# cts198859/deeprl_network

Hardware: AMD Instinct MI355X
Metric: env-steps/sec (agents x envs x steps/s), full rollout + A2C update loop (higher is better)
Workload: dtype f32; 1 GPU; CACC catchup, 8 agents x 4096 replicas/GPU, ia2c_fp (config_ia2c_fp_catchup.ini), n_step 60; replicas_per_gpu=4096, global_replicas=4096, parallelism=dp1, hipgraph_rollout=True, hipgraph_update=True, gemm_autotune=True

## Files before the change

deeprl_network_amd/_lib.py:

```python
import ctypes as C
import os

import torch

_PKG = os.path.dirname(os.path.abspath(__file__))
LIB_PATH = os.path.join(_PKG, 'libnmarl_hip.so')

if not os.path.exists(LIB_PATH):
    raise ImportError(
        'deeprl_network_amd: %s not found. Build it with `python -m deeprl_network_amd.build` '
        '(hipcc --offload-arch=gfx950). There is no CPU fallback.' % LIB_PATH)

from . import build as _build

if _build.built_hash() != _build.source_hash():
    raise ImportError(
        'deeprl_network_amd: %s is stale (built from sources %s, current sources %s). Rebuild it with '
        '`python -m deeprl_network_amd.build`.' % (LIB_PATH, _build.built_hash(), _build.source_hash()))

LIB_PATH = os.environ.get('NMARL_LIB_AB') or LIB_PATH
lib = C.CDLL(LIB_PATH)

ABI_VERSION = 4

# ... 49 lines not shown


class NetTopo(C.Structure):
    _fields_ = [('N', C.c_int32), ('L', C.c_int32), ('A', C.c_int32), ('m_max', C.c_int32), ('n_s', C.c_void_p),
                ('image', C.c_void_p)]


NET_OFF = dict(green=0, src=6144, group=7680, share=8448, fan=11520, dnptr=11648, dnpair=11728, nbr=13264)
NET_IMAGE_BYTES = 13568


class FcPart(C.Structure):
    _fields_ = [('x', C.c_void_p), ('x_sn', C.c_int64), ('x_row', C.c_int64), ('F', C.c_int32), ('gather_A', C.c_int32),
                ('m_max', C.c_int32), ('pad_', C.c_int32), ('nbr_idx', C.c_void_p), ('w', C.c_void_p), ('w_sn', C.c_int64),
                ('b', C.c_void_p), ('b_sn', C.c_int64)]


FC_MAX_PARTS = 4


class CaccEncode(C.Structure):
    _fields_ = ([(k, C.c_void_p) for k in ('w_ob', 'b_ob', 'w_fp', 'b_fp', 'fp', 'nbr_idx', 'out')] +
                [(k, C.c_int64) for k in ('w_ob_sn', 'b_ob_sn', 'w_fp_sn', 'b_fp_sn', 'fp_sn', 'out_sn', 'out_row')] +
                [('act', C.c_int32), ('n_parts', C.c_int32)])


class BatchEpilogue(C.Structure):
    _fields_ = ([('E', C.c_int64)] + [(k, C.c_int32) for k in ('N', 'H', 'A', 'F', 'T', 'T_env')] +
                [(k, C.c_void_p) for k in ('g', 'done', 'ep_sum', 'ep_sq', 'ep_len', 'fin', 'h_fw', 'c_fw', 'h_bw', 'c_bw', 'fp_T',
                                           'fp_uniform', 'x_T', 'fp_0', 'x_0', 'done_pre', 'scratch', 'skip_if')])


class TrainRecord(C.Structure):
    _fields_ = ([('rows', C.c_int64)] + [(k, C.c_int32) for k in ('N', 'A', 'G', 'K')] + [('lr', C.c_float), ('e_coef', C.c_float)] +
                [(k, C.c_void_p) for k in ('n_a', 'terms', 'grad_norm', 'lr_dev', 'R', 'Adv', 'action', 'ring', 'count', 'skip_if',
                                           'ws')])


class BpttCoupled(C.Structure):
    _fields_ = ([(k, C.c_int32) for k in ('kind', 'N', 'T', 'H', 'm_max', 'r_max', 'r_row', 'symmetric', 'mode', 'ring_slots')] +
                [('E', C.c_int64)] +
                [(k, C.c_void_p) for k in ('gates', 'c_all', 'done', 'dh_ext', 'img', 'img_m', 'mask', 'dz', 'd1', 'ring', 'db_part',
                                           'dbm_part', 'dhr_io', 'dc_io', 'ws', 'status', 'rev_agent', 'rev_col', 'rev_w')] +
                [(k, C.c_int64) for k in ('gates_sn', 'gates_st', 'c_sn', 'c_st', 'dh_sn', 'dh_st', 'img_sn', 'imgm_sn', 'mask_sn',
                                          'mask_st', 'mask_row', 'dz_sn', 'dz_st', 'd1_sn', 'd1_st', 'ring_sn', 'ring_slot', 'db_sn',
                                          'dbm_sn', 'io_sn')] +
                [('dy8', C.c_void_p), ('hw', C.c_void_p), ('dy_sn', C.c_int64), ('dy_st', C.c_int64), ('hw_sn', C.c_int64),
                 ('O', C.c_int32), ('pad2_', C.c_int32)])


class BpttDial(C.Structure):
    _fields_ = ([(k, C.c_int32) for k in ('N', 'T', 'H', 'm_max', 'r_max', 'r_row', 'symmetric', 'mode', 'ring_slots', 'O')] +
                [('E', C.c_int64)] +
                [(k, C.c_void_p) for k in ('gates', 'c_all', 'done', 'dh_ext', 'dy8', 'hw', 'img', 'img_m', 'img_f', 'hm', 'msg', 'dz',
                                           'ds', 'd1', 'd2', 'ring', 'db_part', 'dbm_part', 'dbf_part', 'dhr_io', 'dc_io', 'ws',
                                           'status', 'rev_agent', 'rev_col', 'rev_w')] +
                [(k, C.c_int64) for k in ('gates_sn', 'gates_st', 'c_sn', 'c_st', 'dh_sn', 'dh_st', 'dy_sn', 'dy_st', 'hw_sn', 'img_sn',
                                          'imgm_sn', 'imgf_sn', 'hm_sn', 'hm_st', 'hm_row', 'msg_sn', 'msg_st', 'dz_sn', 'dz_st',
                                          'ds_sn', 'ds_st', 'd1_sn', 'd1_st', 'd2_sn', 'd2_st', 'ring_sn', 'ring_slot', 'db_sn',
                                          'dbm_sn', 'dbf_sn', 'io_sn')])


class GridParams(C.Structure):
    _fields_ = [('norm_wave', C.c_float), ('clip_wave', C.c_float), ('peak1', C.c_float), ('peak2', C.c_float),
                ('T', C.c_int32), ('per_agent_reward', C.c_int32), ('compact_obs', C.c_int32),
                ('objective', C.c_int32), ('coef_wait', C.c_float), ('head_wait', C.c_void_p)]


class GridEnv(C.Structure):
    _fields_ = ([('params', C.POINTER(GridParams))] +
                [(k, C.c_void_p) for k in ('q', 'transit', 'prev_action', 't', 'xi', 'obs_out', 'reward', 'done', 'global_reward')] +
                [('auto_reset', C.c_int32), ('pad_', C.c_int32), ('seed', C.c_uint64), ('env_id_base', C.c_int64),
                 ('episode', C.c_void_p), ('words', C.c_void_p)])


class StepX(C.Structure):
    _fields_ = ([('E', C.c_int64)] + [(k, C.c_int32) for k in ('N', 'H', 'KX', 'KX2', 'precision', 'pad_')] +
                [('x', C.c_void_p), ('x_sn', C.c_int64), ('x_row', C.c_int64), ('x2', C.c_void_p), ('x2_sn', C.c_int64),
                 ('x2_row', C.c_int64)] +
                [('h_in', C.c_void_p), ('h_sn', C.c_int64)] +
                [f for k in ('img', 'bias', 'zadd1', 'zadd2', 'c_prev') for f in ((k, C.c_void_p), (k + '_sn', C.c_int64))] +
                [('done', C.c_void_p)] +
                [f for k in ('gates', 'c_new', 'h_new') for f in ((k, C.c_void_p), (k + '_sn', C.c_int64))] +
                [('head', C.POINTER(Head)), ('msg', C.POINTER(Msg)), ('enc', C.POINTER(StepEnc)), ('genv', C.POINTER(GridEnv))])


_p = C.c_void_p
_i64 = C.c_int64
_i32 = C.c_int32
_u64 = C.c_uint64
_f32 = C.c_float

SIGNATURES = {
    'nmarl_abi_version': [],
    'nmarl_cacc_reset': [C.POINTER(CaccParams), _i64, _p, _p, _u64, _i64, _p,
                         _p, _p, _p, _p, _p, _p, _p, _p, _i32, _p],
    'nmarl_cacc_step': [C.POINTER(CaccParams), _i64, _p, _p, _p, _p, _p, _p, _p, _p, _p, _p, _p,
                        _i32, _u64, _i64, _p, _p],
    'nmarl_cacc_step_encode': [C.POINTER(CaccParams), _i64, _p, _p, _p, _p, _p, _p, _p, _p, _p, _p, _p,
                               _i32, _u64, _i64, _p, C.POINTER(CaccEncode), _p],
    'nmarl_cacc_step_nv': [C.POINTER(CaccParams), _i64, _p, _p, _p, _p, _p, _p, _p, _p, _p, _p, _p,
                           _i32, _u64, _i64, _p, _i32, _p],
    'nmarl_cacc_reset_nv': [C.POINTER(CaccParams), _i64, _p, _p, _u64, _i64, _p,
                            _p, _p, _p, _p, _p, _p, _p, _p, _i32, _i32, _p],
    'nmarl_grid_reset': [C.POINTER(GridParams), _i64, _p, _p, _u64, _i64, _p, _p, _p, _p, _p, _p, _p, _p],
    'nmarl_grid_step': [C.POINTER(GridParams), _i64, _p, _p, _p, _p, _p, _p, _p, _p, _p, _p, _i32, _u64, _i64, _p, _p],
    'nmarl_grid_reset_rc': [C.POINTER(GridParams), _i64, _p, _p, _u64, _i64, _p, _p, _p, _p, _p, _p, _p, _p, _i32, _i32],
    'nmarl_grid_step_rc': [C.POINTER(GridParams), _i64, _p, _p, _p, _p, _p, _p, _p, _p, _p, _p, _i32, _u64, _i64, _p, _p,
                           _i32, _i32],
    'nmarl_net_reset': [C.POINTER(NetTopo), _i64, _p, _p, _u64, _i64, _p, _p, _p, _p, _p, _p, _p, _p],
    'nmarl_net_reset_obj': [C.POINTER(NetParams), C.POINTER(NetTopo), _i64, _p, _p, _u64, _i64, _p, _p, _p, _p, _p, _p, _p, _p],
    'nmarl_net_step': [C.POINTER(NetParams), C.POINTER(NetTopo), _i64, _p, _p, _p, _p, _p, _p, _p, _p, _p, _p, _i32, _u64, _i64,
                       _p, _p],
    'nmarl_atsc_traffic_begin': [_i64, _i32, _i32, _p, _p, _p, _p, _p],
    'nmarl_atsc_traffic_step': [_i64, _i32, _i32, _p, _p, _p, _p, _p, _p, _p, _p, _p, _p, _p],
    'nmarl_atsc_greedy': [_i64, _i32, _i32, _p, _p, _p, _i64, _p, _p],
    'nmarl_atsc_maxpressure': [_i64, _i32, _i32, _i32, _p, _p, _i32, _i32, _p, _p, _p, _p, _p, _i64, _p, _p],
    'nmarl_nbr_gather_fwd': [_i64, _i32, _i32, _i32, _p, _p, _p, _p],
    'nmarl_nbr_gather_bwd': [_i64, _i32, _i32, _i32, _p, _p, _p, _p],
    'nmarl_nbr_mean_fwd': [_i64, _i32, _i32, _i32, _p, _p, _p, _p],
    'nmarl_nbr_mean_bwd': [_i64, _i32, _i32, _i32, _p, _p, _p, _p],
    'nmarl_nbr_gather_bwd_add': [_i64, _i32, _i32, _i32, _p, _p, _p, _p, _p],
    'nmarl_nbr_mean_bwd_add': [_i64, _i32, _i32, _i32, _p, _p, _p, _p, _p],
    'nmarl_nbr_onehot': [_i64, _i32, _i32, _i32, _p, _p, _p, _i64, _p],
    'nmarl_lstm_cell_fwd': [_i64, _i32, _i32, _p, _i64, _p, _i64, _p, _i64, _p, _i64, _p, _p, _i64, _p, _i64, _p, _i64, _p],
    'nmarl_lstm_wimage_floats': [_i32],
    'nmarl_lstm_wimage': [_i32, _i32, _p, _i64, _p, _i64, _p, _i64, _i32, _p],
    'nmarl_lstm_step_x': [C.POINTER(StepX), _p],
    'nmarl_lstm_msg_wimage': [_i32, _i32, _p, _i64, _p, _i64, _p],
    'nmarl_lstm_step_sync_words': [_i64, _i32],
    'nmarl_lstm_step_env_words': [_i64],
    'nmarl_lstm_step_grid_words': [_i64],
    'nmarl_lstm_step_grid_env_blocks': [_i64, _i32],
    'nmarl_lstm_bptt_wimage_floats': [_i32],
    'nmarl_lstm_bptt_wimage': [_i32, _i32, _p, _i64, _p, _i64, _p, _i64, _p],
    'nmarl_lstm_bptt_step': [_i64, _i32, _i32, _i32, _p, _i64, _p, _i64, _p, _i64, _p, _p, _i64, _p, _i64, _p, _i64, _p, _i64, _p,
                             _i64, _p, _i64, _p, _i64, _p, _i64, _i64, _p, _i64, _i32, _p, _i64, _p],
    'nmarl_lstm_bptt_step_parts': [_i64],
    'nmarl_lstm_bptt_seq_blocks': [_i64],
    'nmarl_lstm_bptt_seq': [_i32, _i64, _i32, _i32, _p, _i64, _i64, _p, _i64, _i64, _p, _p, _i64, _i64, _p, _i64, _i64, _p, _i64, _i32,
                            _p, _i64, _p, _i64, _i64, _p, _i64, _p, _i64, _p, _i64, _p],
    'nmarl_lstm_bptt_msg_wimage': [_i32, _i32, _p, _i64, _p, _i64, _p],
    'nmarl_lstm_bptt_coupled_ws_words': [_i64, _i32],
    'nmarl_lstm_bptt_coupled': [C.POINTER(BpttCoupled), _p],
    'nmarl_lstm_bptt_dial': [C.POINTER(BpttDial), _p],
    'nmarl_fc_fwd': [_i64, _i32, _i32, _i32, _p, _i64, _i64, _p, _i64, _p, _i64, _i32, _p, _i64, _i64, _p],
    'nmarl_fc_fwd_multi': [_i64, _i32, _i32, C.POINTER(FcPart), _i32, _p, _i64, _i64, _p],
    'nmarl_dial_msg_adjoint': [_i64, _i32, _i32, _p, _i64, _p, _i64, _p, _i64, _p, _i64, _p, _i64, _p, _i64, _p, _p, _p, _i32,
                               _p, _i64, _p, _i64, _p, _i64, _p, _i64, _p, _i64, _p],
    'nmarl_dial_msg_adjoint_parts': [_i64],
    'nmarl_onehot_argmax_add': [_i64, _i32, _i32, _i32, _p, _i64, _p, _p, _i64, _i64, _p],
    'nmarl_fc_bwd_chunks': [_i64, _i32],
    'nmarl_fc_bwd': [_i64, _i32, _i32, _i32, _p, _i64, _i64, _p, _i64, _i64, _p, _i64, _i64, _i32, _p, _p, _i64, _p, _i64, _p],
    'nmarl_fc_bwd_pair': [_i64, _i32, _p, _p, _i64, _i64, _p, _i64, _p, _i64, _i64, _i32, _p, _p, _p],
    'nmarl_fc_bwd_gather': [_i64, _i32, _i32, _i32, _p, _i32, _p, _i64, _i64, _p, _i64, _i64, _p, _i64, _i64, _i32, _p, _p, _i64, _p, _i64, _p],
    'nmarl_heads_loss': [_i64, _i32, _i32, _i32, _p, _i64, _p, _i64, _p, _i64, _p, _p, _p, _p, _f32, _f32, _p, _p, _p, _p, _p, _i64, _p, _i64, _p,
                         _i64, _p],
    'nmarl_thin_linear_bwd': [_i64, _i32, _i32, _i32, _p, _i64, _p, _i64, _p, _i64, _p, _i64, _p, _p, _i64, _p, _i64, _p, _i64, _p],
    'nmarl_nbr_action_value_fwd': [_i64, _i32, _i32, _i32, _p, _p, _p, _i64, _p, _i32, _p],
    'nmarl_nbr_action_value_bwd': [_i64, _i32, _i32, _i32, _p, _p, _p, _p, _p, _i64, _p],
    'nmarl_bias_act': [_i64, _i32, _i32, _p, _i64, _p, _i64, _i32, _p, _i64, _i64, _p],
    'nmarl_lstm_cell_bwd': [_i64, _i32, _i32, _p, _i64, _p, _i64, _p, _i64, _p, _p, _i64, _p, _i64, _p, _i64, _p, _i64, _p, _i64, _p],
    'nmarl_a2c_loss_chunks': [_i64, _i32],
    'nmarl_a2c_loss_fwd': [_i64, _i32, _i32, _p, _i64, _i64, _p, _p, _p, _p, _f32, _f32, _p, _p, _p],
    'nmarl_a2c_loss_bwd': [_i64, _i32, _i32, _p, _i64, _i64, _p, _p, _p, _p, _f32, _f32, _p, _p, _p, _p],
    'nmarl_sample_actions': [_i64, _i32, _i32, _p, _p, _i32, _u64, _i64, _i64, _p, _p, _p],
    'nmarl_nstep_return': [_i64, _i32, _i32, _p, _p, _p, _p, C.c_double, C.c_double, _p, _p, _p, _p],
# ... 49 lines not shown
```

deeprl_network_amd/agents/models.py:

```python
import logging
import os

import numpy as np
import torch

from .. import ops, train_record
from .policies import (ConsensusPolicy, DIALMultiAgentPolicy, FPPolicy, IC3MultiAgentPolicy, LstmPolicy,
                       NCMultiAgentPolicy)
from .utils import Scheduler

F32 = torch.float32


class IA2C:

    policy_cls = LstmPolicy
    per_agent_optimizer = True
    uses_fingerprint = False

    def __init__(self, n_s_ls, n_a_ls, neighbor_mask, distance_mask, coop_gamma, total_step, model_config,
                 seed=0, num_envs=1, device='cuda', dist_group=None, n_feat=None, n_feat_ls=None, obs_order=None):
        self.name = getattr(self, 'name', 'ia2c')
        self._init_algo(n_s_ls, n_a_ls, neighbor_mask, distance_mask, coop_gamma, total_step, seed,
                        model_config, num_envs, device, dist_group, n_feat, n_feat_ls, obs_order)
# ... 144 lines not shown
        p = self.policy
        if p.hetero or p.n_obs == p.n_feat:
            return False
        if p.params[p.k_ob].shape[2] != ops.FC_J or p.n_obs > ops.FC_MAX_F:
            return False
        T, E, N = self.n_step, self.E, self.n_agent
        self.buf_x = torch.zeros(T + 1, E, N, p.n_feat, dtype=F32, device=self.device)
        self.compact_obs = True
        return True

    compact_obs = False

    def _save_slots(self, t):
        d = {k: v[:, t] for k, v in self.policy._extra.items()}
        d['S'] = self.S_buf[:, t]
        for k, v in getattr(self, '_extra_next', {}).items():
            d[k + '_next'] = v[:, t + 1]
        return d

    def reset_states(self, mask=None):
        self.policy.invalidate_cached_msg()
        if mask is None:
            for s in (self.h_fw, self.c_fw, self.h_bw, self.c_bw):
                s.zero_()
            self.fp.copy_(self.fp_uniform.expand_as(self.fp))
        else:
            keep = (mask == 0).to(F32).view(1, -1, 1)
            for s in (self.h_fw, self.c_fw, self.h_bw, self.c_bw):
                s.mul_(keep)
            self.fp.mul_(keep).add_((1.0 - keep) * self.fp_uniform)

    def _policy_step(self, obs, done, done_is_zero=False):
        self.policy.refresh_wimage()
        self._enc = self.policy.encode(obs, self.fp)
        self.policy.step(self._enc, self.h_fw, self.c_fw, done, self.h_fw, self.c_fw, done_is_zero)
        with torch.no_grad():
            return self.policy.pi(self.h_fw)

    def _value_step(self, obs, done, na_onehot, done_is_zero=False, out=None, reuse_enc=False):
        if not reuse_enc:
            self.policy.refresh_wimage()
        enc = self._enc if reuse_enc else self.policy.encode(obs, self.fp)
        self.policy.step(enc, self.h_fw, self.c_fw, done, self._h2, self._c2, done_is_zero, second=True)
        with torch.no_grad():
            return self.policy.value(self._h2, na_onehot, out=out)

    def encode_target(self, t):
        if t < self.n_step:
            return self.S_buf[:, t]
        if getattr(self, '_enc_boot', None) is None:
            self._enc_boot = torch.zeros_like(self.S_buf[:, 0])
        return self._enc_boot

    def act(self, done, mode=ops.SAMPLE_PHILOX, u=None, seed=0, env_id_base=0, step=0, step_dev=None,
            done_is_zero=False, pre_encoded=False, env_step=None):
        t = self.t
        p = self.policy
        ob = None
        if t == 0:
            p.refresh_wimage()
            if self.save_acts:
                self.H_all[:, 0].copy_(self.h_fw)
                self.C_all[:, 0].copy_(self.c_fw)
        if pre_encoded:
            enc = self.S_buf[:, t]
        elif self.save_acts and p.enc_in_kernel(self.E, self.compact_obs):
            enc, ob = self.S_buf[:, t], dict(x=self.buf_x[t], fp=self.fp, env=env_step, bits=self._relu_bits(t))
        elif self.save_acts and 'ENC' in p._extra:
            if p.encodes_in_step(self.E, self.compact_obs):
                enc, ob = p._extra['ENC'][:, t], (self.buf_x[t] if env_step is None else dict(x=self.buf_x[t], genv=env_step))
            else:
                enc = p.encode(self.buf_x[t], self.fp, out=p._extra['ENC'][:, t])
            p._enc_was_saved = True
        else:
            enc = p.encode(self.buf_x[t], self.fp, out=self.S_buf[:, t]) if self.save_acts else p.encode(self.buf_x[t], self.fp)
        if env_step is not None and (ob is None or not isinstance(ob, dict)):
            raise ValueError('env_step needs the lock-step kernel that runs the input encoders itself (policy.enc_in_kernel / encodes_in_step)')
        draw = dict(mode=mode, u=u, seed=seed, env_id_base=env_id_base, step=step, step_dev=step_dev)
        if self.save_acts and p.pv_one_launch(self.E):
            p.step_policy_value(enc, self.H_all[:, t], self.C_all[:, t], done, self.buf_fp[t + 1], self.buf_act[t],
                                self.buf_vn[:, t], h_out=self.H_all[:, t + 1], c_out=self.C_all[:, t + 1],
                                gates=self.G_buf[:, t], defer_action_term=True,
                                **(dict(save=self._save_slots(t), ob=ob, carry=self._msg_carry(t)) if p.coupled else
                                   (dict(ob=ob) if ob is not None else {})),
                                **draw)
            return self.buf_act[t]
        if self.save_acts:
            p.step_policy(enc, self.H_all[:, t], self.C_all[:, t], done, self.H_all[:, t + 1], self.C_all[:, t + 1],
                          self.buf_fp[t + 1], self.buf_act[t], done_is_zero, gates=self.G_buf[:, t], save=self._save_slots(t),
                          **draw)
            p.step_value(enc, self.H_all[:, t + 1], self.C_all[:, t + 1], done, self._h2, self._c2, self.buf_act[t],
                         self.buf_v[t], done_is_zero)
            return self.buf_act[t]
        if p.fused_pv:
            p.step_policy_value(enc, self.h_fw, self.c_fw, done, self.buf_fp[t + 1], self.buf_act[t], self.buf_v[t], **draw)
            return self.buf_act[t]
        p.step_policy(enc, self.h_fw, self.c_fw, done, self.h_fw, self.c_fw, self.buf_fp[t + 1], self.buf_act[t],
                      done_is_zero, **draw)
        p.step_value(enc, self.h_fw, self.c_fw, done, self._h2, self._c2, self.buf_act[t], self.buf_v[t], done_is_zero)
        return self.buf_act[t]

    _carry_buf = None
    _carry_holds = -1

    def _msg_carry(self, t):
        p = self.policy
        if not p.coupled or getattr(p, 'msg_kind', 0) not in (ops.MSG_GATHER_RELU, ops.MSG_MEAN_ADD) or \
                os.environ.get('NMARL_MSG_CARRY', '1') == '0':
            return None
        if self._carry_buf is None:
            self._carry_buf = torch.zeros(self.n_agent, self.E, self.n_lstm, dtype=F32, device=self.device)
        d = dict(carry_in=self._carry_buf if (t > 0 and self._carry_holds == t) else None,
                 carry_out=self._carry_buf if t < self.n_step else None)
        mm = getattr(p, '_extra_full', {}).get('MM')
        if mm is not None and t + 1 < self.n_step and p.msg_kind == ops.MSG_MEAN_ADD:
            d['mean_next'] = mm[:, t + 1]
        self._carry_holds = t + 1 if t < self.n_step else -1
        return d

    S_bits = None

    def _relu_bits(self, t):
        if os.environ.get('NMARL_FC_BWD_PAIR', '1') == '0' or not getattr(self.policy, 'enc_writes_bits', False):
            return None
        if self.S_bits is None:
            self.S_bits = torch.zeros(self.n_agent, self.n_step, self.E, 4, dtype=torch.int32, device=self.device)
        p = self.policy
        p._bits_steps = 1 if t == 0 else p._bits_steps + 1
        return self.S_bits[:, t]

    def record(self, reward, done_post):
        t = self.t
        self.buf_r[t].copy_(self._norm_reward(reward))
        self.buf_done_post[t].copy_(done_post)
        self.t = t + 1

    def _norm_reward(self, r):
        if self.reward_norm > 0:
            r = r / self.reward_norm
        if self.reward_clip > 0:
            r = torch.clamp(r, -self.reward_clip, self.reward_clip)
        return r

    def load_rewards(self, raw_rewards):
        if self.reward_norm > 0:
            torch.div(raw_rewards, self.reward_norm, out=self.buf_r)
        else:
            torch.mul(raw_rewards, 1.0, out=self.buf_r)
        if self.reward_clip > 0:
            self.buf_r.clamp_(-self.reward_clip, self.reward_clip)
        self.t = self.n_step

    def bootstrap(self, done, action_scratch, mode=ops.SAMPLE_PHILOX, u=None, seed=0, env_id_base=0,
                  step=0, step_dev=None, done_is_zero=False, pre_encoded=False):
        assert self.t == self.n_step
        p = self.policy
        ob = None
        if pre_encoded:
            enc = self.encode_target(self.n_step)
        elif self.save_acts and p.enc_in_kernel(self.E, self.compact_obs):
            enc, ob = (self.encode_target(self.n_step) if p.coupled else None), dict(x=self.buf_x[self.n_step], fp=self.fp)
        elif self.save_acts and p.encodes_in_step(self.E, self.compact_obs):
            enc, ob = self.encode_target(self.n_step), self.buf_x[self.n_step]
        else:
            enc = p.encode(self.buf_x[self.n_step], self.fp)
        if self.save_acts and p.pv_one_launch(self.E):
            T = self.n_step
            p.step_policy_value(enc, self.H_all[:, T], self.C_all[:, T], done, self._pi_boot, action_scratch, self._v_boot,
                                h_out=self.h_fw, c_out=self.c_fw, mode=mode, u=u, seed=seed, env_id_base=env_id_base,
                                step=step, step_dev=step_dev, **(dict(ob=ob) if ob is not None else {}),
                                **(dict(carry=self._msg_carry(T)) if p.coupled else {}))
            return self._v_boot
        if self.save_acts:
            T = self.n_step
            p.step_policy(enc, self.H_all[:, T], self.C_all[:, T], done, self.h_fw, self.c_fw, self._pi_boot, action_scratch,
                          done_is_zero, mode=mode, u=u, seed=seed, env_id_base=env_id_base, step=step, step_dev=step_dev)
            return p.step_value(enc, self.h_fw, self.c_fw, done, self._h2, self._c2, action_scratch, self._v_boot,
                                done_is_zero)
        if p.fused_pv:
            p.step_policy_value(enc, self.h_fw, self.c_fw, done, self._pi_boot, action_scratch, self._v_boot, mode=mode, u=u,
                                seed=seed, env_id_base=env_id_base, step=step, step_dev=step_dev)
            return self._v_boot
        p.step_policy(enc, self.h_fw, self.c_fw, done, self.h_fw, self.c_fw, self._pi_boot, action_scratch,
                      done_is_zero, mode=mode, u=u, seed=seed, env_id_base=env_id_base, step=step, step_dev=step_dev)
        return p.step_value(enc, self.h_fw, self.c_fw, done, self._h2, self._c2, action_scratch, self._v_boot,
                            done_is_zero)

    def _loss_backward_fused(self, Hs):
        N, T, E = self.n_agent, self.n_step, self.E
        p = self.policy
        if Hs.dim() != 3 or not ops.heads_loss_supported(Hs, self.n_a, p.nbr_idx) or \
                (not self.identical_agent and not self.per_agent_optimizer) or Hs.stride(2) != 1 or Hs.stride(1) != Hs.shape[2]:
            return False
        prm = p.params
        action = self.buf_act.view(T * E, N)
        as_dy = self.save_acts and p.bptt_takes_head_dy and os.environ.get('NMARL_BPTT_HEAD_DY', '1') != '0'
        r = ops.heads_loss(Hs.detach(), prm['pi_w'], prm['pi_b'], prm['v_w'], prm['v_b'], action, p.nbr_idx, self.n_a,
                           self.Adv.view(N, T * E), self.R.view(N, T * E), self.v_coef, self.e_coef, want_dh=not as_dy)
        terms = self._terms = r['terms']
        self.last_loss = (terms[:, 0], terms[:, 1], terms[:, 2], terms.sum(dim=1))
        for k in ('pi_w', 'pi_b', 'v_w', 'v_b'):
            prm[k].grad = r[k].reshape(prm[k].shape)
        Hs.backward(gradient=ops.head_dy_placeholder(r['dy8'], r['hw'], Hs) if as_dy else r['dh'])
        if as_dy and ops._pending_head_dy.pop(Hs.device, None) is not None:
            raise RuntimeError('the recurrence below Hs did not take the heads\' dy8 (ops.take_head_dy): its gradient is wrong')
        return True

    def _loss(self, Hs):
        N, T, E = self.n_agent, self.n_step, self.E
        p = self.policy
        action = self.buf_act.view(T * E, N)
        logits, v = p.heads(Hs, action)
        adv = self.Adv.view(N, T * E)
        R = self.R.view(N, T * E)
        if not self.identical_agent and not self.per_agent_optimizer:
            adv = adv.sum(dim=0, keepdim=True).expand(N, T * E).contiguous()
        if ops.a2c_loss_supported(self.n_a):
            per_agent, terms = ops.a2c_loss(logits, v, action, adv, R, self.v_coef, self.e_coef)
            self._terms = terms
            self.last_loss = (terms[:, 0], terms[:, 1], terms[:, 2], per_agent.detach())
            return per_agent.sum()
        pi = torch.softmax(logits, dim=-1)
        acts = action.t().long().unsqueeze(-1)
        log_pi = torch.log(torch.clamp(pi, 1e-10, 1.0))
        entropy = -(pi * log_pi).sum(-1)
        logp_a = log_pi.gather(-1, acts).squeeze(-1)
        policy_loss = -(logp_a * adv).mean(-1)
        value_loss = (R - v).pow(2).mean(-1) * 0.5 * self.v_coef
        entropy_loss = -entropy.mean(-1) * self.e_coef
        per_agent = policy_loss + value_loss + entropy_loss
        self._terms = None
        self.last_loss = (policy_loss.detach(), value_loss.detach(), entropy_loss.detach(), per_agent.detach())
        return per_agent.sum()

    def loss_terms(self):
        if self._terms is not None:
            return self._terms
        return torch.stack(self.last_loss[:3], dim=1).contiguous()

    def update(self, R_end, rotate=True):
        lr = self.update_begin()
        self.update_grads(R_end)
        self.update_reduce()
        self.update_apply(lr, rotate=rotate)
        self.update_end()

    def update_begin(self):
        assert self.t == self.n_step, 'update() needs a full n_step batch (got %d)' % self.t
        self.cur_lr = self.lr_scheduler.get(self.n_step)
        return self.cur_lr

    @property
    def handoff_guarded(self):
        return bool(self.policy.coupled) and self.device.type == 'cuda'
# ... 274 lines not shown
```

deeprl_network_amd/agents/policies.py:

```python
import os
import warnings

import numpy as np
import torch

from .. import ops
from . import sequence

warnings.filterwarnings('ignore', message='grad and param do not obey the gradient layout contract')

F32 = torch.float32


def ortho_init(shape, scale=np.sqrt(2)):
    a = np.random.standard_normal(shape)
    u, _, v = np.linalg.svd(a, full_matrices=False)
    q = u if u.shape == tuple(shape) else v
    return (scale * q.reshape(shape)).astype(np.float32)


class Layout:

    def __init__(self, rows=None, cols=None, exists=True, fill=0.0):
        self.rows, self.cols, self.exists, self.fill = rows, cols, exists, fill
# ... 245 lines not shown
        p = self.params
        H, A = self.n_h, self.n_a
        if ops.heads_supported(h, A, self.nbr_idx):
            return ops.heads(h, p['pi_w'], p['pi_b'], p['v_w'], p['v_b'], action, self.nbr_idx, A)
        w = torch.cat([p['pi_w'], p['v_w'][:, :H]], dim=2)
        b = torch.cat([p['pi_b'], p['v_b']], dim=1)
        out = torch.baddbmm(b.unsqueeze(1), h, w)
        na = ops.nbr_onehot(action, self.nbr_idx, A)
        return out[..., :A], out[..., A] + torch.bmm(na, p['v_w'][:, H:]).squeeze(-1)

    def value(self, h, na_onehot, out=None):
        p = self.params
        H = self.n_h
        v = torch.baddbmm(p['v_b'].unsqueeze(1), h, p['v_w'][:, :H])
        if out is not None:
            torch.baddbmm(v, na_onehot, p['v_w'][:, H:], out=out.unsqueeze(-1))
            return out
        return torch.baddbmm(v, na_onehot, p['v_w'][:, H:]).squeeze(-1)

    def encode(self, x, fp_prev, out=None):
        with torch.no_grad():
            if out is not None:
                return self._enc_infer(x.transpose(0, 1), fp_prev, out=out)
            return self._enc_infer(x.transpose(0, 1), fp_prev)

    def step(self, enc, h, c, done, h_out, c_out, done_is_zero=False, second=False):
        with torch.no_grad():
            z1, z2, xs = self._recur_addends(enc, h, second=second)
            wh, b = self.params[self.k_wh], self.params[self.k_b]
            if self.n_h == ops.FUSED_H:
                ops.lstm_step_fused(h, wh, b, z1, z2, c, done, None, c_out, h_out, xs=xs, **self._prec_kw)
            else:
                hk = h if done_is_zero else h * (1.0 - done).view(1, -1, 1)
                z = torch.bmm(hk, wh) if z2 is None else torch.baddbmm(z2, hk, wh)
                ops.lstm_cell_infer(z, b, c, done, c_out, h_out, z2=z1)
        return h_out, c_out

    @property
    def fused_heads(self):
        return self.n_h == ops.FUSED_H and self.n_a <= ops.HEAD_MAX_A

    def step_policy(self, enc, h, c, done, h_out, c_out, pi_out, act_out, done_is_zero=False, gates=None, save=None,
                    **draw):
        with torch.no_grad():
            if self.fused_heads:
                z1, z2, xs = self._recur_addends(enc, h, save=save, fuse_msg=self.msg_inplace_ok or h_out.data_ptr() != h.data_ptr())
                p = self.params
                ops.lstm_step_policy(h, p[self.k_wh], p[self.k_b], z1, z2, c, done, c_out, h_out, p['pi_w'], p['pi_b'],
                                     pi_out, act_out, xs=xs, gates=gates, **self._prec_kw, **draw)
            else:
                self.step(enc, h, c, done, h_out, c_out, done_is_zero)
                pi_out.copy_(self.pi(h_out))
                ops.sample_actions(pi_out, act_out, **draw)
        return pi_out, act_out

    @property
    def fused_pv(self):
        return self.fused_heads and not self.coupled

    @property
    def fused_pv_coupled(self):
        return self.coupled and self.fused_heads and self.msg_kind != ops.MSG_DIAL and self._msg() is not None

    def pv_one_launch(self, E):
        if self.fused_pv:
            return True
        K = self.n_h * self.m_max if self.msg_kind == ops.MSG_GATHER_RELU else self.n_h
        if K > ops.MSG_MAX_K:
            return False
        return self.fused_pv_coupled and ops.step_handoff_supported(self.N, E, self.device, K=K)

    def _sync_words(self, E):
        pool = self.__dict__.setdefault('_sync_pool', {})
        if E not in pool:
            pool[E] = ops.step_sync_words(self.N, E, self.device)
        return pool[E]

    def encodes_in_step(self, E, compact):
        return False

    _bits_steps = 0

    def invalidate_cached_msg(self):
        """(lstm_dial keeps message vectors of the last policy step: see DIALMultiAgentPolicy)"""

    def enc_in_kernel(self, E, compact):
        return False

    @property
    def env_step_in_kernel(self):
        return True

    def step_policy_value(self, enc, h, c, done, pi_out, act_out, v_out, h_out=None, c_out=None, gates=None,
                          defer_action_term=False, save=None, ob=None, carry=None, **draw):
        with torch.no_grad():
            if self.coupled:
                z1, z2, xs = self._recur_addends(enc, h, save=save, fuse_msg=True)
                xs[4]['sync'] = self._sync_words(h.shape[1])
                if carry:
                    xs[4].update(carry)
                if isinstance(ob, dict) and 'genv' in ob:
                    xs[4]['ob'], xs[4]['genv'] = self._ob_spec(ob['x']), ob['genv']
                elif isinstance(ob, dict):
                    xs[4]['enc_spec'] = self._enc_spec(ob['x'], ob['fp'], None, ob.get('env'), ob.get('bits'))
                elif ob is not None:
                    xs[4]['ob'] = self._ob_spec(ob)
            elif ob is not None:
                z1, z2, xs = None, None, (self._enc_spec(ob['x'], ob['fp'], enc, ob.get('env'), ob.get('bits')), self.params[self.k_wx],
                                          self._step_img)
            else:
                z1, z2, xs = self._recur_addends(enc, h)
            p = self.params
            ops.lstm_step_policy_value(h, p[self.k_wh], p[self.k_b], z1, z2, c, done, p['pi_w'], p['pi_b'], pi_out, act_out,
                                       p['v_w'], p['v_b'], self.nbr_idx, self.n_a, v_out, xs=xs, h_out=h_out, c_out=c_out,
                                       gates=gates, defer_action_term=defer_action_term, **self._prec_kw, **draw)
        return act_out

    @property
    def bptt_takes_head_dy(self):
        if self.coupled and os.environ.get('NMARL_BPTT_HEAD_DY_COUPLED', '1') == '0':
            return False
        return self.xside

    @property
    def can_save_acts(self):
        return self.xside and self.fused_heads

    def unroll_saved(self, X, FP, S, G, Hall, Call, done, masked_steps=None, S_ext=None, S_bits=None):
        T, E = done.shape
        Xv = X.reshape(T * E, self.N, X.shape[-1]).transpose(0, 1)
        if self.coupled:
            return self._unroll_saved_coupled(Xv, FP, S, G, Hall, Call, done, masked_steps, S_ext, S_bits)
        if S_bits is not None:
            s = self._enc(Xv, FP, saved=S.view(self.N, T * E, S.shape[-1]), bits=S_bits.view(self.N, T * E, 4))
        else:
            s = self._enc(Xv, FP, saved=S.view(self.N, T * E, S.shape[-1]))
        Hs = ops.lstm_sequence_saved(s.view(self.N, T, E, s.shape[-1]), self.params[self.k_wx], self.params[self.k_wh],
                                     self.params[self.k_b], G, Hall, Call, done, masked_steps, s_ext=S_ext)
        return Hs.reshape(self.N, T * E, self.n_h)

    def save_spec(self):
        return {}

    def _unroll_saved_coupled(self, Xv, FP, S, G, Hall, Call, done, masked_steps, S_ext=None, S_bits=None):
        T, E = done.shape
        kind, wx, w_msg, b_msg, mfc_w, mfc_b = self._seq_args()
        enc = self._enc_saved(Xv, FP, S) if S_bits is None else self._enc_saved(Xv, FP, S, bits=S_bits.view(self.N, T * E, 4))
        extra = dict(getattr(self, '_extra', {}))
        if kind == 'dial' and 'A2' in getattr(self, '_extra_full', {}) and extra.get('A2') is not None:
            extra['A2'] = self._extra_full['A2']
        if kind == 'ic3':
            mm = getattr(self, '_extra_full', {}).get('MM') if getattr(self, '_mm_was_saved', False) else None
            extra['A1'] = mm if (mm is not None and mm.shape[1] == T + 1) else None
        Hs = sequence.coupled_sequence_saved(kind, self.nbr_idx, masked_steps, enc.view(self.N, T, E, enc.shape[-1]), done,
                                             self.params[self.k_wx], self.params[self.k_wh], self.params[self.k_b],
                                             w_msg, b_msg, mfc_w, mfc_b, G, Hall, Call, S, extra, s_ext=S_ext)
        return Hs.reshape(self.N, T * E, self.n_h)

    def step_value(self, enc, h, c, done, h_out, c_out, action, v_out, done_is_zero=False):
        with torch.no_grad():
            if self.fused_heads:
                z1, z2, xs = self._recur_addends(enc, h, second=True, fuse_msg=True)
                p = self.params
                ops.lstm_step_value(h, p[self.k_wh], p[self.k_b], z1, z2, c, done, c_out, h_out, p['v_w'], p['v_b'],
                                    action, self.nbr_idx, self.n_a, v_out, xs=xs, **self._prec_kw)
            else:
                self.step(enc, h, c, done, h_out, c_out, done_is_zero, second=True)
                self.value(h_out, ops.nbr_onehot(action, self.nbr_idx, self.n_a), out=v_out)
        return v_out

    def fused_env_encode(self, fp_next, out):
        return None

    def _fused_spec(self, ob, fp_keys, fp_next, out):
        p = self.params
        if self.hetero or self.n_feat != 5 or self.m_max != 2 or self.n_a != 4 or p[ob[0]].shape[1:] != (15, 64):
            return None
        d = dict(w_ob=p[ob[0]], b_ob=p[ob[1]], nbr_idx=self.nbr_idx, out=out, act=ops.BIAS_RELU)
        if fp_keys is not None:
            if p[fp_keys[0]].shape[1:] != (8, 64):
                return None
            d.update(w_fp=p[fp_keys[0]], b_fp=p[fp_keys[1]], fp=fp_next)
        return d

    def _enc_one_launch(self, xv, width):
        return width == ops.FC_J and self.n_obs <= ops.FC_MAX_F and self.n_na <= ops.FC_MAX_F

    def _compact(self, xv):
        return xv.shape[2] == self.n_feat and self.n_obs != self.n_feat

    def _ob_part(self, xv, w_key, b_key):
        p = self.params
        return (xv, p[w_key], p[b_key], self.nbr_self if self._compact(xv) else None)

    def _fc_ob_infer(self, xv, w_key, b_key, act, out=None):
        if self._compact(xv):
            return ops.fc_fwd_multi([self._ob_part(xv, w_key, b_key)], act, out=out)
        return self._fc_infer(xv, w_key, b_key, act, out=out)

    def expand_obs(self, X):
        idx = self.nbr_self.long()
        g = X[..., idx.clamp(min=0), :] * (idx >= 0).to(X.dtype).unsqueeze(-1)
        return g.reshape(*X.shape[:-1], self.n_obs)

    def _fc_infer(self, x, w_key, b_key, act, out=None):
        w, b = self.params[w_key], self.params[b_key]
        if ops.fc_supported(x, w):
            return ops.fc_fwd(x, w, b, act, out=out)
        return ops.bias_act_(torch.bmm(x, w), b, act, out=out)

    def _recur_addends(self, enc, h, second=False, save=None, fuse_msg=False):
        if self.xside:
            return None, None, (enc, self.params[self.k_wx], self._step_img)
        return enc, None, self._wh_xs()

    k_wx = None
    _img = None
    _img_x3 = None

    @property
    def _prec_kw(self):
        return {} if self.precision == 'fp32' else {'precision': self.precision}

    @property
    def _step_img(self):
        return self._img_x3 if self.precision == 'bf16x3' else self._img

    @property
    def xside(self):
        return self.k_wx is not None and ops.xside_supported(self.params[self.k_wx].shape[1], self.n_h)

    def refresh_wimage(self):
        if self.xside:
            self._img = ops.lstm_wimage(self.params[self.k_wx], self.params[self.k_wh], out=self._img)
            if self.precision == 'bf16x3':
                self._img_x3 = ops.lstm_wimage(self.params[self.k_wx], self.params[self.k_wh], out=self._img_x3, precision='bf16x3')
            if self.msg_kind and ops.msg_supported(self.msg_kind, self.m_max, self.n_h):
                self._msg_img = ops.lstm_msg_wimage(self.params['w_msg'], out=self._msg_img)
        elif self.n_h == ops.FUSED_H:
            self._img = ops.lstm_wimage(None, self.params[self.k_wh], out=self._img)

    def _wh_xs(self):
        return (None, None, self._img) if self.n_h == ops.FUSED_H else None

    msg_kind = 0
    msg_inplace_ok = False
    _msg_img = None

    def _msg(self, **kw):
        if not (self.xside and self.msg_kind and self._msg_img is not None):
            return None
        p = self.params
        return dict(kind=self.msg_kind, nbr_idx=self.nbr_idx, w_msg=p['w_msg'], b_msg=p['w_msg_b'], img=self._msg_img, **kw)

    def unroll(self, X, FP, done, h0, c0, masked_steps=None):
        T, E = done.shape
        Xv = X.reshape(T * E, self.N, X.shape[-1]).transpose(0, 1)
        enc = self._enc(Xv, FP)
        if not self.coupled:
            if self.xside:
                self.refresh_wimage()
                Hs = ops.lstm_sequence_x(enc.view(self.N, T, E, enc.shape[-1]), self.params[self.k_wx],
                                         self.params[self.k_wh], self.params[self.k_b], h0, c0, done, masked_steps,
                                         self._img)
            else:
                Hs = ops.lstm_sequence(enc.view(self.N, T, E, enc.shape[-1]), self.params[self.k_wh],
                                       self.params[self.k_b], h0, c0, done, masked_steps)
            return Hs.reshape(self.N, T * E, self.n_h)
        if self.fused_coupled:
            kind, wx, w_msg, b_msg, mfc_w, mfc_b = self._seq_args()
            Hs = sequence.coupled_sequence(kind, self.nbr_idx, masked_steps, enc.view(self.N, T, E, enc.shape[-1]), h0, c0,
                                           done, wx, self.params[self.k_wh], self.params[self.k_b], w_msg, b_msg,
                                           mfc_w, mfc_b)
            return Hs.reshape(self.N, T * E, self.n_h)
        enc_steps = enc.view(self.N, T, E, enc.shape[-1]).unbind(1)
        h, c = h0, c0
        hs = []
        wh, b = self.params[self.k_wh], self.params[self.k_b]
        for t in range(T):
            zx = self._recur_in(enc_steps[t], h)
            keep = (1.0 - done[t]).view(1, -1, 1)
            z = torch.baddbmm(zx, h * keep, wh)
            h, c = ops.lstm_cell(z, b, c, done[t])
            hs.append(h)
        return torch.stack(hs, dim=1).reshape(self.N, T * E, self.n_h)


class LstmPolicy(BatchedPolicy):
    name = 'lstm'
    summary_name = 'lstm_0'
    k_wh, k_b, k_wx = 'lstm_wh', 'lstm_b', 'lstm_wx'
    k_ob = 'fc_w'
    coupled = False

    def _phases(self):
        nf, H, F = self.n_fc, self.n_h, self.n_feat
        return [[('fc_w', 'lstm_%d/fc/w', (self.n_obs, nf), self._L_slots),
                 ('fc_b', 'lstm_%d/fc/b', (nf,), None),
                 ('lstm_wx', 'lstm_%d/lstm/wx', (nf, 4 * H), None),
                 ('lstm_wh', 'lstm_%d/lstm/wh', (H, 4 * H), None),
                 ('lstm_b', 'lstm_%d/lstm/b', (4 * H,), None)] + self._head_phase('lstm_%d/pi', 'lstm_%d/v')]

    def _enc(self, xv, fp, saved=None):
        p = self.params
        s = ops.fc_concat([self._ob_part(xv, 'fc_w', 'fc_b')], ops.BIAS_RELU, saved=saved)
        return s if self.xside else ops.linear(s, p['lstm_wx'])

    def _enc_infer(self, xv, fp, out=None):
        s = self._fc_ob_infer(xv, 'fc_w', 'fc_b', ops.BIAS_RELU, out=out)
        return s if self.xside else torch.bmm(s, self.params['lstm_wx'])

    def fused_env_encode(self, fp_next, out):
        return self._fused_spec(('fc_w', 'fc_b'), None, fp_next, out) if self.xside else None

    enc_writes_bits = False
# ... 280 lines not shown
                for j in tab[i]:
                    if j >= 0:
                        A[i, j] = 1.0
            self._avg = torch.from_numpy(A / A.sum(1, keepdims=True)).to(self.device)
        with torch.no_grad():
            blk = ps.flat[:, o0:o1]
            blk.copy_(self._avg @ blk)


class DIALMultiAgentPolicy(BatchedPolicy):
    @property
    def bptt_takes_head_dy(self):
        return BatchedPolicy.bptt_takes_head_dy.fget(self) and ops.dial_bptt_table(self.nbr_idx, self.n_h) is not None

    name = 'dial'
    summary_name = 'dial'
    k_wh, k_b, k_wx = 'wh_hid', 'hid_b', 'wx_hid'
    k_ob = 'w_ob'
    coupled = True
    msg_kind = ops.MSG_DIAL
    msg_inplace_ok = True

    def _phases(self):
        H, F = self.n_h, self.n_feat
        s = 'dial/lstm_comm_%d'
        return [[('w_msg', s + '/w_msg', (H * self.m_max, H), self._L_nbr(H)),
                 ('w_msg_b', s + '/b_msg', (H,), self._L_nbr()),
                 ('w_ob', s + '/w_ob', (self.n_obs, H), self._L_slots),
                 ('w_ob_b', s + '/b_ob', (H,), None),
                 ('wx_hid', s + '/wx_hid', (H, 4 * H), None),
                 ('wh_hid', s + '/wh_hid', (H, 4 * H), None),
                 ('hid_b', s + '/b_hid', (4 * H,), None)],
                [('mfc_w', 'dial/mfc_%d/w', (H, H), None), ('mfc_b', 'dial/mfc_%d/b', (H,), None)],
                self._head_phase('dial/pi_%d', 'dial/v_%d')]

    def _ai_scale(self, fp):
        if not self.hetero:
            return None
        if not hasattr(self, '_has_nbr'):
            self._has_nbr = torch.tensor([float(self._m(i) > 0) for i in range(self.N)], dtype=fp.dtype,
                                         device=fp.device).view(self.N, 1, 1)
        return self._has_nbr

    def _own_action_onehot(self, fp):
        oh = torch.nn.functional.one_hot(torch.argmax(fp, dim=-1), self.n_h).to(fp.dtype)
        sc = self._ai_scale(fp)
        return oh if sc is None else oh * sc

    def _enc(self, xv, fp):
        p = self.params
        return ops.fc_concat([self._ob_part(xv, 'w_ob', 'w_ob_b')], ops.BIAS_RELU) + self._own_action_onehot(fp)

    def _recur_in(self, enc, h):
        p = self.params
        msg = torch.relu(torch.baddbmm(p['mfc_b'].unsqueeze(1), h, p['mfc_w']))
        hm = torch.relu(torch.baddbmm(p['w_msg_b'].unsqueeze(1), ops.nbr_gather(msg, self.nbr_idx), p['w_msg']))
        return torch.bmm(enc + hm, p['wx_hid'])

    def _enc_saved(self, xv, fp, S):
        return ops.fc_concat([self._ob_part(xv, 'w_ob', 'w_ob_b')], ops.BIAS_RELU)

    def _enc_infer(self, xv, fp, out=None):
        sc = self._ai_scale(fp)
        return ops.onehot_argmax_add_(self._fc_ob_infer(xv, 'w_ob', 'w_ob_b', ops.BIAS_RELU), fp, None if sc is None else sc.view(-1))

    def save_spec(self):
        return {'A1': self.n_h, 'A2': self.n_h}

    _x_target = IC3MultiAgentPolicy._x_target

    save_next = ('A2',)
    _mfc_img = None
    _m_next = None
    _h_out = None
    _nxt = None

    def refresh_wimage(self):
        super().refresh_wimage()
        if self._msg_img is not None:
            self._mfc_img = ops.lstm_msg_wimage(self.params['mfc_w'], out=self._mfc_img)
        self._m_next = None

    def invalidate_cached_msg(self):
        self._m_next = None

    def _cached_msg(self, h):
        m = self._m_next
        if m is not None and m[0] == h.data_ptr() and m[1] == h._version and m[2].shape == h.shape:
            return m[2]
        return None

    def step_policy(self, enc, h, c, done, h_out, c_out, pi_out, act_out, done_is_zero=False, gates=None, save=None, **draw):
        self._nxt, self._h_out = None, h_out
        try:
            r = super().step_policy(enc, h, c, done, h_out, c_out, pi_out, act_out, done_is_zero, gates=gates, save=save, **draw)
        finally:
            self._h_out = None
        self._m_next = None if self._nxt is None else (h_out.data_ptr(), h_out._version, self._nxt)
        return r

    def _recur_addends(self, enc, h, second=False, save=None, fuse_msg=False):
        p = self.params
        keep = save is not None and not second
        fused = fuse_msg and self._msg() is not None
        msg = self._cached_msg(h) if fused else None
        if msg is None:
            msg = self._fc_infer(h, 'mfc_w', 'mfc_b', ops.BIAS_RELU, out=save['A2'] if keep else None)
        elif keep and msg.data_ptr() != save['A2'].data_ptr():
            save['A2'].copy_(msg)
        if fused:
            m = self._msg(src=msg, enc=enc, out=save['S'] if keep else None, out2=save['A1'] if keep else None)
            if not second and self._h_out is not None and self._mfc_img is not None:
                nxt = save.get('A2_next') if keep else None
                if nxt is None:
                    nxt = self._scratch('_mn0', h)
                    if nxt.data_ptr() == msg.data_ptr():
                        nxt = self._scratch('_mn1', h)
                m['next'] = dict(img=self._mfc_img, b=p['mfc_b'], w=p['mfc_w'], out=nxt)
                self._nxt = nxt
            return None, None, (None, p['wx_hid'], self._img, None, m)
        hm = self._fc_infer(ops.nbr_gather(msg, self.nbr_idx), 'w_msg', 'w_msg_b', ops.BIAS_RELU,
                            out=save['A1'] if keep else None)
        if self.xside:
            x = self._x_target(h, second, save)
            torch.add(hm, enc, out=x)
            return None, None, (x, p['wx_hid'], self._img)
        return torch.bmm(hm.add_(enc), p['wx_hid']), None, self._wh_xs()

    def _seq_args(self):
        p = self.params
        return 'dial', p['wx_hid'], p['w_msg'], p['w_msg_b'], p['mfc_w'], p['mfc_b']
```

deeprl_network_amd/csrc/lstm_mfma.hip:

```cpp
#include "common.h"
#include "cacc_tile.h"
#include "grid_tile.h"
#include <stdlib.h>
#include <type_traits>

namespace {

typedef float f32x16 __attribute__((ext_vector_type(16)));

constexpr int H = 64;
constexpr int G4 = 4 * H;
constexpr int ROWS_B = 128;
constexpr int APITCH = H + 1;

struct FusedArgs {
    const float *h_in, *bias, *zadd1, *zadd2, *c_prev, *done;
    float *gates, *c_new, *h_new;
    int64_t h_sn, bias_sn, zadd1_sn, zadd2_sn, c_prev_sn, gates_sn, c_new_sn, h_new_sn;
    int64_t E;
    int blocks_per_agent;
    nmarl_head_t hd;
};

constexpr int MAXA = 8;

__device__ __forceinline__ float sigm(float x) {
    return __builtin_amdgcn_rcpf(1.0f + __builtin_amdgcn_exp2f(-1.4426950408889634f * x));
}
__device__ __forceinline__ float tanh_fast(float x) { return 2.0f * sigm(2.0f * x) - 1.0f; }

typedef float f32x4 __attribute__((ext_vector_type(4)));
__device__ __forceinline__ f32x4 sigm4(const f32x4 x) {
    f32x4 t = x * -1.4426950408889634f;
    t[0] = __builtin_amdgcn_exp2f(t[0]); t[1] = __builtin_amdgcn_exp2f(t[1]);
    t[2] = __builtin_amdgcn_exp2f(t[2]); t[3] = __builtin_amdgcn_exp2f(t[3]);
    t = t + 1.0f;
    t[0] = __builtin_amdgcn_rcpf(t[0]); t[1] = __builtin_amdgcn_rcpf(t[1]);
    t[2] = __builtin_amdgcn_rcpf(t[2]); t[3] = __builtin_amdgcn_rcpf(t[3]);
    return t;
}
__device__ __forceinline__ f32x4 tanh4(const f32x4 x) { return sigm4(x * 2.0f) * 2.0f - 1.0f; }
constexpr int R16 = 16;
constexpr int WAVES2 = 8;

#ifdef NMARL_STEP_TIMELINE
__device__ unsigned long long* g_timeline = nullptr;
__global__ void timeline_set_kernel(unsigned long long* p) { g_timeline = p; }
#define NMARL_STAMP(i) if (g_timeline && blockIdx.x == 0 && (threadIdx.x & 63) == 0) g_timeline[(threadIdx.x >> 6) * 64 + (i)] = __builtin_amdgcn_s_memtime();
#define NMARL_NOTE(i, v) if (g_timeline && blockIdx.x == 0 && (threadIdx.x & 63) == 0) g_timeline[(threadIdx.x >> 6) * 64 + (i)] = (unsigned long long)(v);
#else
#define NMARL_STAMP(i)
#define NMARL_NOTE(i, v)
#endif

template <int KIND>
__device__ __forceinline__ void head_epilogue(const FusedArgs& a, const int n, const int N, const int64_t row0,
                                              const int lane, const float* a_tile, const float* w_h) {
    static_assert(KIND == 2 || KIND == 3, "critic heads only (the actor's is head_policy_lds)");
    const nmarl_head_t& hd = a.hd;
    const int rl = lane & 15, q = lane >> 4;
    float acc = 0.0f;
#pragma unroll 4
    for (int kk = 0; kk < 16; ++kk) {
        const int k = q * 16 + kk;
        acc += a_tile[rl * APITCH + k] * w_h[k];
    }
    if (KIND == 3) { NMARL_STAMP(34) }
    acc += __shfl_xor(acc, 16, 64);
    acc += __shfl_xor(acc, 32, 64);
    if (KIND == 3) { NMARL_STAMP(35) }
    const int64_t row = row0 + rl;
    if (q != 0 || row >= a.E) return;
    const float* b = KIND == 3 ? hd.b2 + (int64_t)n * hd.b2_sn : hd.b + (int64_t)n * hd.b_sn;
    float v = acc + b[0];
    if (KIND == 2) {
        const float* w = hd.w + (int64_t)n * hd.w_sn;
        for (int k = 0; k < hd.m_max; ++k) {
            const int j = hd.nbr_idx[n * hd.m_max + k];
            if (j >= 0) v += w[H + k * hd.A + (int)hd.act_in[row * N + j]];
        }
    }
    hd.v_out[(int64_t)n * hd.v_sn + row] = v;
// ... 66 lines not shown
            const Philox4 r = philox4x32_10((uint32_t)(hd.env_id_base + row), (uint32_t)(n >> 2), (uint32_t)step, NMARL_STREAM_ACTION,
                                            (uint32_t)hd.seed, (uint32_t)(hd.seed >> 32));
            const uint32_t w = (n & 3) == 0 ? r.x : (n & 3) == 1 ? r.y : (n & 3) == 2 ? r.z : r.w;
            uu = u01_from_bits(w);
        }
        double tot = 0.0;
#pragma unroll
        for (int k = 0; k < AN; ++k) tot += (double)p[k];
        double cum = 0.0;
#pragma unroll
        for (int k = 0; k < AN; ++k) {
            cum += (double)p[k];
            act = (k < A && cum / tot <= (double)uu) ? k + 1 : act;
        }
        act = act > A - 1 ? A - 1 : act;
    }
    hd.act_out[row * N + n] = (uint8_t)act;
    return act;
}

__device__ __forceinline__ int head_policy_lds(const FusedArgs& a, const int n, const int N, const int64_t row0,
                                               const int lane, const float* a_tile, const float* wl, const float* bl) {
    if (a.hd.A <= 4) return head_policy_lds_n<4>(a, n, N, row0, lane, a_tile, wl, bl);
    if (a.hd.A == 5) return head_policy_lds_n<8, 5>(a, n, N, row0, lane, a_tile, wl, bl);
    return head_policy_lds_n<8>(a, n, N, row0, lane, a_tile, wl, bl);
}

constexpr int CH_K = 32;
constexpr int CH_FLOATS = CH_K * 16 * 20;
constexpr int HW_FLOATS = H * MAXA + MAXA + H;
constexpr int LDSX_FLOATS = 2 * CH_FLOATS + WAVES2 * R16 * APITCH + HW_FLOATS;
constexpr int MAX_KX = 256;

struct XArgs {
    FusedArgs f;
    const float* x; int64_t x_sn, x_row;
    const float* x2; int64_t x2_sn, x2_row;
    const float* img; int64_t img_sn;
    int nx, nx1, N;
    int msg_kc, m_max;
    const int32_t* nbr_idx;
    const float* msg_img; int64_t msg_img_sn;
    const float* msg_b; int64_t msg_b_sn;
    const float* enc; int64_t enc_sn, enc_row;
    float* xm_out; int64_t xm_sn, xm_row;
    const float* carry_in; int64_t carry_in_sn;
    float* carry_out; int64_t carry_out_sn;
    float* mm_next; int64_t mm_next_sn, mm_next_row;
    float* mm_out; int64_t mm_sn, mm_row;
    const float* src; int64_t src_sn;
    float* xm2_out; int64_t xm2_sn, xm2_row;
    const float* nxt_img; int64_t nxt_img_sn;
    const float* nxt_b; int64_t nxt_b_sn;
    float* nxt_out; int64_t nxt_out_sn;
    unsigned* sync;
    const float* ob; int64_t ob_row;
    int ob_F, ob_segs;
    const int32_t* ob_nbr;
    const float* ob_img; int64_t ob_img_sn;
    const float* ob_b; int64_t ob_b_sn;
    int32_t* status;
    unsigned max_spins;
    int fault;
    const float* e_ob; int64_t e_ob_row;
    const float* e_fp; int64_t e_fp_sn;
    const float *e_wob, *e_bob, *e_wfp, *e_bfp;
    int64_t e_wob_sn, e_bob_sn, e_wfp_sn, e_bfp_sn;
    float* e_out; int64_t e_out_sn, e_out_row;
    unsigned* e_bits; int64_t e_bits_sn;
    int e_nbr[64];
    int e_ob_rows;
    int ev_on, ev_auto_reset;
    nmarl_cacc_params_t ev_p;
    float *ev_h, *ev_v, *ev_u; int32_t* ev_t; uint8_t* ev_coll; float* ev_v0;
    float* ev_obs; float* ev_rew; uint8_t* ev_done; float* ev_grew;
    uint64_t ev_seed; int64_t ev_base; int32_t* ev_episode;
    unsigned* ev_cnt;
    int gv_on, gv_lstm_blocks, gv_auto_reset;
    nmarl_grid_params_t gv_p;
    float *gv_q, *gv_tr; uint8_t* gv_prev; int32_t* gv_t; float* gv_xi;
    float* gv_obs; float* gv_rew; uint8_t* gv_done; float* gv_grew;
    uint64_t gv_seed; int64_t gv_base; int32_t* gv_episode;
    unsigned long long* gv_words;
};

typedef unsigned int u32x4v __attribute__((__vector_size__(16)));
typedef __attribute__((address_space(1))) unsigned gu32;
constexpr int SC1 = 16;
__device__ __forceinline__ __amdgpu_buffer_rsrc_t make_rsrc(const float* p, const uint32_t bytes) {
    return __builtin_amdgcn_make_buffer_rsrc(const_cast<float*>(p), 0, bytes, 0x00020000);
}

#define NMARL_MFMA16(av, b0, b1, b2, b3)                                                  \
    {                                                                                     \
        acc[0] = __builtin_amdgcn_mfma_f32_16x16x4f32(av, b0.x, acc[0], 0, 0, 0);         \
        acc[1] = __builtin_amdgcn_mfma_f32_16x16x4f32(av, b0.y, acc[1], 0, 0, 0);         \
        acc[2] = __builtin_amdgcn_mfma_f32_16x16x4f32(av, b0.z, acc[2], 0, 0, 0);         \
        acc[3] = __builtin_amdgcn_mfma_f32_16x16x4f32(av, b0.w, acc[3], 0, 0, 0);         \
        acc[4] = __builtin_amdgcn_mfma_f32_16x16x4f32(av, b1.x, acc[4], 0, 0, 0);         \
        acc[5] = __builtin_amdgcn_mfma_f32_16x16x4f32(av, b1.y, acc[5], 0, 0, 0);         \
        acc[6] = __builtin_amdgcn_mfma_f32_16x16x4f32(av, b1.z, acc[6], 0, 0, 0);         \
        acc[7] = __builtin_amdgcn_mfma_f32_16x16x4f32(av, b1.w, acc[7], 0, 0, 0);         \
        acc[8] = __builtin_amdgcn_mfma_f32_16x16x4f32(av, b2.x, acc[8], 0, 0, 0);         \
        acc[9] = __builtin_amdgcn_mfma_f32_16x16x4f32(av, b2.y, acc[9], 0, 0, 0);         \
        acc[10] = __builtin_amdgcn_mfma_f32_16x16x4f32(av, b2.z, acc[10], 0, 0, 0);       \
        acc[11] = __builtin_amdgcn_mfma_f32_16x16x4f32(av, b2.w, acc[11], 0, 0, 0);       \
        acc[12] = __builtin_amdgcn_mfma_f32_16x16x4f32(av, b3.x, acc[12], 0, 0, 0);       \
        acc[13] = __builtin_amdgcn_mfma_f32_16x16x4f32(av, b3.y, acc[13], 0, 0, 0);       \
        acc[14] = __builtin_amdgcn_mfma_f32_16x16x4f32(av, b3.z, acc[14], 0, 0, 0);       \
        acc[15] = __builtin_amdgcn_mfma_f32_16x16x4f32(av, b3.w, acc[15], 0, 0, 0);       \
    }
#define NMARL_BLOAD(dst, buf, krow)                                                       \
    {                                                                                     \
        const float4* q_ = reinterpret_cast<const float4*>((buf) + (krow) * 320);         \
        dst##0 = q_[0]; dst##1 = q_[1]; dst##2 = q_[2]; dst##3 = q_[3];                   \
    }
#define NMARL_CHUNK(buf, A0, A1)                                                          \
    {                                                                                     \
        float4 p0, p1, p2, p3, q0, q1, q2, q3;                                            \
        NMARL_BLOAD(p, buf, 0)                                                            \
        NMARL_BLOAD(q, buf, 1) __builtin_amdgcn_sched_barrier(0);                         \
        NMARL_MFMA16(A0.x, p0, p1, p2, p3) __builtin_amdgcn_sched_barrier(0);             \
        NMARL_BLOAD(p, buf, 2) __builtin_amdgcn_sched_barrier(0);                         \
        NMARL_MFMA16(A0.y, q0, q1, q2, q3) __builtin_amdgcn_sched_barrier(0);             \
        NMARL_BLOAD(q, buf, 3) __builtin_amdgcn_sched_barrier(0);                         \
        NMARL_MFMA16(A0.z, p0, p1, p2, p3) __builtin_amdgcn_sched_barrier(0);             \
        NMARL_BLOAD(p, buf, 16) __builtin_amdgcn_sched_barrier(0);                        \
        NMARL_MFMA16(A0.w, q0, q1, q2, q3) __builtin_amdgcn_sched_barrier(0);             \
        NMARL_BLOAD(q, buf, 17) __builtin_amdgcn_sched_barrier(0);                        \
        NMARL_MFMA16(A1.x, p0, p1, p2, p3) __builtin_amdgcn_sched_barrier(0);             \
        NMARL_BLOAD(p, buf, 18) __builtin_amdgcn_sched_barrier(0);                        \
        NMARL_MFMA16(A1.y, q0, q1, q2, q3) __builtin_amdgcn_sched_barrier(0);             \
        NMARL_BLOAD(q, buf, 19) __builtin_amdgcn_sched_barrier(0);                        \
        NMARL_MFMA16(A1.z, p0, p1, p2, p3) __builtin_amdgcn_sched_barrier(0);             \
        NMARL_MFMA16(A1.w, q0, q1, q2, q3)                                                \
    }

typedef __attribute__((ext_vector_type(8))) __bf16 bf16x8;
constexpr int X3_PITCH = 132;
static_assert(63 * X3_PITCH + 128 <= CH_FLOATS, "bf16x3 chunk image fits the fp32 chunk");

__device__ __forceinline__ void split_bf16x3(const float4 a0, const float4 a1, bf16x8& hi, bf16x8& lo) {
    const float v[8] = {a0.x, a0.y, a0.z, a0.w, a1.x, a1.y, a1.z, a1.w};
#pragma unroll
    for (int j = 0; j < 8; ++j) {
        const __bf16 h = (__bf16)v[j];
        hi[j] = h;
        lo[j] = (__bf16)(v[j] - (float)h);
    }
}

#define NMARL_MFMA3(ACC, ah, al, bh, bl)                                                  \
    ACC = __builtin_amdgcn_mfma_f32_16x16x32_bf16(al, bh, ACC, 0, 0, 0);                  \
    ACC = __builtin_amdgcn_mfma_f32_16x16x32_bf16(ah, bl, ACC, 0, 0, 0);                  \
    ACC = __builtin_amdgcn_mfma_f32_16x16x32_bf16(ah, bh, ACC, 0, 0, 0);

__device__ __forceinline__ void chunk_bf16x3(f32x4 (&acc)[16], const float* buf, const float4 a0, const float4 a1) {
    bf16x8 ah, al;
    split_bf16x3(a0, a1, ah, al);
    const bf16x8* q = reinterpret_cast<const bf16x8*>(buf);
    bf16x8 p0 = q[0], p1 = q[1], r0 = q[2], r1 = q[3];
    __builtin_amdgcn_sched_barrier(0);
#pragma unroll
    for (int t = 0; t < 16; t += 2) {
        NMARL_MFMA3(acc[t], ah, al, p0, p1)
        __builtin_amdgcn_sched_barrier(0);
        if (t + 2 < 16) { p0 = q[2 * t + 4]; p1 = q[2 * t + 5]; }
        __builtin_amdgcn_sched_barrier(0);
        NMARL_MFMA3(acc[t + 1], ah, al, r0, r1)
        __builtin_amdgcn_sched_barrier(0);
        if (t + 2 < 16) { r0 = q[2 * t + 6]; r1 = q[2 * t + 7]; }
        __builtin_amdgcn_sched_barrier(0);
    }
}


template <int HEAD, int MSG, int ENC = 0, int CARRY = 0, int PREC = 0>
__global__ __launch_bounds__(512, 1) void lstm_step_x_kernel(const XArgs xa) {
    extern __shared__ __attribute__((aligned(16))) float lds[];
    const FusedArgs& a = xa.f;
    NMARL_STAMP(0)
    constexpr bool GENV = HEAD == 4 && MSG == 2;
    const unsigned n_lstm = (GENV && xa.gv_on) ? (unsigned)xa.gv_lstm_blocks : gridDim.x;
    if (GENV && xa.gv_on && blockIdx.x >= n_lstm) {
        nmarl_grid::Lds* el = reinterpret_cast<nmarl_grid::Lds*>(lds);
        float* bq = reinterpret_cast<float*>(el + 16);
        float* bt = bq + 16 * nmarl_grid::NQ;
        nmarl_grid::grid_step_groups<0, true, false, 16, true>(
            xa.gv_p, a.E, (int64_t)(blockIdx.x - n_lstm), (int64_t)(gridDim.x - n_lstm), nullptr, xa.gv_words, xa.status, xa.max_spins, xa.gv_q,
            xa.gv_tr, xa.gv_prev, xa.gv_t, xa.gv_xi, xa.gv_obs, xa.gv_rew, xa.gv_done, xa.gv_grew, xa.gv_auto_reset, xa.gv_seed, xa.gv_base,
            xa.gv_episode, el, bq, bt, bt);
        return;
    }
    int n, blk_u;
    nmarl_xcd_work(blockIdx.x, n_lstm, a.blocks_per_agent, n, blk_u);
    unsigned ka_touch = 0;
    if (ENC) {
        const __attribute__((address_space(4))) unsigned* ka =
            (const __attribute__((address_space(4))) unsigned*)__builtin_amdgcn_kernarg_segment_ptr();
#pragma unroll
        for (unsigned o = 0; o < sizeof(XArgs); o += 64) ka_touch |= ka[o / 4];
    }
    const float* const e_ob = xa.e_ob; const float* const e_fp = xa.e_fp;
    const float* const e_wob = xa.e_wob; const float* const e_bob = xa.e_bob;
    const float* const e_wfp = xa.e_wfp; const float* const e_bfp = xa.e_bfp;
    float* const e_out = xa.e_out;
    unsigned* const e_bits = xa.e_bits;
    const int64_t e_bits_sn = xa.e_bits_sn;
    const int64_t e_ob_row = xa.e_ob_row, e_fp_sn = xa.e_fp_sn, e_wob_sn = xa.e_wob_sn, e_bob_sn = xa.e_bob_sn, e_wfp_sn = xa.e_wfp_sn,
                  e_bfp_sn = xa.e_bfp_sn, e_out_sn = xa.e_out_sn, e_out_row = xa.e_out_row;
    int e_nb0 = -1, e_nb1 = -1;
    int e_nb2 = -1, e_nb3 = -1;
    if (ENC >= 3) {
        const int ns_ = __builtin_amdgcn_readfirstlane(n);
        const int nb4_ = xa.e_nbr[ns_];
        e_nb0 = (nb4_ << 24) >> 24; e_nb1 = (nb4_ << 16) >> 24; e_nb2 = (nb4_ << 8) >> 24; e_nb3 = nb4_ >> 24;
        asm volatile("" :: "s"(e_ob), "s"(e_fp), "s"(e_wob), "s"(e_bob), "s"(e_wfp), "s"(e_bfp), "s"(e_out), "s"(e_ob_row), "s"(e_fp_sn),
                     "s"(e_wob_sn), "s"(e_bob_sn), "s"(e_wfp_sn), "s"(e_bfp_sn), "s"(e_out_sn), "s"(e_out_row), "s"(e_nb0), "s"(e_nb1), "s"(e_nb2),
                     "s"(e_nb3), "s"(e_bits), "s"(e_bits_sn));
    } else if (ENC) {
        const int ns_ = __builtin_amdgcn_readfirstlane(n);
        e_nb0 = xa.e_nbr[2 * ns_]; e_nb1 = xa.e_nbr[2 * ns_ + 1];
        asm volatile("" :: "s"(e_ob), "s"(e_fp), "s"(e_wob), "s"(e_bob), "s"(e_wfp), "s"(e_bfp), "s"(e_out), "s"(e_ob_row), "s"(e_fp_sn),
                     "s"(e_wob_sn), "s"(e_bob_sn), "s"(e_wfp_sn), "s"(e_bfp_sn), "s"(e_out_sn), "s"(e_out_row), "s"(e_nb0), "s"(e_nb1), "s"(e_bits),
                     "s"(e_bits_sn));
    }
    const int64_t row_blk = (int64_t)blk_u * ROWS_B;
    const int lane = threadIdx.x & 63, wave = threadIdx.x >> 6;
    const int64_t row0 = row_blk + wave * R16;
    const int c = lane & 15, grp = lane >> 4;
    static_assert(HEAD != 4 || MSG != 0, "HEAD 4 is the coupled nets' policy + value step");
    static_assert(PREC == 0 || MSG == 0, "bf16x3: the uncoupled nets' step forms only");
    constexpr bool PV = HEAD == 3 || HEAD == 4;
    unsigned epoch_raw = 0;
    if (HEAD == 4) epoch_raw = __hip_atomic_load((gu32*)xa.sync, __ATOMIC_RELAXED, __HIP_MEMORY_SCOPE_AGENT);
    int nbj[8];
    if (MSG != 0) {
#pragma unroll
        for (int k = 0; k < 8; ++k) nbj[k] = xa.nbr_idx[n * xa.m_max + (k < xa.m_max ? k : 0)];
    }
    constexpr bool OBENC = HEAD == 4 && MSG == 2;
    const bool ob_here = OBENC && xa.ob != nullptr;
    float4 bv4 = float4{0.f, 0.f, 0.f, 0.f}, bo4 = float4{0.f, 0.f, 0.f, 0.f};
    if (MSG != 0) {
        const float* mbias_ = xa.msg_b + (int64_t)n * xa.msg_b_sn;
        bv4 = *reinterpret_cast<const float4*>(mbias_ + 4 * (lane & 15));
        if (OBENC) bo4 = *reinterpret_cast<const float4*>((ob_here ? xa.ob_b + (int64_t)n * xa.ob_b_sn : mbias_) + 4 * (lane & 15));
    }
    NMARL_STAMP(40)
    constexpr bool DEPH = MSG == 0 && ENC == 0;
    constexpr int NBUF = DEPH ? 3 : 2;
    static_assert(ENC == 0 || (MSG == 0 && HEAD == 3) || (ENC == 1 && MSG == 1 && HEAD == 4), "ENC: the policy + value launch of IA2C(-FP) / ConseNet / NeurComm");
    static_assert(ENC >= 0 && ENC <= 4 && (ENC < 3 || PREC == 0), "ENC 3 / 4 (general input layout): fp32 only");
    constexpr bool EFP = ENC == 1 || ENC == 3;
    constexpr bool EGEN = ENC >= 3;
    constexpr int EMT = EFP ? 8 : 4;
    constexpr bool ENC_LDS = ENC != 0 && MSG == 0, ENC_GLB = ENC != 0 && MSG != 0;
    float* hw_lds = ENC_LDS ? lds + NBUF * CH_FLOATS : lds + NBUF * CH_FLOATS + WAVES2 * R16 * APITCH;
    float* a_tile = (ENC_LDS ? hw_lds + HW_FLOATS : lds + NBUF * CH_FLOATS) + wave * R16 * APITCH;
    float4* xslot = reinterpret_cast<float4*>(hw_lds + HW_FLOATS) + threadIdx.x;
    const int nx = xa.nx, nch = xa.nx + 2;
    const float4* img = reinterpret_cast<const float4*>(xa.img + (int64_t)n * xa.img_sn);

    float4 sg0, sg1, sg2, sg3, sg4;
#define NMARL_STAGE_LOAD(ch)                                                              \
    {                                                                                     \
        const float4* g_ = img + (int64_t)(ch) * (CH_FLOATS / 4) + threadIdx.x;           \
        sg0 = g_[0]; sg1 = g_[512]; sg2 = g_[1024]; sg3 = g_[1536]; sg4 = g_[2048];       \
    }
#define NMARL_STAGE_STORE(b)                                                              \
    {                                                                                     \
        float4* d_ = reinterpret_cast<float4*>(lds + (b) * CH_FLOATS) + threadIdx.x;      \
        d_[0] = sg0; d_[512] = sg1; d_[1024] = sg2; d_[1536] = sg3; d_[2048] = sg4;       \
    }
    NMARL_STAGE_LOAD(0)
    float4 tg0, tg1, tg2, tg3, tg4;
    {
        const float4* g_ = img + (CH_FLOATS / 4) + threadIdx.x;
        tg0 = g_[0]; tg1 = g_[512]; tg2 = g_[1024]; tg3 = g_[1536]; tg4 = g_[2048];
    }

    const int64_t arow = row0 + c < a.E ? row0 + c : a.E - 1;
    const float keepA = 1.0f - a.done[arow];
    const float* xrow = xa.x ? xa.x + (int64_t)n * xa.x_sn + arow * xa.x_row + 4 * grp : nullptr;
    const float* x2row = xa.x2 ? xa.x2 + (int64_t)n * xa.x2_sn + arow * xa.x2_row + 4 * grp : nullptr;
    const int nx1 = xa.nx1;
    const float* hrow = a.h_in + (int64_t)n * a.h_sn + arow * H + 4 * grp;
    float4 a0, a1, n0, n1;
#define NMARL_A_LOAD(ch, d0, d1)      \
    if (ENC_LDS) {       \
        const int hc_ = (ch) - nx < 0 ? 0 : (ch) - nx;                                    \
        const int xc_ = (ch) < nx ? (ch) : nx - 1;                                        \
        const float4 h0_ = *reinterpret_cast<const float4*>(hrow + hc_ * CH_K);           \
        const float4 h1_ = *reinterpret_cast<const float4*>(hrow + hc_ * CH_K + 16);      \
        const float4 x0_ = xslot[512 * (2 * xc_)], x1_ = xslot[512 * (2 * xc_ + 1)];      \
        const bool isx_ = (ch) < nx;                                                      \
        d0.x = isx_ ? x0_.x : h0_.x; d0.y = isx_ ? x0_.y : h0_.y; d0.z = isx_ ? x0_.z : h0_.z; d0.w = isx_ ? x0_.w : h0_.w; \
        d1.x = isx_ ? x1_.x : h1_.x; d1.y = isx_ ? x1_.y : h1_.y; d1.z = isx_ ? x1_.z : h1_.z; d1.w = isx_ ? x1_.w : h1_.w; \
    } else if (MSG != 0 && (ch) >= nx - 2 && (ch) < nx) {        \
        const float* t_ = a_tile + c * APITCH + ((ch) - (nx - 2)) * CH_K + 4 * grp;       \
        d0.x = t_[0]; d0.y = t_[1]; d0.z = t_[2]; d0.w = t_[3];                           \
        d1.x = t_[16]; d1.y = t_[17]; d1.z = t_[18]; d1.w = t_[19];                       \
    } else if ((ch) < nx) {                                                               \
        const float* p_ = (ch) < nx1 ? xrow + (ch) * CH_K : x2row + ((ch) - nx1) * CH_K;  \
        d0 = *reinterpret_cast<const float4*>(p_);                                        \
        d1 = *reinterpret_cast<const float4*>(p_ + 16);                                   \
    } else {                                                                              \
        d0 = *reinterpret_cast<const float4*>(hrow + ((ch) - nx) * CH_K);                 \
        d1 = *reinterpret_cast<const float4*>(hrow + ((ch) - nx) * CH_K + 16);            \
    }
#define NMARL_A_MASK(ch, d0, d1)                                                          \
    {                                                                                     \
        const float kf_ = (ch) < nx ? 1.0f : keepA;                                       \
        d0.x *= kf_; d0.y *= kf_; d0.z *= kf_; d0.w *= kf_;                               \
        d1.x *= kf_; d1.y *= kf_; d1.z *= kf_; d1.w *= kf_;                               \
    }
#define NMARL_KCHUNK(CB, A0, A1)                                                          \
    if constexpr (PREC != 0) {                                                            \
        chunk_bf16x3(acc, (CB) + (16 * grp + c) * X3_PITCH, A0, A1);                      \
    } else {                                                                              \
        const float* buf = (CB) + (4 * grp * 16 + c) * 20;                                \
        NMARL_CHUNK(buf, A0, A1)                                                          \
    }
    if (MSG == 0 && ENC == 0) { NMARL_A_LOAD(0, a0, a1) }
    float ein[ENC == 3 ? 24 : ENC == 4 ? 16 : ENC == 1 ? 6 : (ENC ? 4 : 1)];
    float ewt[ENC == 3 ? 12 : ENC == 4 ? 8 : ENC == 1 ? 3 : (ENC ? 2 : 1)];
    f32x4 eacc[EFP ? 8 : (ENC ? 4 : 1)];
    if constexpr (EGEN) {
        __builtin_amdgcn_sched_barrier(0);
        const int ns = __builtin_amdgcn_readfirstlane(n);
        const int F = xa.ob_F, A = (xa.e_ob_rows >> 16) & 255, fp_rows = (xa.e_ob_rows >> 8) & 255;
        const int obk = (xa.e_ob_rows & 255) >> 2, fpk = (fp_rows + 3) >> 2;
        {
            const float* obr = e_ob + arow * e_ob_row + grp;
            int slot = 0, f0 = 0;
#pragma unroll
            for (int s_ = 0; s_ < 16; ++s_) {
                int ag = ns;
                ag = slot == 1 ? e_nb0 : ag; ag = slot == 2 ? e_nb1 : ag; ag = slot == 3 ? e_nb2 : ag; ag = slot == 4 ? e_nb3 : ag;
                const bool ok = s_ < obk && ag >= 0;
                const float v = obr[ok ? ag * F + f0 : ns * F];
                ein[s_] = ok ? v : 0.0f;
                f0 += 4;
                if (f0 >= F) { f0 = 0; ++slot; }
            }
            if constexpr (EFP) {
#pragma unroll
                for (int s_ = 0; s_ < 8; ++s_) {
                    const int kk = 4 * s_ + grp;
                    const int sl = (kk >= A ? 1 : 0) + (kk >= 2 * A ? 1 : 0) + (kk >= 3 * A ? 1 : 0);
                    int ag = e_nb0;
                    ag = sl == 1 ? e_nb1 : ag; ag = sl == 2 ? e_nb2 : ag; ag = sl == 3 ? e_nb3 : ag;
                    const bool ok = s_ < fpk && kk < fp_rows && ag >= 0;
                    const float v = e_fp[(int64_t)(ok ? ag : ns) * e_fp_sn + arow * A + (ok ? kk - sl * A : 0)];
                    ein[16 + s_] = ok ? v : 0.0f;
                }
            }
        }
#pragma unroll
        for (int q = 0; q < (EFP ? 12 : 8); ++q) {
            const int e = (q < 8 ? q : q - 8) * 512 + (int)threadIdx.x;
            const int s_ = e >> 8, l_ = (e >> 2) & 63, mt_ = e & 3, g_ = l_ >> 4, i_ = l_ & 15;
            const bool live = s_ < (q < 8 ? obk : fpk);
            int row = 4 * s_ + g_;
            row = q < 8 ? row : (row < fp_rows ? row : fp_rows - 1);
            const float* src = q < 8 ? e_wob + (int64_t)n * e_wob_sn : e_wfp + (int64_t)n * e_wfp_sn;
            ewt[q] = src[(live ? row : 0) * H + 16 * mt_ + i_];
        }
        float4 eb4 = float4{0.f, 0.f, 0.f, 0.f};
        if (threadIdx.x < (EFP ? 32 : 16))
            eb4 = *reinterpret_cast<const float4*>((threadIdx.x < 16 ? e_bob + (int64_t)n * e_bob_sn : e_bfp + (int64_t)n * e_bfp_sn - H) + 4 * threadIdx.x);
        eacc[0] = f32x4{eb4.x, eb4.y, eb4.z, eb4.w};
        __builtin_amdgcn_sched_barrier(0);
// ... 31 lines not shown
            eb4 = *reinterpret_cast<const float4*>((threadIdx.x < 16 ? e_bob + (int64_t)n * e_bob_sn : e_bfp + (int64_t)n * e_bfp_sn - H) + 4 * threadIdx.x);
        eacc[0] = f32x4{eb4.x, eb4.y, eb4.z, eb4.w};
        __builtin_amdgcn_sched_barrier(0);
        NMARL_STAMP(36)
    }
    int64_t rofs[4];
#pragma unroll
    for (int r = 0; r < 4; ++r) {
        const int64_t row = row0 + 4 * grp + r;
        rofs[r] = row < a.E ? row : a.E - 1;
    }
    float* m_lds = hw_lds + HW_FLOATS;
    float hw0 = 0.0f, hw1 = 0.0f, hw2 = 0.0f;
    if (HEAD != 0) {
        const nmarl_head_t& hd = a.hd;
        const float* w1 = hd.w + (int64_t)n * hd.w_sn;
        if (HEAD == 2) {
            hw2 = w1[threadIdx.x & (H - 1)];
        } else {
            const int A = hd.A;
            const int k = threadIdx.x >> 3, o = threadIdx.x & 7;
            hw0 = w1[k * A + (o < A ? o : 0)];
            hw1 = (hd.b + (int64_t)n * hd.b_sn)[(threadIdx.x & 7) < A ? (threadIdx.x & 7) : 0];
            if (PV) hw2 = (hd.w2 + (int64_t)n * hd.w2_sn)[threadIdx.x & (H - 1)];
        }
    }
    NMARL_STAMP(44)
    float* o_lds = m_lds + xa.msg_kc * (CH_K * 64);
    constexpr int MIQ = MSG == 2 ? 2 : 4;
    float4 mi[MSG != 0 ? MIQ : 1], oi[OBENC ? 2 : 1];
    if (MSG != 0) {
        const float4* g = reinterpret_cast<const float4*>(xa.msg_img + (int64_t)n * xa.msg_img_sn);
        const int lim = xa.msg_kc * (CH_K * 64 / 4);
#pragma unroll
        for (int q = 0; q < MIQ; ++q) { const int i = threadIdx.x + 512 * q; mi[q] = g[i < lim ? i : 0]; }
    }
    if (OBENC) {
        const float4* g = ob_here ? reinterpret_cast<const float4*>(xa.ob_img + (int64_t)n * xa.ob_img_sn) : img;
#pragma unroll
        for (int q = 0; q < 2; ++q) oi[q] = g[threadIdx.x + 512 * q];
    }
    constexpr bool NXT = HEAD == 1 && MSG == 3;
    const bool nxt_here = NXT && xa.nxt_out != nullptr;
    float4 nfa = float4{0.f, 0.f, 0.f, 0.f}, nfb = nfa, nb4 = nfa;
    if (NXT) {
        const float4* g = nxt_here ? reinterpret_cast<const float4*>(xa.nxt_img + (int64_t)n * xa.nxt_img_sn) : img;
        nfa = g[threadIdx.x]; nfb = g[threadIdx.x + 512];
        nb4 = *reinterpret_cast<const float4*>((nxt_here ? xa.nxt_b + (int64_t)n * xa.nxt_b_sn : xa.msg_b + (int64_t)n * xa.msg_b_sn) + 4 * (lane & 15));
    }
    auto msg_load = [&](auto second_c, auto k0_c, float4 (&U)[16], float (&W)[4]) {
        constexpr bool SECOND = decltype(second_c)::value;
        constexpr int k0 = decltype(k0_c)::value;
        const float* hsrc = MSG == 3 ? xa.src : SECOND ? a.h_new : a.h_in;
        const int64_t hsn = MSG == 3 ? xa.src_sn : SECOND ? a.h_new_sn : a.h_sn;
        const float* hbase = hsrc + arow * H + 4 * grp;
        const uint32_t hoff = (uint32_t)((arow * H + 4 * grp) * 4), hbytes = (uint32_t)(a.E * (H * 4));
        auto load2 = [&](const int jj, const int col, float4& u0, float4& u1) {
            if (SECOND) {
                const __amdgpu_buffer_rsrc_t r_ = make_rsrc(hsrc + (int64_t)jj * hsn, hbytes);
                u0 = __builtin_bit_cast(float4, __builtin_amdgcn_raw_buffer_load_b128(r_, hoff + col * 4, 0, SC1));
                u1 = __builtin_bit_cast(float4, __builtin_amdgcn_raw_buffer_load_b128(r_, hoff + col * 4 + 64, 0, SC1));
            } else {
                const float* p_ = hbase + (int64_t)jj * hsn + col;
                u0 = *reinterpret_cast<const float4*>(p_);
                u1 = *reinterpret_cast<const float4*>(p_ + 16);
            }
        };
#pragma unroll
        for (int q = 0; q < (MSG == 2 ? 4 : 2); ++q) {
            const int k = k0 + q;
            const int j = nbj[k];
            const bool ok = k < xa.m_max && j >= 0;
            W[q] = ok ? 1.0f : 0.0f;
            load2(ok ? j : n, 0, U[4 * q + 0], U[4 * q + 1]);
            load2(ok ? j : n, CH_K, U[4 * q + 2], U[4 * q + 3]);
        }
    };
    float4 PU[16];
    float PW[4];
    using K0 = std::integral_constant<int, 0>;
    using K2 = std::integral_constant<int, 2>;
    using K4 = std::integral_constant<int, 4>;
    constexpr bool MSG_WIDE = HEAD != 4 && MSG == 1;
    static_assert(CARRY == 0 || (HEAD == 4 && (MSG == 1 || MSG == 2)), "the message carry exists between one-launch lock-steps");
    constexpr bool carried = CARRY == 2;
    if (MSG != 0) {
        if (carried) {
            const float* ci = xa.carry_in + (int64_t)n * xa.carry_in_sn + 4 * c;
#pragma unroll
            for (int r = 0; r < 4; ++r) PU[r] = *reinterpret_cast<const float4*>(ci + rofs[r] * H);
            PW[0] = PW[1] = PW[2] = PW[3] = 0.0f;
        } else {
            msg_load(std::false_type{}, K0{}, PU, PW);
        }
    }
    float4 ea[OBENC ? 4 : 1];
    float eaw[OBENC ? 4 : 1];
    if (OBENC) {
        const float* obr = ob_here ? xa.ob + arow * xa.ob_row : hrow;
        const int F = ob_here ? xa.ob_F : 64, segs = ob_here ? xa.ob_segs : 0;
#pragma unroll
        for (int q = 0; q < 4; ++q) {
            int f = (q >> 1) * CH_K + 16 * (q & 1) + 4 * grp, seg = 0;
            while (f >= F) { f -= F; ++seg; }
            int j = n;
#pragma unroll
            for (int k = 0; k < 8; ++k) j = seg == k + 1 ? nbj[k] : j;
            const bool ok = seg < segs && (seg == 0 || seg - 1 < xa.m_max) && j >= 0;
            eaw[q] = ok ? 1.0f : 0.0f;
            ea[q] = *reinterpret_cast<const float4*>(obr + (ok ? j * F + f : 0));
        }
    }
    NMARL_STAMP(41)
    NMARL_STAGE_STORE(0)
    NMARL_STAMP(42)

    f32x4 acc[16];
    float4 b4s[4];
    {
        const float* bn = a.bias + (int64_t)n * a.bias_sn;
        const float* z1 = MSG == 0 && a.zadd1 ? a.zadd1 + (int64_t)n * a.zadd1_sn : nullptr;
        const float* z2 = MSG == 0 && a.zadd2 ? a.zadd2 + (int64_t)n * a.zadd2_sn : nullptr;
#pragma unroll
        for (int g4 = 0; g4 < 4; ++g4) b4s[g4] = *reinterpret_cast<const float4*>(bn + g4 * H + 4 * c);
        if (MSG == 0) {
#pragma unroll
            for (int g4 = 0; g4 < 4; ++g4)
#pragma unroll
                for (int r = 0; r < 4; ++r) {
                    acc[4 * g4 + 0][r] = b4s[g4].x; acc[4 * g4 + 1][r] = b4s[g4].y; acc[4 * g4 + 2][r] = b4s[g4].z; acc[4 * g4 + 3][r] = b4s[g4].w;
                }
        }
        if (z1) {
#pragma unroll
            for (int g4 = 0; g4 < 4; ++g4)
#pragma unroll
                for (int r = 0; r < 4; ++r) {
                    const float4 v4 = *reinterpret_cast<const float4*>(z1 + rofs[r] * G4 + g4 * H + 4 * c);
                    acc[4 * g4 + 0][r] += v4.x; acc[4 * g4 + 1][r] += v4.y; acc[4 * g4 + 2][r] += v4.z; acc[4 * g4 + 3][r] += v4.w;
                }
        }
        if (z2) {
#pragma unroll
            for (int g4 = 0; g4 < 4; ++g4)
#pragma unroll
                for (int r = 0; r < 4; ++r) {
                    const float4 v4 = *reinterpret_cast<const float4*>(z2 + rofs[r] * G4 + g4 * H + 4 * c);
                    acc[4 * g4 + 0][r] += v4.x; acc[4 * g4 + 1][r] += v4.y; acc[4 * g4 + 2][r] += v4.z; acc[4 * g4 + 3][r] += v4.w;
                }
        }
    }
    float cp[4][4];
    {
        const float* cpn = a.c_prev + (int64_t)n * a.c_prev_sn;
#pragma unroll
        for (int r = 0; r < 4; ++r) {
            const float4 v4 = *reinterpret_cast<const float4*>(cpn + rofs[r] * H + 4 * c);
            cp[0][r] = v4.x; cp[1][r] = v4.y; cp[2][r] = v4.z; cp[3][r] = v4.w;
        }
    }
    {
        float4* d_ = reinterpret_cast<float4*>(lds + CH_FLOATS) + threadIdx.x;
        d_[0] = tg0; d_[512] = tg1; d_[1024] = tg2; d_[1536] = tg3; d_[2048] = tg4;
    }
    NMARL_STAMP(43)
    NMARL_STAMP(45)
    if (MSG != 0) {
// ... 227 lines not shown
                }
                if (SECOND && CARRY != 0 && xa.mm_next) {
                    const __amdgpu_buffer_rsrc_t rm_ = make_rsrc(xa.mm_next + (int64_t)n * xa.mm_next_sn, (uint32_t)(a.E * xa.mm_next_row * 4));
                    const uint32_t mo = row0 + c < a.E ? (uint32_t)(((row0 + c) * xa.mm_next_row + kc * CH_K + 4 * grp) * 4) : 0xfffffff0u;
                    __builtin_amdgcn_raw_buffer_store_b128(__builtin_bit_cast(u32x4v, m0), rm_, mo, 0, 0);
                    __builtin_amdgcn_raw_buffer_store_b128(__builtin_bit_cast(u32x4v, m1), rm_, mo, 64, 0);
                }
                NMARL_MCHUNK(macc, m_lds, kc, m0, m1)
            }
        }
        if (SECOND) { NMARL_STAMP(53) }
        const float* encn = MSG != 1 ? xa.enc + (int64_t)n * xa.enc_sn : nullptr;
        float* xo = (!SECOND && xa.xm_out) ? xa.xm_out + (int64_t)n * xa.xm_sn : nullptr;
        float* xo2 = (MSG == 3 && xa.xm2_out) ? xa.xm2_out + (int64_t)n * xa.xm2_sn : nullptr;
        const float4 bv = bv4;
#pragma unroll
        for (int r = 0; r < 4; ++r) {
            float4 v = float4{macc[0][r] + bv.x, macc[1][r] + bv.y, macc[2][r] + bv.z, macc[3][r] + bv.w};
            if (MSG != 2) {
                v.x = fmaxf(v.x, 0.0f); v.y = fmaxf(v.y, 0.0f); v.z = fmaxf(v.z, 0.0f); v.w = fmaxf(v.w, 0.0f);
            }
            if (reuse) v = U[r];
            if (SECOND && CARRY != 0 && xa.carry_out)
                __builtin_amdgcn_raw_buffer_store_b128(__builtin_bit_cast(u32x4v, v), make_rsrc(xa.carry_out + (int64_t)n * xa.carry_out_sn, (uint32_t)(a.E * (H * 4))),
                                                       (uint32_t)(((row0 + 4 * grp + r) * H + 4 * c) * 4), 0, 0);
            if (MSG == 3 && xo2 && row0 + 4 * grp + r < a.E)
                *reinterpret_cast<float4*>(xo2 + (row0 + 4 * grp + r) * xa.xm2_row + 4 * c) = v;
            if (MSG != 1) {
                float4 e4;
                if (OBENC && !SECOND && ob_here) {
                    e4 = encv[r];
                } else if (HEAD == 4) {
                    const uint32_t rr_ = row0 + 4 * grp + r < a.E ? (uint32_t)(row0 + 4 * grp + r) : (uint32_t)(a.E - 1);
                    e4 = __builtin_bit_cast(float4, __builtin_amdgcn_raw_buffer_load_b128(make_rsrc(encn, (uint32_t)(a.E * xa.enc_row * 4)),
                                                                                         (rr_ * (uint32_t)xa.enc_row + 4 * c) * 4, 0, 0));
                } else {
                    e4 = *reinterpret_cast<const float4*>(encn + rofs[r] * xa.enc_row + 4 * c);
                }
                v.x += e4.x; v.y += e4.y; v.z += e4.z; v.w += e4.w;
            }
            float* t_ = a_tile + (4 * grp_w + r) * APITCH + 4 * c;
            t_[0] = v.x; t_[1] = v.y; t_[2] = v.z; t_[3] = v.w;
            if (xo && row0 + 4 * grp + r < a.E) *reinterpret_cast<float4*>(xo + (row0 + 4 * grp + r) * xa.xm_row + 4 * c) = v;
        }
        __builtin_amdgcn_fence(__ATOMIC_RELEASE, "wavefront");
        __builtin_amdgcn_wave_barrier();
        __builtin_amdgcn_fence(__ATOMIC_ACQUIRE, "wavefront");
    };
    NMARL_STAMP(48)
    float keepr[4];
#pragma unroll
    for (int r = 0; r < 4; ++r) keepr[r] = 1.0f - a.done[rofs[r]];
    if (MSG != 0) {
        const float* p0_ = nx > 2 ? xrow : hrow;
        a0 = *reinterpret_cast<const float4*>(p0_);
        a1 = *reinterpret_cast<const float4*>(p0_ + 16);
        msg_phase(std::false_type{}, PU, PW);
        if (nx <= 2) {
            const float* t_ = a_tile + c * APITCH + 4 * grp;
            a0.x = t_[0]; a0.y = t_[1]; a0.z = t_[2]; a0.w = t_[3];
            a1.x = t_[16]; a1.y = t_[17]; a1.z = t_[18]; a1.w = t_[19];
        }
    }
    NMARL_STAMP(49)
    if (MSG != 0) {
#pragma unroll
        for (int g4 = 0; g4 < 4; ++g4)
#pragma unroll
            for (int r = 0; r < 4; ++r) {
                acc[4 * g4 + 0][r] = b4s[g4].x; acc[4 * g4 + 1][r] = b4s[g4].y; acc[4 * g4 + 2][r] = b4s[g4].z; acc[4 * g4 + 3][r] = b4s[g4].w;
            }
    }

    constexpr bool ZS_BIAS = HEAD == 4 && MSG == 2;
    f32x4 zs[PV && !ZS_BIAS ? 16 : 1];
    constexpr bool CP_PARK = HEAD == 4 && MSG == 1;
    float4* cp_park = reinterpret_cast<float4*>(m_lds + xa.msg_kc * (CH_K * 64)) + threadIdx.x;
    if (CP_PARK) *cp_park = float4{cp[0][3], cp[1][3], cp[2][3], cp[3][3]};
    NMARL_A_MASK(0, a0, a1)
    const int lag = DEPH ? (wave >> 2) : 0;
    if (DEPH && lag) __builtin_amdgcn_s_setprio(1);
    int bsel = lag ? NBUF - 1 : 0;
    int wsel = 2 % NBUF;
    for (int tau = 0; tau < nch; ++tau) {
        const int ch = tau - lag;
        const int chn = ch + 1 < nch ? ch + 1 : nch - 1;
        NMARL_A_LOAD(chn, n0, n1)
        if (ch >= 0) {
            if (!ZS_BIAS && ((HEAD == 3 && ch == nx) || (HEAD == 4 && ch == nx - 2))) {
#pragma unroll
                for (int t = 0; t < 16; ++t) zs[t] = acc[t];
            }
            NMARL_KCHUNK(lds + bsel * CH_FLOATS, a0, a1)
            if (ENC_LDS && ch < nx && e_out != nullptr && row0 + c < a.E) {
                float* so = e_out + (int64_t)n * e_out_sn + (row0 + c) * e_out_row + 4 * grp + ch * CH_K;
                *reinterpret_cast<float4*>(so) = a0;
                *reinterpret_cast<float4*>(so + 16) = a1;
            }
        }
        NMARL_STAMP(2 + 2 * tau)
        __syncthreads();
        NMARL_STAMP(3 + 2 * tau)
        if (tau + 2 < nch) NMARL_STAGE_STORE(wsel)
        const int chs = tau + 3 < nch ? tau + 3 : nch - 1;
        NMARL_STAGE_LOAD(chs)
        a0 = n0; a1 = n1;
        NMARL_A_MASK(chn, a0, a1)
        bsel = bsel + 1 == NBUF ? 0 : bsel + 1;
        wsel = wsel + 1 == NBUF ? 0 : wsel + 1;
    }
    if (DEPH && lag) {
        if (HEAD == 3 && nch - 1 == nx) {
#pragma unroll
            for (int t = 0; t < 16; ++t) zs[t] = acc[t];
        }
        NMARL_KCHUNK(lds + bsel * CH_FLOATS, a0, a1)
    }
    NMARL_STAMP(20)
    if (CP_PARK) {
        const float4 v = *cp_park;
        cp[0][3] = v.x; cp[1][3] = v.y; cp[2][3] = v.z; cp[3][3] = v.w;
        int l_ = threadIdx.x;
        asm volatile("" : "+v"(l_));
        grp_w = (l_ & 63) >> 4;
    }
    if (nxt_here) {
        float4* d = reinterpret_cast<float4*>(m_lds);
        d[threadIdx.x] = nfa; d[threadIdx.x + 512] = nfb;
    }
    const unsigned epoch = HEAD == 4 ? (unsigned)__builtin_amdgcn_readfirstlane((int)epoch_raw) + 1u : 0u;
    bool early_ok = false;
    unsigned ev_old = 0;
    int ev_act = -1;
    float ev_h[2] = {0.f, 0.f}, ev_v[2] = {0.f, 0.f}, ev_v0[2] = {0.f, 0.f};
    int ev_t[2] = {0, 0}, ev_c[2] = {0, 0};

    float* gn = a.gates ? a.gates + (int64_t)n * a.gates_sn : nullptr;
    float* cn = a.c_new + (int64_t)n * a.c_new_sn;
    float* hn_out = a.h_new + (int64_t)n * a.h_new_sn;
    float hv_[4][4];
    const f32x4 keepv = f32x4{keepr[0], keepr[1], keepr[2], keepr[3]};
#pragma unroll
    for (int jj = 0; jj < 4; ++jj) {
        const f32x4 gi = sigm4(acc[0 + jj]), gf = sigm4(acc[4 + jj]), go = sigm4(acc[8 + jj]), gu = tanh4(acc[12 + jj]);
        const f32x4 cpv = f32x4{cp[jj][0], cp[jj][1], cp[jj][2], cp[jj][3]};
        const f32x4 cv = gf * (cpv * keepv) + gi * gu;
        const f32x4 hv = go * tanh4(cv);
#pragma unroll
        for (int r = 0; r < 4; ++r) {
            if (HEAD != 0) a_tile[(4 * grp_w + r) * APITCH + 4 * c + jj] = hv[r];
            cp[jj][r] = cv[r];
            hv_[jj][r] = hv[r];
        }
        acc[0 + jj] = gi; acc[4 + jj] = gf; acc[8 + jj] = go; acc[12 + jj] = gu;
    }
    {
        if (HEAD == 4) {
            const __amdgpu_buffer_rsrc_t rh_ = make_rsrc(hn_out, (uint32_t)(a.E * (H * 4)));
#pragma unroll
            for (int r = 0; r < 4; ++r) {
                const int64_t row = row0 + 4 * grp + r;
                if (row < a.E)
                    __builtin_amdgcn_raw_buffer_store_b128(__builtin_bit_cast(u32x4v, float4{hv_[0][r], hv_[1][r], hv_[2][r], hv_[3][r]}), rh_,
                                                           (uint32_t)((row * H + 4 * c) * 4), 0, SC1);
            }
            asm volatile("s_waitcnt vmcnt(0)" ::: "memory");
            if (lane == 0 && !(xa.fault && blockIdx.x == 0))
                __hip_atomic_store((gu32*)(xa.sync + 16) + ((n * a.blocks_per_agent + blk_u) * WAVES2 + wave), epoch, __ATOMIC_RELAXED,
                                   __HIP_MEMORY_SCOPE_AGENT);
            NMARL_STAMP(26)
        }
#pragma unroll
        for (int r = 0; r < 4; ++r) {
            const int64_t row = row0 + 4 * grp + r;
            if (row < a.E) {
                *reinterpret_cast<float4*>(cn + row * H + 4 * c) = float4{cp[0][r], cp[1][r], cp[2][r], cp[3][r]};
                const float4 h4 = float4{hv_[0][r], hv_[1][r], hv_[2][r], hv_[3][r]};
                if (HEAD != 4)
                    *reinterpret_cast<float4*>(hn_out + row * H + 4 * c) = h4;
                if (gn) {
#pragma unroll
                    for (int g4 = 0; g4 < 4; ++g4)
                        *reinterpret_cast<float4*>(gn + row * G4 + g4 * H + 4 * c) =
                            float4{acc[4 * g4 + 0][r], acc[4 * g4 + 1][r], acc[4 * g4 + 2][r], acc[4 * g4 + 3][r]};
                }
            }
        }
    }
    NMARL_STAMP(21)
    if (HEAD != 0) {
        __builtin_amdgcn_fence(__ATOMIC_RELEASE, "wavefront");
        __builtin_amdgcn_wave_barrier();
        __builtin_amdgcn_fence(__ATOMIC_ACQUIRE, "wavefront");
        int act_l = -1;
        if (HEAD == 2) head_epilogue<2>(a, n, xa.N, row0, lane, a_tile, hw_lds + H * MAXA + MAXA);
        else act_l = head_policy_lds(a, n, xa.N, row0, lane, a_tile, hw_lds, hw_lds + H * MAXA);
        if (GENV && xa.gv_on && act_l >= 0 && !(xa.fault && blockIdx.x == 0)) {
            typedef __attribute__((address_space(1))) unsigned long long gu64;
            const int hi_ = n >= 13 ? 1 : 0;
            __hip_atomic_fetch_add((gu64*)xa.gv_words + 2 * (row0 + lane) + hi_,
                                   ((unsigned long long)act_l << (3 * (n - 13 * hi_))) | (1ull << 59), __ATOMIC_RELAXED, __HIP_MEMORY_SCOPE_AGENT);
        }
        if (ENC && !EGEN && xa.ev_on) {
            if (act_l >= 0)
                ev_old = __hip_atomic_fetch_add((gu32*)xa.ev_cnt + (row0 + lane), ((unsigned)act_l << (2 * n)) | 0x10000u, __ATOMIC_RELAXED,
                                                __HIP_MEMORY_SCOPE_AGENT);
            ev_act = act_l;
            const int64_t n_lanes = a.E * nmarl_cacc::N;
#pragma unroll
            for (int q = 0; q < 2; ++q) {
                const int64_t gq = row0 * nmarl_cacc::N + q * NMARL_WAVE + lane;
                const int64_t gc = gq < n_lanes ? gq : n_lanes - 1;
                ev_h[q] = xa.ev_h[gc]; ev_v[q] = xa.ev_v[gc];
                ev_t[q] = xa.ev_t[gc >> 3]; ev_c[q] = xa.ev_coll[gc >> 3]; ev_v0[q] = xa.ev_v0[gc >> 3];
            }
        }
    }
    NMARL_STAMP(22)
    if (nxt_here) {
        __syncthreads();
        f32x4 facc[4];
#pragma unroll
        for (int t = 0; t < 4; ++t) facc[t] = f32x4{0.f, 0.f, 0.f, 0.f};
#pragma unroll
        for (int kc = 0; kc < 2; ++kc) {
            const float* t_ = a_tile + c * APITCH + kc * CH_K + 4 * grp;
            const float4 m0 = float4{t_[0], t_[1], t_[2], t_[3]};
            const float4 m1 = float4{t_[16], t_[17], t_[18], t_[19]};
            NMARL_MCHUNK(facc, m_lds, kc, m0, m1)
        }
        float* no = xa.nxt_out + (int64_t)n * xa.nxt_out_sn;
#pragma unroll
        for (int r = 0; r < 4; ++r)
            if (row0 + 4 * grp + r < a.E)
                *reinterpret_cast<float4*>(no + (row0 + 4 * grp + r) * H + 4 * c) =
                    float4{fmaxf(facc[0][r] + nb4.x, 0.0f), fmaxf(facc[1][r] + nb4.y, 0.0f), fmaxf(facc[2][r] + nb4.z, 0.0f),
                           fmaxf(facc[3][r] + nb4.w, 0.0f)};
    }
    if (HEAD == 4) {
        gu32* flags = (gu32*)(xa.sync + 16);
        const int bpa = a.blocks_per_agent, blk = blk_u;
        {
            int jl = -1;
#pragma unroll
            for (int k = 0; k < 8; ++k) jl = lane == k ? nbj[k] : jl;
            const bool watch = lane < xa.m_max && lane < 8 && jl >= 0;
            const unsigned v = __hip_atomic_load(flags + (((watch ? jl : n) * bpa + blk) * WAVES2 + wave), __ATOMIC_RELAXED, __HIP_MEMORY_SCOPE_AGENT);
            const bool up = __ballot(watch && v != epoch) == 0ull;
            early_ok = up;
            NMARL_NOTE(54, up ? 1 : 2)
            asm volatile("" ::: "memory");
            msg_load(std::true_type{}, K0{}, PU, PW);
        }
        NMARL_STAMP(31)
    }
    if (PV) {
        if (ZS_BIAS) {
            const float* bn = a.bias + (int64_t)n * a.bias_sn;
#pragma unroll
            for (int g4 = 0; g4 < 4; ++g4) {
                const float4 b4 = *reinterpret_cast<const float4*>(bn + g4 * H + 4 * c);
#pragma unroll
                for (int r = 0; r < 4; ++r) { acc[4 * g4 + 0][r] = b4.x; acc[4 * g4 + 1][r] = b4.y; acc[4 * g4 + 2][r] = b4.z; acc[4 * g4 + 3][r] = b4.w; }
            }
        } else {
#pragma unroll
            for (int t = 0; t < 16; ++t) acc[t] = zs[t];
        }
#pragma unroll
        for (int hc = 0; hc < 2; ++hc) {
            const float* ar = a_tile + c * APITCH + hc * CH_K + 4 * grp;
            float4 r0, r1;
            r0.x = ar[0] * keepA; r0.y = ar[1] * keepA; r0.z = ar[2] * keepA; r0.w = ar[3] * keepA;
            r1.x = ar[16] * keepA; r1.y = ar[17] * keepA; r1.z = ar[18] * keepA; r1.w = ar[19] * keepA;
            NMARL_KCHUNK(lds + ((nx + hc) % NBUF) * CH_FLOATS, r0, r1)
        }
        NMARL_STAMP(23)
        __builtin_amdgcn_wave_barrier();
        if (HEAD == 4) {
            gu32* flags = (gu32*)(xa.sync + 16);
            const int bpa = a.blocks_per_agent, blk = blk_u;
            bool give_up = false;
            if (!early_ok) {
#pragma unroll
                for (int k = 0; k < 8; ++k) {
                    const int j = nbj[k];
                    if (k >= xa.m_max || j < 0 || give_up) continue;
                    gu32* f = flags + ((j * bpa + blk) * WAVES2 + wave);
                    for (unsigned spins = 0;; ++spins) {
                        const unsigned v = __builtin_amdgcn_readfirstlane(__hip_atomic_load(f, __ATOMIC_RELAXED, __HIP_MEMORY_SCOPE_AGENT));
                        if (v == epoch) break;
                        if (spins > xa.max_spins) {
                            if (lane == 0) {
                                __hip_atomic_store((gu32*)xa.sync + 2, 1u, __ATOMIC_RELAXED, __HIP_MEMORY_SCOPE_AGENT);
                                if (xa.status) __hip_atomic_store((gu32*)xa.status, 1u, __ATOMIC_RELAXED, __HIP_MEMORY_SCOPE_AGENT);
                            }
                            give_up = true;
                            break;
                        }
                        __builtin_amdgcn_s_sleep(2);
                    }
                }
                asm volatile("" ::: "memory");
                msg_load(std::true_type{}, K0{}, PU, PW);
            }
            NMARL_STAMP(27)
            NMARL_STAGE_LOAD(nx - 2)
            {
                const float4* g_ = img + (int64_t)(nx - 1) * (CH_FLOATS / 4) + threadIdx.x;
                tg0 = g_[0]; tg1 = g_[512]; tg2 = g_[1024]; tg3 = g_[1536]; tg4 = g_[2048];
            }
            msg_phase(std::true_type{}, PU, PW);
            NMARL_STAMP(28)
            __syncthreads();
            NMARL_STAGE_STORE(0)
            {
                float4* d_ = reinterpret_cast<float4*>(lds + CH_FLOATS) + threadIdx.x;
                d_[0] = tg0; d_[512] = tg1; d_[1024] = tg2; d_[1536] = tg3; d_[2048] = tg4;
            }
            __syncthreads();
            NMARL_STAMP(29)
#pragma unroll
            for (int mc = 0; mc < 2; ++mc) {
                const float* buf = lds + mc * CH_FLOATS + (4 * grp * 16 + c) * 20;
                const float* ar = a_tile + c * APITCH + mc * CH_K + 4 * grp;
                float4 r0, r1;
                r0.x = ar[0]; r0.y = ar[1]; r0.z = ar[2]; r0.w = ar[3];
                r1.x = ar[16]; r1.y = ar[17]; r1.z = ar[18]; r1.w = ar[19];
                NMARL_CHUNK(buf, r0, r1)
            }
            NMARL_STAMP(30)
            __builtin_amdgcn_wave_barrier();
        }
#pragma unroll
        for (int jj = 0; jj < 4; ++jj) {
            const f32x4 gi = sigm4(acc[0 + jj]), gf = sigm4(acc[4 + jj]), go = sigm4(acc[8 + jj]), gu = tanh4(acc[12 + jj]);
            const f32x4 cpv = f32x4{cp[jj][0], cp[jj][1], cp[jj][2], cp[jj][3]};
            const f32x4 cv = gf * (cpv * keepv) + gi * gu;
            const f32x4 hv = go * tanh4(cv);
#pragma unroll
            for (int r = 0; r < 4; ++r) a_tile[(4 * grp_w + r) * APITCH + 4 * c + jj] = hv[r];
        }
        NMARL_STAMP(33)
        __builtin_amdgcn_fence(__ATOMIC_RELEASE, "wavefront");
        __builtin_amdgcn_wave_barrier();
        __builtin_amdgcn_fence(__ATOMIC_ACQUIRE, "wavefront");
        NMARL_STAMP(24)
        head_epilogue<3>(a, n, xa.N, row0, lane, a_tile, hw_lds + H * MAXA + MAXA);
        NMARL_STAMP(25)
        if (ENC && !EGEN && xa.ev_on) {
            const bool last_l = ev_act >= 0 && (ev_old >> 16) == (unsigned)(xa.N - 1);
            const unsigned pay_l = (ev_old | ((unsigned)(ev_act < 0 ? 0 : ev_act) << (2 * n))) & 0xffffu;
            if (last_l) xa.ev_cnt[row0 + lane] = 0u;
            unsigned long long todo = __ballot(last_l);
            while (todo) {
                int rsel = -1;
#pragma unroll
                for (int k = 0; k < 8; ++k) {
                    const int rk = todo ? (int)__builtin_ctzll(todo) : -1;
                    todo = todo ? (todo & (todo - 1)) : 0ull;
                    rsel = (lane >> 3) == k ? rk : rsel;
                }
                const bool valid = rsel >= 0;
                const int rr = valid ? rsel : 0;
                const int av = lane & 7;
                const int q = rr * nmarl_cacc::N + av;
                const unsigned pay = (unsigned)__shfl((int)pay_l, rr, NMARL_WAVE);
                const float h0 = __shfl(ev_h[0], q & 63, NMARL_WAVE), h1 = __shfl(ev_h[1], q & 63, NMARL_WAVE);
                const float v0 = __shfl(ev_v[0], q & 63, NMARL_WAVE), v1 = __shfl(ev_v[1], q & 63, NMARL_WAVE);
                const float w0 = __shfl(ev_v0[0], q & 63, NMARL_WAVE), w1 = __shfl(ev_v0[1], q & 63, NMARL_WAVE);
                const int t0 = __shfl(ev_t[0], q & 63, NMARL_WAVE), t1 = __shfl(ev_t[1], q & 63, NMARL_WAVE);
                const int c0 = __shfl(ev_c[0], q & 63, NMARL_WAVE), c1 = __shfl(ev_c[1], q & 63, NMARL_WAVE);
                const bool hi = q >= NMARL_WAVE;
                int64_t e = row0 + rr;
                e = e < a.E ? e : a.E - 1;
                nmarl_cacc::cacc_step_group(xa.ev_p, e, av, valid, hi ? h1 : h0, hi ? v1 : v0, (int)((pay >> (2 * av)) & 3u), hi ? t1 : t0,
                                            (hi ? c1 : c0) != 0, hi ? w1 : w0, xa.ev_h, xa.ev_v, xa.ev_u, xa.ev_t, xa.ev_coll, xa.ev_v0,
                                            xa.ev_obs, xa.ev_rew, xa.ev_done, xa.ev_grew, xa.ev_auto_reset, xa.ev_seed, xa.ev_base,
                                            xa.ev_episode);
            }
            NMARL_STAMP(39)
        }
        if (HEAD == 4) {
            __syncthreads();
            if (threadIdx.x == 0) {
                gu32* sy = (gu32*)xa.sync;
                const unsigned old = __hip_atomic_fetch_add(sy + 1, 1u, __ATOMIC_RELAXED, __HIP_MEMORY_SCOPE_AGENT);
                if (old == n_lstm - 1) {
                    __hip_atomic_store(sy + 1, 0u, __ATOMIC_RELAXED, __HIP_MEMORY_SCOPE_AGENT);
                    __hip_atomic_store(sy, epoch, __ATOMIC_RELAXED, __HIP_MEMORY_SCOPE_AGENT);
                }
            }
        }
    }
#undef NMARL_MCHUNK
#undef NMARL_MSTEP
#undef NMARL_STAGE_LOAD
#undef NMARL_STAGE_STORE
#undef NMARL_A_LOAD
#undef NMARL_A_MASK
#undef NMARL_KCHUNK
}

__global__ void lstm_wimage_kernel(const int N, const int KX, const float* wx, const int64_t wx_sn, const float* wh,
                                   const int64_t wh_sn, float* img, const int64_t img_sn) {
    const int per_agent = (KX + H) * 320;
    const int64_t i = (int64_t)blockIdx.x * blockDim.x + threadIdx.x;
    if (i >= (int64_t)N * per_agent) return;
    const int n = (int)(i / per_agent), o = (int)(i % per_agent);
    const int k = o / 320, cc = (o % 320) / 20, t = o % 20;
    float v = 0.0f;
    const int col = (t >> 2) * H + 4 * cc + (t & 3);
    if (t < 16) v = k < KX ? wx[(int64_t)n * wx_sn + (int64_t)k * G4 + col] : wh[(int64_t)n * wh_sn + (int64_t)(k - KX) * G4 + col];
    img[(int64_t)n * img_sn + o] = v;
}

__global__ void lstm_wimage_bf16x3_kernel(const int N, const int KX, const float* wx, const int64_t wx_sn, const float* wh,
                                          const int64_t wh_sn, unsigned* img, const int64_t img_sn) {
    const int per_agent = (KX + H) * 320;
    const int64_t i = (int64_t)blockIdx.x * blockDim.x + threadIdx.x;
    if (i >= (int64_t)N * per_agent) return;
    const int n = (int)(i / per_agent), o = (int)(i % per_agent);
    const int ch = o / CH_FLOATS, r = o % CH_FLOATS;
    const int gc = r / X3_PITCH, q = r % X3_PITCH;
    unsigned v = 0u;
    if (gc < 64 && q < 128) {
        const int grp = gc >> 4, cc = gc & 15, t = q >> 3, hl = (q >> 2) & 1, jp = q & 3;
        const int col = (t >> 2) * H + 4 * cc + (t & 3);
#pragma unroll
        for (int e = 0; e < 2; ++e) {
            const int j = 2 * jp + e;
            const int k = ch * CH_K + (j < 4 ? 4 * grp + j : 16 + 4 * grp + j - 4);
            const float w = k < KX ? wx[(int64_t)n * wx_sn + (int64_t)k * G4 + col] : wh[(int64_t)n * wh_sn + (int64_t)(k - KX) * G4 + col];
            const __bf16 hb = (__bf16)w;
            const __bf16 b = hl ? (__bf16)(w - (float)hb) : hb;
            v |= (unsigned)__builtin_bit_cast(unsigned short, b) << (16 * e);
        }
    }
    img[(int64_t)n * img_sn + o] = v;
}

__global__ void lstm_msg_wimage_kernel(const int N, const int K, const float* w, const int64_t w_sn, float* img,
                                       const int64_t img_sn) {
    const int per_agent = K * 64;
    const int64_t i = (int64_t)blockIdx.x * blockDim.x + threadIdx.x;
    if (i >= (int64_t)N * per_agent) return;
    const int n = (int)(i / per_agent), o = (int)(i % per_agent);
    const int k = o / 64, cc = (o % 64) / 4, t = o % 4;
    img[(int64_t)n * img_sn + o] = w[(int64_t)n * w_sn + (int64_t)k * 64 + 4 * cc + t];
}

inline bool stride_ok(int64_t s, int64_t need) { return s >= need && (s % 4) == 0; }

}

extern "C" int nmarl_lstm_wimage_floats(int32_t KX) { return (KX + H) * 320; }

extern "C" int nmarl_lstm_step_sync_words(int64_t E, int32_t N) {
    return (int)(16 + (int64_t)N * ((E + ROWS_B - 1) / ROWS_B) * WAVES2);
}

extern "C" int nmarl_lstm_wimage(int32_t N, int32_t KX, const float* wx, int64_t wx_sn, const float* wh, int64_t wh_sn,
                                 float* img, int64_t img_sn, int32_t precision, void* stream) {
    if (N <= 0 || KX < 0 || KX > MAX_KX || KX % CH_K || !wh || !img || (KX > 0 && !wx) || img_sn < (int64_t)(KX + H) * 320 ||
        (img_sn % 4) || ((uintptr_t)img % 16) || wh_sn < H * G4 || (KX > 0 && wx_sn < (int64_t)KX * G4) || precision < 0 || precision > 1)
        return NMARL_EINVAL;
    const int64_t total = (int64_t)N * (KX + H) * 320;
    const dim3 grid((unsigned)((total + 255) / 256));
    hipStream_t st = static_cast<hipStream_t>(stream);
    if (precision)
        hipLaunchKernelGGL(lstm_wimage_bf16x3_kernel, grid, dim3(256), 0, st, N, KX, wx, wx_sn, wh, wh_sn, reinterpret_cast<unsigned*>(img), img_sn);
    else
        hipLaunchKernelGGL(lstm_wimage_kernel, grid, dim3(256), 0, st, N, KX, wx, wx_sn, wh, wh_sn, img, img_sn);
    return nmarl_check_launch();
}

extern "C" int nmarl_lstm_msg_wimage(int32_t N, int32_t K, const float* w_msg, int64_t w_sn, float* img, int64_t img_sn,
                                     void* stream) {
    if (N <= 0 || K <= 0 || K % CH_K || K > 256 || !w_msg || !img || w_sn < (int64_t)K * 64 || img_sn < (int64_t)K * 64 ||
        (img_sn % 4) || ((uintptr_t)img % 16))
        return NMARL_EINVAL;
    const int64_t total = (int64_t)N * K * 64;
    hipLaunchKernelGGL(lstm_msg_wimage_kernel, dim3((unsigned)((total + 255) / 256)), dim3(256), 0, static_cast<hipStream_t>(stream),
                       N, K, w_msg, w_sn, img, img_sn);
    return nmarl_check_launch();
// ... 21 lines not shown
    while (v > 0 && !g_fault_in.compare_exchange_weak(v, v - 1)) {}
    return v == 1;
}

NMARL_INTERNAL int nmarl_bptt_coupled_occupancy(int K);
NMARL_INTERNAL int nmarl_bptt_dial_occupancy(int K);

extern "C" int nmarl_handoff_capacity(int32_t which, int32_t K) {
    const int cus = nmarl_handoff_cus();
    if (cus < 0 || K <= 0) return -1;
    int per_cu = 0;
    if (which == 1) {
        if (K % CH_K || K > 128) return -1;
        const size_t lb = (size_t)(LDSX_FLOATS + K * 64 + (K == H ? H * 64 : 0)) * sizeof(float) + (K == H ? 0 : 512 * sizeof(float4));
        const int lb_max = (int)((LDSX_FLOATS + CH_FLOATS) * sizeof(float));
        static std::atomic<int> cache[64][2];
        int dev = 0;
        if (hipGetDevice(&dev) != hipSuccess) return -1;
        const int kd = K == H ? 1 : 0;
        const int hit = (dev >= 0 && dev < 64) ? cache[dev][kd].load() : 0;
        if (hit > 0) {
            per_cu = hit - 1;
        } else {
            const void* fn = K == H ? reinterpret_cast<const void*>(lstm_step_x_kernel<4, 2>) : reinterpret_cast<const void*>(lstm_step_x_kernel<4, 1>);
            hipError_t rc = hipFuncSetAttribute(fn, hipFuncAttributeMaxDynamicSharedMemorySize, lb_max);
            if (rc == hipSuccess)
                rc = K == H ? hipOccupancyMaxActiveBlocksPerMultiprocessor(&per_cu, lstm_step_x_kernel<4, 2>, 512, lb)
                            : hipOccupancyMaxActiveBlocksPerMultiprocessor(&per_cu, lstm_step_x_kernel<4, 1>, 512, lb);
            if (rc != hipSuccess) return -1;
            if (dev >= 0 && dev < 64) cache[dev][kd].store(per_cu + 1);
        }
    } else if (which == 2) {
        per_cu = nmarl_bptt_coupled_occupancy(K);
        if (per_cu < 0) return -1;
    } else if (which == 3) {
        per_cu = nmarl_bptt_dial_occupancy(K);
        if (per_cu < 0) return -1;
    } else {
        return -1;
    }
    return per_cu * cus;
}

extern "C" int nmarl_lstm_step_grid_env_blocks(int64_t E, int32_t N);

extern "C" int nmarl_lstm_step_x(const nmarl_step_x_t* s, void* stream) {
    if (!s) return NMARL_EINVAL;
    const int64_t E = s->E;
    const int32_t N = s->N, KX = s->KX, KX2 = s->KX2, prec = s->precision;
    const float *x = s->x, *x2 = s->x2, *h_in = s->h_in, *img = s->img, *bias = s->bias, *zadd1 = s->zadd1, *zadd2 = s->zadd2,
                *c_prev = s->c_prev, *done = s->done;
    float *gates = s->gates, *c_new = s->c_new, *h_new = s->h_new;
    const int64_t x_sn = s->x_sn, x_row = s->x_row, x2_sn = s->x2_sn, x2_row = s->x2_row, h_sn = s->h_sn, img_sn = s->img_sn,
                  bias_sn = s->bias_sn, zadd1_sn = s->zadd1_sn, zadd2_sn = s->zadd2_sn, c_prev_sn = s->c_prev_sn, gates_sn = s->gates_sn,
                  c_new_sn = s->c_new_sn, h_new_sn = s->h_new_sn;
    const nmarl_head_t* head = s->head;
    const nmarl_msg_t* msg = s->msg;
    const nmarl_step_enc_t* enc = s->enc;
    const nmarl_grid_env_t* genv = s->genv;
    const int mk = msg ? msg->kind : 0;
    const int kind = head ? head->kind : 0;
    if ((msg && (mk == 0 || kind == 0 || zadd1 || zadd2)) || ((enc || genv) && kind != 3) || (enc && (mk > 1 || (mk == 1) != !!x)) ||
        (genv && mk != 2) || prec < 0 || prec > 1 || (prec && (msg || genv)))
        return NMARL_EINVAL;
    const int KM = mk ? H : 0;
    if (s->H != H || E < 0 || N <= 0 || KX < 0 || KX > MAX_KX || KX % CH_K || KX2 < 0 || KX2 > KX || KX2 % CH_K || mk < 0 || mk > 3 ||
        (mk && (KX2 != 0 || KX < H)) ||
        (E > 0 && (!h_in || !img || !bias || !c_prev || !done || !c_new || !h_new || (KX - KX2 - KM > 0 && !x && (!enc || mk)) || (KX2 > 0 && !x2))))
        return NMARL_EINVAL;
    if (mk && E > 0) {
        if (msg->m_max <= 0 || msg->m_max > 8 || !msg->nbr_idx || !msg->img || !msg->b || msg->b_sn < H ||
            msg->K != (mk == 2 ? H : H * msg->m_max) || msg->K > ((mk == 1 && (kind == 1 || kind == 2)) ? 256 : 128) || msg->img_sn < (int64_t)msg->K * 64 || (msg->img_sn % 4) ||
            ((uintptr_t)msg->img % 16) || ((uintptr_t)msg->b % 16) || (msg->b_sn % 4) ||
            (mk != 1 && (!msg->enc || msg->enc_row < H || msg->enc_sn < E * msg->enc_row || ((uintptr_t)msg->enc % 16) ||
                         (msg->enc_row % 4) || (msg->enc_sn % 4))) ||
            (msg->out && (msg->out_row < H || msg->out_sn < E * msg->out_row || ((uintptr_t)msg->out % 16) || (msg->out_row % 4) ||
                          (msg->out_sn % 4))) ||
            (mk == 3 && (KX != H || !msg->src || msg->src_sn < E * (int64_t)H || (msg->src_sn % 4) || ((uintptr_t)msg->src % 16) ||
                         (msg->out2 && (msg->out2_row < H || msg->out2_sn < E * msg->out2_row || ((uintptr_t)msg->out2 % 16) ||
                                        (msg->out2_row % 4) || (msg->out2_sn % 4))))))
            return NMARL_EINVAL;
    }
    if (kind < 0 || kind > 3 || (mk == 3 && kind == 3)) return NMARL_EINVAL;
    if (kind != 0 && E > 0) {
        if (head->A <= 0 || head->A > MAXA || !head->w || !head->b || head->b_sn < (kind == 2 ? 1 : head->A)) return NMARL_EINVAL;
        if ((kind == 1 || kind == 3) && (head->w_sn < (int64_t)H * head->A || !head->pi_out || head->pi_sn < E * head->A || !head->act_out ||
                          head->mode < 0 || head->mode > 2 || (head->mode == 0 && !head->u)))
            return NMARL_EINVAL;
        if (kind == 3 && (!head->w2 || !head->b2 || head->w2_sn < H || head->b2_sn < 1 || !head->v_out || head->v_sn < E))
            return NMARL_EINVAL;
        if (kind == 2 && (head->m_max < 0 || head->w_sn < H + (int64_t)head->m_max * head->A || !head->v_out || head->v_sn < E ||
                          (head->m_max > 0 && (!head->act_in || !head->nbr_idx))))
            return NMARL_EINVAL;
    }
    if (E == 0) return NMARL_OK;
    if (!stride_ok(h_sn, E * H) || !stride_ok(bias_sn, G4) || (zadd1 && !stride_ok(zadd1_sn, E * G4)) ||
        (zadd2 && !stride_ok(zadd2_sn, E * G4)) || !stride_ok(c_prev_sn, E * H) || !stride_ok(c_new_sn, E * H) ||
        !stride_ok(h_new_sn, E * H) || (gates && !stride_ok(gates_sn, E * G4)) || ((uintptr_t)h_in % 16) || ((uintptr_t)img % 16) ||
        ((uintptr_t)c_new % 16) || ((uintptr_t)h_new % 16) || (gates && ((uintptr_t)gates % 16)) ||
        ((uintptr_t)bias % 16) || ((uintptr_t)c_prev % 16) || (zadd1 && ((uintptr_t)zadd1 % 16)) || (zadd2 && ((uintptr_t)zadd2 % 16)) ||
        img_sn < (int64_t)(KX + H) * 320 || (img_sn % 4) ||
        (KX - KX2 - KM > 0 && (!enc || mk) && (x_row < KX - KX2 - KM || (x_row % 4) || (x_sn % 4) || ((uintptr_t)x % 16))) ||
        (KX2 > 0 && (x2_row < KX2 || (x2_row % 4) || (x2_sn % 4) || ((uintptr_t)x2 % 16))))
        return NMARL_EINVAL;
    XArgs xa{};
    FusedArgs& a = xa.f;
    a.h_in = h_in; a.bias = bias; a.zadd1 = zadd1; a.zadd2 = zadd2; a.c_prev = c_prev; a.done = done;
    a.gates = gates; a.c_new = c_new; a.h_new = h_new;
    a.h_sn = h_sn; a.bias_sn = bias_sn; a.zadd1_sn = zadd1_sn; a.zadd2_sn = zadd2_sn;
    a.c_prev_sn = c_prev_sn; a.gates_sn = gates_sn; a.c_new_sn = c_new_sn; a.h_new_sn = h_new_sn;
    a.E = E;
    a.blocks_per_agent = (int)((E + ROWS_B - 1) / ROWS_B);
    if (kind != 0) a.hd = *head;
    xa.x = (KX - KX2 - KM > 0 && (!enc || mk)) ? x : nullptr; xa.x_sn = x_sn; xa.x_row = x_row;
    xa.x2 = KX2 > 0 ? x2 : nullptr; xa.x2_sn = x2_sn; xa.x2_row = x2_row;
    xa.img = img; xa.img_sn = img_sn;
    xa.nx = KX / CH_K; xa.nx1 = (KX - KX2) / CH_K; xa.N = N;
    if (mk) {
        xa.msg_kc = msg->K / CH_K; xa.m_max = msg->m_max; xa.nbr_idx = msg->nbr_idx; xa.msg_img = msg->img;
        xa.msg_img_sn = msg->img_sn; xa.msg_b = msg->b; xa.msg_b_sn = msg->b_sn; xa.enc = msg->enc; xa.enc_sn = msg->enc_sn;
        xa.enc_row = msg->enc_row; xa.xm_out = msg->out; xa.xm_sn = msg->out_sn; xa.xm_row = msg->out_row;
        if (mk == 2 && msg->mean_out) {
            if (msg->mean_out_row < H || msg->mean_out_sn < E * msg->mean_out_row || ((uintptr_t)msg->mean_out % 16) || (msg->mean_out_row % 4) ||
                (msg->mean_out_sn % 4))
                return NMARL_EINVAL;
            xa.mm_out = msg->mean_out; xa.mm_sn = msg->mean_out_sn; xa.mm_row = msg->mean_out_row;
        }
        if (msg->carry_in || msg->carry_out || msg->mean_next) {
            if (kind != 3 || mk == 3 || (msg->carry_in && (msg->carry_in_sn < E * (int64_t)H || (msg->carry_in_sn % 4) || ((uintptr_t)msg->carry_in % 16))) ||
                (msg->carry_out && (msg->carry_out_sn < E * (int64_t)H || (msg->carry_out_sn % 4) || ((uintptr_t)msg->carry_out % 16))) ||
                (msg->mean_next && (mk != 2 || msg->mean_next_row < H || msg->mean_next_sn < E * msg->mean_next_row || ((uintptr_t)msg->mean_next % 16) ||
                                    (msg->mean_next_row % 4) || (msg->mean_next_sn % 4))))
                return NMARL_EINVAL;
            xa.carry_in = msg->carry_in; xa.carry_in_sn = msg->carry_in_sn; xa.carry_out = msg->carry_out; xa.carry_out_sn = msg->carry_out_sn;
            xa.mm_next = msg->mean_next; xa.mm_next_sn = msg->mean_next_sn; xa.mm_next_row = msg->mean_next_row;
        }
        if (mk == 3) {
            xa.src = msg->src; xa.src_sn = msg->src_sn; xa.xm2_out = msg->out2; xa.xm2_sn = msg->out2_sn; xa.xm2_row = msg->out2_row;
            if (msg->next_out) {
                if (kind != 1 || !msg->next_img || !msg->next_b || msg->next_img_sn < H * 64 || (msg->next_img_sn % 4) ||
                    ((uintptr_t)msg->next_img % 16) || msg->next_b_sn < H || (msg->next_b_sn % 4) || ((uintptr_t)msg->next_b % 16) ||
                    msg->next_out_sn < E * (int64_t)H || (msg->next_out_sn % 4) || ((uintptr_t)msg->next_out % 16))
                    return NMARL_EINVAL;
                xa.nxt_img = msg->next_img; xa.nxt_img_sn = msg->next_img_sn; xa.nxt_b = msg->next_b; xa.nxt_b_sn = msg->next_b_sn;
                xa.nxt_out = msg->next_out; xa.nxt_out_sn = msg->next_out_sn;
            }
        }
    }
    static NmarlPerDeviceOnce lds_once;
    const int lb_max = (int)((LDSX_FLOATS + CH_FLOATS) * sizeof(float));
    const size_t lb = (size_t)(LDSX_FLOATS + (mk ? (msg->K < 128 ? msg->K : 128) * 64 : CH_FLOATS)) * sizeof(float);
    if (const unsigned long long lds_bit = lds_once.pending(); lds_bit != ~0ull) {
#define NMARL_SET_LDS(k) \
        if (hipFuncSetAttribute(reinterpret_cast<const void*>(k), hipFuncAttributeMaxDynamicSharedMemorySize, lb_max) != hipSuccess) return NMARL_EHIP;
        NMARL_SET_LDS((lstm_step_x_kernel<0, 0>)) NMARL_SET_LDS((lstm_step_x_kernel<1, 0>)) NMARL_SET_LDS((lstm_step_x_kernel<2, 0>))
        NMARL_SET_LDS((lstm_step_x_kernel<3, 0>)) NMARL_SET_LDS((lstm_step_x_kernel<1, 1>)) NMARL_SET_LDS((lstm_step_x_kernel<2, 1>))
        NMARL_SET_LDS((lstm_step_x_kernel<1, 2>)) NMARL_SET_LDS((lstm_step_x_kernel<2, 2>))
        NMARL_SET_LDS((lstm_step_x_kernel<1, 3>)) NMARL_SET_LDS((lstm_step_x_kernel<2, 3>))
        NMARL_SET_LDS((lstm_step_x_kernel<4, 1>)) NMARL_SET_LDS((lstm_step_x_kernel<4, 2>)) NMARL_SET_LDS((lstm_step_x_kernel<4, 1, 1>))
        NMARL_SET_LDS((lstm_step_x_kernel<4, 1, 0, 1>)) NMARL_SET_LDS((lstm_step_x_kernel<4, 2, 0, 1>)) NMARL_SET_LDS((lstm_step_x_kernel<4, 1, 1, 1>))
        NMARL_SET_LDS((lstm_step_x_kernel<4, 1, 0, 2>)) NMARL_SET_LDS((lstm_step_x_kernel<4, 2, 0, 2>)) NMARL_SET_LDS((lstm_step_x_kernel<4, 1, 1, 2>))
        NMARL_SET_LDS((lstm_step_x_kernel<0, 0, 0, 0, 1>)) NMARL_SET_LDS((lstm_step_x_kernel<1, 0, 0, 0, 1>))
        NMARL_SET_LDS((lstm_step_x_kernel<2, 0, 0, 0, 1>)) NMARL_SET_LDS((lstm_step_x_kernel<3, 0, 0, 0, 1>))
#undef NMARL_SET_LDS
        lds_once.done(lds_bit);
    }
    dim3 grid(a.blocks_per_agent * N);
    if (enc && enc->F != 5) {
        const bool single = !enc->w_fp;
        const int F = enc->F, A = enc->A, mm = enc->m_max;
        if (mk != 0 || prec || enc->env || F <= 0 || (F % 4) || mm < 0 || mm > 4 || F * (1 + mm) > H || N > 32 ||
            KX != (single ? H : 2 * H) || KX2 != 0 || zadd1 || zadd2 ||
            (!single && (A <= 0 || A > MAXA || mm < 1 || A * mm > 32)))
            return NMARL_EINVAL;
        const int ob_rows = F * (1 + mm), fp_rows = single ? 0 : A * mm;
        if (!enc->ob || !enc->w_ob || !enc->b_ob || enc->ob_row < (int64_t)N * F || enc->w_ob_sn < (int64_t)ob_rows * H || enc->b_ob_sn < H ||
            (enc->b_ob_sn % 4) || ((uintptr_t)enc->b_ob % 16) ||
            (!single && (!enc->fp || !enc->b_fp || enc->fp_sn < E * A || enc->w_fp_sn < (int64_t)fp_rows * H || enc->b_fp_sn < H ||
                         (enc->b_fp_sn % 4) || ((uintptr_t)enc->b_fp % 16))) ||
            (enc->out && (((uintptr_t)enc->out % 16) || enc->out_row < (single ? H : 2 * H) || (enc->out_row % 4) || (enc->out_sn % 4) ||
                          enc->out_sn < E * enc->out_row)) ||
            (enc->relu_bits && (single || ((uintptr_t)enc->relu_bits % 4) || enc->relu_bits_sn < E * 4)))
            return NMARL_EINVAL;
        for (int i = 0; i < N * mm; ++i)
            if (enc->nbr[i] < -1 || enc->nbr[i] >= N) return NMARL_EINVAL;
        xa.e_ob = enc->ob; xa.e_ob_row = enc->ob_row; xa.e_fp = enc->fp; xa.e_fp_sn = enc->fp_sn;
        xa.e_wob = enc->w_ob; xa.e_bob = enc->b_ob; xa.e_wfp = enc->w_fp; xa.e_bfp = enc->b_fp;
        xa.e_wob_sn = enc->w_ob_sn; xa.e_bob_sn = enc->b_ob_sn; xa.e_wfp_sn = enc->w_fp_sn; xa.e_bfp_sn = enc->b_fp_sn;
        xa.e_out = enc->out; xa.e_out_sn = enc->out_sn; xa.e_out_row = enc->out_row;
        xa.e_bits = enc->relu_bits; xa.e_bits_sn = enc->relu_bits_sn;
        for (int i = 0; i < 64; ++i) {
            unsigned w = 0;
            for (int k = 0; k < 4; ++k) w |= (unsigned)((i < N && k < mm ? enc->nbr[i * mm + k] : -1) & 255) << (8 * k);
            xa.e_nbr[i] = (int)w;
        }
        xa.ob_F = F; xa.e_ob_rows = ob_rows | (fp_rows << 8) | ((single ? 1 : A) << 16);
        const size_t lb_g = (size_t)(2 * CH_FLOATS + HW_FLOATS + 8 * 512 * 4 + 6 * 64 * 4 + 2 * H) * sizeof(float);
        static NmarlPerDeviceOnce gen_once;
        if (const unsigned long long bit = gen_once.pending(); bit != ~0ull) {
            if (hipFuncSetAttribute(reinterpret_cast<const void*>(lstm_step_x_kernel<3, 0, 3>), hipFuncAttributeMaxDynamicSharedMemorySize,
                                    (int)lb_g) != hipSuccess ||
                hipFuncSetAttribute(reinterpret_cast<const void*>(lstm_step_x_kernel<3, 0, 4>), hipFuncAttributeMaxDynamicSharedMemorySize,
                                    (int)lb_g) != hipSuccess)
                return NMARL_EHIP;
            gen_once.done(bit);
        }
        hipStream_t st = static_cast<hipStream_t>(stream);
        if (single) hipLaunchKernelGGL((lstm_step_x_kernel<3, 0, 4>), grid, dim3(512), lb_g, st, xa);
        else hipLaunchKernelGGL((lstm_step_x_kernel<3, 0, 3>), grid, dim3(512), lb_g, st, xa);
        return nmarl_check_launch();
    }
    if (enc) {
        const bool coupled = mk == 1 && kind == 3;
        const bool single = !enc->w_fp;
        const int ob_rows = 5 * (1 + enc->m_max);
        if ((mk != 0 && !coupled) || KX != (coupled ? 3 * H : single ? H : 2 * H) || KX2 != 0 || zadd1 || zadd2 || N > 32 || enc->F != 5 ||
            (coupled && single) || (single ? (enc->m_max != 0 && enc->m_max != 2) : (enc->A != 4 || enc->m_max != 2)) ||
            !enc->ob || !enc->w_ob || !enc->b_ob || enc->ob_row < (int64_t)N * 5 || enc->w_ob_sn < (int64_t)ob_rows * H || enc->b_ob_sn < H ||
            (enc->b_ob_sn % 4) || ((uintptr_t)enc->b_ob % 16) ||
            (!single && (!enc->fp || !enc->b_fp || enc->fp_sn < E * 4 || enc->w_fp_sn < 8 * H || enc->b_fp_sn < H || (enc->b_fp_sn % 4) ||
                         ((uintptr_t)enc->b_fp % 16))) ||
            (enc->out && (((uintptr_t)enc->out % 16) || enc->out_row < (single ? H : 2 * H) || (enc->out_row % 4) || (enc->out_sn % 4) ||
                          enc->out_sn < E * enc->out_row)) ||
            (coupled && enc->out && (enc->out != x || enc->out_sn != x_sn || enc->out_row != x_row)))
            return NMARL_EINVAL;
        for (int i = 0; i < 2 * N; ++i)
            if (enc->nbr[i] < -1 || enc->nbr[i] >= N) return NMARL_EINVAL;
        xa.e_ob = enc->ob; xa.e_ob_row = enc->ob_row; xa.e_fp = enc->fp; xa.e_fp_sn = enc->fp_sn;
        xa.e_wob = enc->w_ob; xa.e_bob = enc->b_ob; xa.e_wfp = enc->w_fp; xa.e_bfp = enc->b_fp;
        xa.e_wob_sn = enc->w_ob_sn; xa.e_bob_sn = enc->b_ob_sn; xa.e_wfp_sn = enc->w_fp_sn; xa.e_bfp_sn = enc->b_fp_sn;
        xa.e_out = enc->out; xa.e_out_sn = enc->out_sn; xa.e_out_row = enc->out_row;
        if (coupled) { xa.e_out = const_cast<float*>(x); xa.e_out_sn = x_sn; xa.e_out_row = x_row; }
        if (enc->relu_bits && (((uintptr_t)enc->relu_bits % 4) || enc->relu_bits_sn < E * 4)) return NMARL_EINVAL;
        xa.e_bits = enc->relu_bits; xa.e_bits_sn = enc->relu_bits_sn;
        for (int i = 0; i < 64; ++i) xa.e_nbr[i] = (i < 2 * N && enc->m_max == 2) ? enc->nbr[i] : -1;
        xa.e_ob_rows = ob_rows;
        if (single && enc->relu_bits) return NMARL_EINVAL;
        if (enc->env) {
            const nmarl_cacc_params_t* p = enc->env;
            if (N != NMARL_CACC_N || head->A > 4 || !p->compact_obs || p->T <= 0 || p->batch_size <= 0 || (p->scenario != 0 && p->scenario != 1) || p->dt <= 0.f ||
                p->h_g <= p->h_s || p->u_max == 0.f || p->v_star == 0.f || p->h_star == 0.f || !enc->h || !enc->v || !enc->u || !enc->t ||
                !enc->collided || !enc->v0_init || !enc->obs_out || !enc->reward || !enc->done || !enc->global_reward ||
                !enc->cnt || ((uintptr_t)enc->cnt % 4) || ((uintptr_t)enc->obs_out % 16) || (enc->auto_reset && !enc->episode) ||
                head->act_out == nullptr)
                return NMARL_EINVAL;
            xa.ev_on = 1; xa.ev_auto_reset = enc->auto_reset ? 1 : 0; xa.ev_p = *p;
            xa.ev_h = enc->h; xa.ev_v = enc->v; xa.ev_u = enc->u; xa.ev_t = enc->t; xa.ev_coll = enc->collided; xa.ev_v0 = enc->v0_init;
            xa.ev_obs = enc->obs_out; xa.ev_rew = enc->reward; xa.ev_done = enc->done; xa.ev_grew = enc->global_reward;
            xa.ev_seed = enc->seed; xa.ev_base = enc->env_id_base; xa.ev_episode = enc->episode;
            xa.ev_cnt = enc->cnt;
        }
        if (!coupled) {
            static NmarlPerDeviceOnce enc_once;
            const size_t lb_e = (size_t)(2 * CH_FLOATS + HW_FLOATS + 8 * 512 * 4 + 6 * 64 * 4 + 2 * H) * sizeof(float);
            if (const unsigned long long bit = enc_once.pending(); bit != ~0ull) {
                if (hipFuncSetAttribute(reinterpret_cast<const void*>(lstm_step_x_kernel<3, 0, 1>), hipFuncAttributeMaxDynamicSharedMemorySize,
                                        (int)lb_e) != hipSuccess ||
                    hipFuncSetAttribute(reinterpret_cast<const void*>(lstm_step_x_kernel<3, 0, 2>), hipFuncAttributeMaxDynamicSharedMemorySize,
                                        (int)lb_e) != hipSuccess ||
                    hipFuncSetAttribute(reinterpret_cast<const void*>(lstm_step_x_kernel<3, 0, 1, 0, 1>), hipFuncAttributeMaxDynamicSharedMemorySize,
                                        (int)lb_e) != hipSuccess ||
                    hipFuncSetAttribute(reinterpret_cast<const void*>(lstm_step_x_kernel<3, 0, 2, 0, 1>), hipFuncAttributeMaxDynamicSharedMemorySize,
                                        (int)lb_e) != hipSuccess)
                    return NMARL_EHIP;
                enc_once.done(bit);
            }
            hipStream_t st = static_cast<hipStream_t>(stream);
            if (prec) {
                if (single) hipLaunchKernelGGL((lstm_step_x_kernel<3, 0, 2, 0, 1>), grid, dim3(512), lb_e, st, xa);
                else hipLaunchKernelGGL((lstm_step_x_kernel<3, 0, 1, 0, 1>), grid, dim3(512), lb_e, st, xa);
            } else if (single) hipLaunchKernelGGL((lstm_step_x_kernel<3, 0, 2>), grid, dim3(512), lb_e, st, xa);
            else hipLaunchKernelGGL((lstm_step_x_kernel<3, 0, 1>), grid, dim3(512), lb_e, st, xa);
            return nmarl_check_launch();
        }
    }
    if (mk && kind == 3) {
        const int cap = nmarl_handoff_capacity(1, msg->K);
        if (cap < 0) return NMARL_EHIP;
        if (!msg->sync || ((uintptr_t)msg->sync % 4) || ((uintptr_t)msg->status % 4) || (int)grid.x > cap ||
            E * (int64_t)(H * 4) >= (int64_t)1 << 32 || (mk == 2 && (KX != H || E * msg->enc_row * 4 >= (int64_t)1 << 32)))
            return NMARL_EINVAL;
        xa.sync = msg->sync;
        xa.status = msg->status;
        xa.fault = nmarl_handoff_take_fault() ? 1 : 0;
        xa.max_spins = xa.fault ? NMARL_HANDOFF_FAULT_SPINS : NMARL_HANDOFF_MAX_SPINS;
        if (genv) {
            const nmarl_grid_params_t* gp = genv->params;
            const int env_blocks = nmarl_lstm_step_grid_env_blocks(E, N);
            if (!gp || env_blocks <= 0 || N != NMARL_GRID_N || head->A > 7 || !msg->ob || !gp->compact_obs || gp->objective != 0 || gp->T <= 0 ||
                gp->norm_wave <= 0.f || !genv->q || !genv->transit || !genv->prev_action || !genv->t || !genv->xi || !genv->obs_out ||
                !genv->reward || !genv->done || !genv->global_reward || !genv->words || ((uintptr_t)genv->words % 8) ||
                ((uintptr_t)genv->obs_out % 16) || ((uintptr_t)genv->q % 16) || ((uintptr_t)genv->transit % 16) ||
                (genv->auto_reset && !genv->episode) || !msg->status)
                return NMARL_EINVAL;
            xa.gv_on = 1; xa.gv_lstm_blocks = (int)grid.x; xa.gv_auto_reset = genv->auto_reset ? 1 : 0; xa.gv_p = *gp;
            xa.gv_q = genv->q; xa.gv_tr = genv->transit; xa.gv_prev = genv->prev_action; xa.gv_t = genv->t; xa.gv_xi = genv->xi;
            xa.gv_obs = genv->obs_out; xa.gv_rew = genv->reward; xa.gv_done = genv->done; xa.gv_grew = genv->global_reward;
            xa.gv_seed = genv->seed; xa.gv_base = genv->env_id_base; xa.gv_episode = genv->episode;
            xa.gv_words = reinterpret_cast<unsigned long long*>(genv->words);
            grid = dim3(grid.x + env_blocks);
        }
    }
    size_t lb_extra = 0;
    if (msg && msg->ob) {
        if (mk != 2 || kind != 3 || msg->ob_F <= 0 || (msg->ob_F % 4) || msg->ob_segs != msg->m_max + 1 || msg->ob_F * msg->ob_segs > H ||
            !msg->ob_nbr || !msg->ob_img || !msg->ob_b || ((uintptr_t)msg->ob % 16) || (msg->ob_row % 4) ||
            msg->ob_row < (int64_t)N * msg->ob_F || ((uintptr_t)msg->ob_img % 16) || msg->ob_img_sn < H * 64 || (msg->ob_img_sn % 4) ||
            ((uintptr_t)msg->ob_b % 16) || (msg->ob_b_sn % 4) || msg->ob_b_sn < H)
            return NMARL_EINVAL;
        xa.ob = msg->ob; xa.ob_row = msg->ob_row; xa.ob_F = msg->ob_F; xa.ob_segs = msg->ob_segs; xa.ob_nbr = msg->ob_nbr;
        xa.ob_img = msg->ob_img; xa.ob_img_sn = msg->ob_img_sn; xa.ob_b = msg->ob_b; xa.ob_b_sn = msg->ob_b_sn;
        lb_extra = (size_t)H * 64 * sizeof(float);
    }
    if (mk == 1 || mk == 2) {
        const int64_t span = E * (int64_t)H;
        for (int i = 0; i < N; ++i)
            for (int j = 0; j < N; ++j) {
                const float* a0 = h_in + i * h_sn;
                const float* b0 = h_new + j * h_new_sn;
                if (a0 < b0 + span && b0 < a0 + span) return NMARL_EINVAL;
            }
    }
    hipStream_t st = static_cast<hipStream_t>(stream);
    if (mk == 1 && kind == 3) lb_extra += 512 * sizeof(float4);
#define NMARL_LX(HD, MS)                                                                                                         \
    if (prec) hipLaunchKernelGGL((lstm_step_x_kernel<HD, 0, 0, 0, 1>), grid, dim3(512), lb + lb_extra, st, xa);                 \
    else hipLaunchKernelGGL((lstm_step_x_kernel<HD, MS>), grid, dim3(512), lb + lb_extra, st, xa)
    const int carry = !msg ? 0 : msg->carry_in ? 2 : (msg->carry_out || msg->mean_next) ? 1 : 0;
#define NMARL_LC(MS, EN)                                                                                                         \
    if (carry == 2) hipLaunchKernelGGL((lstm_step_x_kernel<4, MS, EN, 2>), grid, dim3(512), lb + lb_extra, st, xa);              \
    else if (carry == 1) hipLaunchKernelGGL((lstm_step_x_kernel<4, MS, EN, 1>), grid, dim3(512), lb + lb_extra, st, xa);         \
    else hipLaunchKernelGGL((lstm_step_x_kernel<4, MS, EN, 0>), grid, dim3(512), lb + lb_extra, st, xa);
    if (mk == 0) {
        if (kind == 0) NMARL_LX(0, 0); else if (kind == 1) NMARL_LX(1, 0); else if (kind == 2) NMARL_LX(2, 0); else NMARL_LX(3, 0);
    } else if (mk == 1) {
        if (kind == 1) NMARL_LX(1, 1); else if (kind == 2) NMARL_LX(2, 1);
        else if (enc) { NMARL_LC(1, 1) }
        else { NMARL_LC(1, 0) }
    } else if (mk == 2) {
        if (kind == 1) NMARL_LX(1, 2); else if (kind == 2) NMARL_LX(2, 2); else { NMARL_LC(2, 0) }
    } else {
        if (kind == 1) NMARL_LX(1, 3); else NMARL_LX(2, 3);
    }
#undef NMARL_LX
#undef NMARL_LC
    return nmarl_check_launch();
}

extern "C" int nmarl_lstm_step_grid_env_blocks(int64_t E, int32_t N) {
    if (E <= 0 || N <= 0) return 0;
    const int cap = nmarl_handoff_capacity(1, H);
    const int64_t lstm = (int64_t)N * ((E + ROWS_B - 1) / ROWS_B), groups = (E + 15) / 16;
    if (cap <= 0 || lstm >= cap) return 0;
    const int64_t room = cap - lstm;
    return (int)(room < groups ? room : groups);
}

extern "C" int nmarl_lstm_step_grid_words(int64_t E) { return E <= 0 ? 0 : (int)(2 * E); }

extern "C" int nmarl_lstm_step_env_words(int64_t E) { return E <= 0 ? 0 : (int)((E + 63) / 64 * 64); }

#ifdef NMARL_STEP_TIMELINE
extern "C" int nmarl_timeline_set(unsigned long long* p, void* stream) {
    hipLaunchKernelGGL(timeline_set_kernel, dim3(1), dim3(1), 0, static_cast<hipStream_t>(stream), p);
    return nmarl_check_launch();
}
#endif
```

deeprl_network_amd/ops.py:

```python
import ctypes as C
import os

import numpy as np
import torch

from . import _lib
from ._lib import check, lib, ptr, stream

F32 = torch.float32


_handoff_status = {}
_handoff_off = [False]


def handoff_status(device):
    dev = torch.device(device)
    if dev.index is None:
        dev = torch.device('cuda', torch.cuda.current_device())
    if dev not in _handoff_status:
        _handoff_status[dev] = torch.zeros(4, dtype=torch.int32, device=dev)
    return _handoff_status[dev]


# ... 136 lines not shown


def _bias(bias):
    if bias.stride(1) != 1:
        raise _lib.NmarlError('bias rows must be contiguous')
    return ptr(bias, F32, strided=True), bias.stride(0)


def cell_fwd(z, bias, c_prev, done, gates, c_new, h_new, z2=None):
    N, E, H4 = z.shape
    check(lib.nmarl_lstm_cell_fwd(E, N, H4 // 4, *_pn(z), *_pn(z2), *_bias(bias), *_pn(c_prev), ptr(done, F32),
                                  *_pn(gates), *_pn(c_new), *_pn(h_new), stream()), 'nmarl_lstm_cell_fwd')


FUSED_H = 64


XSIDE_MAX_K = 256


def xside_supported(kx, n_h):
    return n_h == FUSED_H and kx % 32 == 0 and 0 <= kx <= XSIDE_MAX_K


PRECISIONS = ('fp32', 'bf16x3')


def check_precision(precision, what='precision'):
    if precision not in PRECISIONS:
        raise ValueError('%s: %r is not one of %s' % (what, precision, ', '.join(PRECISIONS)))
    return precision


def lstm_wimage(wx, wh, out=None, precision='fp32'):
    check_precision(precision, 'lstm_wimage')
    N = wh.shape[0]
    KX = 0 if wx is None else wx.shape[1]
    n = lib.nmarl_lstm_wimage_floats(KX)
    x3 = precision == 'bf16x3'
    dt, width = (torch.bfloat16, 2 * n) if x3 else (F32, n)
    if out is None:
        out = torch.empty(N, width, dtype=dt, device=wh.device)
    if out.shape != (N, width) or out.stride(1) != 1 or out.stride(0) % (2 if x3 else 1):
        raise _lib.NmarlError('lstm_wimage: out must be [%d, %d] %s with rows of whole words' % (N, width, dt))
    if wh.stride(2) != 1 or wh.stride(1) != wh.shape[2] or (wx is not None and (wx.stride(2) != 1 or wx.stride(1) != wx.shape[2])):
        raise _lib.NmarlError('lstm_wimage: weights need contiguous per-agent panels')
    check(lib.nmarl_lstm_wimage(N, KX, ptr(wx, F32, strided=True), 0 if wx is None else wx.stride(0), ptr(wh, F32, strided=True),
                                wh.stride(0), ptr(out, dt), out.stride(0) // (2 if x3 else 1), 1 if x3 else 0, stream()),
          'nmarl_lstm_wimage')
    return out


def _img_arg(img, N, KX, precision, what):
    n = lib.nmarl_lstm_wimage_floats(KX)
    if precision == 'bf16x3':
        if img.dtype != torch.bfloat16 or img.shape != (N, 2 * n) or img.stride(0) % 2:
            raise _lib.NmarlError('%s: bf16x3 needs the split image lstm_wimage(..., precision="bf16x3") of KX = %d' % (what, KX))
        return ptr(img, torch.bfloat16), img.stride(0) // 2
    if img.dtype != F32 or img.shape != (N, n):
        raise _lib.NmarlError('%s: weight image does not match KX = %d (fp32)' % (what, KX))
    return ptr(img, F32), img.stride(0)


MSG_GATHER_RELU, MSG_MEAN_ADD, MSG_DIAL = 1, 2, 3
MSG_MAX_K = 128
MSG_KIND_MAX_K = {MSG_GATHER_RELU: 256, MSG_MEAN_ADD: 64, MSG_DIAL: 128}


def msg_supported(kind, m_max, n_h):
    return n_h == FUSED_H and m_max <= 8 and (n_h if kind == MSG_MEAN_ADD else n_h * m_max) <= MSG_KIND_MAX_K.get(kind, 0)


def lstm_msg_wimage(w_msg, out=None):
    N, K, J = w_msg.shape
    if out is None:
        out = torch.empty(N, K * J, dtype=F32, device=w_msg.device)
    if J != FC_J or w_msg.stride(2) != 1 or w_msg.stride(1) != J:
        raise _lib.NmarlError('lstm_msg_wimage: w_msg must be [N,K,64] with contiguous panels')
    check(lib.nmarl_lstm_msg_wimage(N, K, ptr(w_msg, F32, strided=True), w_msg.stride(0), ptr(out, F32), out.stride(0), stream()),
          'nmarl_lstm_msg_wimage')
    return out


def _step_x(h, bias, zadd1, zadd2, c_prev, done, gates, c_out, h_out, xs, head, what, precision='fp32'):
    N, E, H = h.shape
    x, _, img = xs[:3]
    x2 = xs[3] if len(xs) > 3 else None
    msg = xs[4] if len(xs) > 4 else None
    x3 = check_precision(precision, what) == 'bf16x3'
    if x3 and msg is not None:
        raise _lib.NmarlError('%s: bf16x3 exists for the uncoupled nets\' step forms only (no message term); coupled nets are fp32-only' % what)
    a = _lib.StepX(E=E, N=N, H=H, precision=1 if x3 else 0)
    a.h_in, a.h_sn = _pn(h)
    a.bias, a.bias_sn = _bias(bias)
    a.zadd1, a.zadd1_sn = _pn(zadd1)
    a.zadd2, a.zadd2_sn = _pn(zadd2)
    a.c_prev, a.c_prev_sn = _pn(c_prev)
    a.done = ptr(done, F32)
    a.gates, a.gates_sn = _pn(gates)
    a.c_new, a.c_new_sn = _pn(c_out)
    a.h_new, a.h_new_sn = _pn(h_out)
    if head is not None:
        a.head = C.pointer(head)
    if isinstance(x, dict):
        if head is None or head.kind != 3 or x2 is not None or msg is not None or zadd1 is not None or zadd2 is not None:
            raise _lib.NmarlError('%s: the in-kernel encoders need the policy + value step of an uncoupled net' % what)
        a.KX = FC_J if x.get('w_fp') is None else 2 * FC_J
        a.enc = C.pointer(_step_enc(x, N, E))
    else:
        K1, K2 = (0 if t is None else t.shape[2] for t in (x, x2))
        if x is not None:
            a.x, a.x_sn, a.x_row = _rows_view(x, K1, what + ' x')
        if x2 is not None:
            a.x2, a.x2_sn, a.x2_row = _rows_view(x2, K2, what + ' x2')
        a.KX, a.KX2 = K1 + K2 + (H if msg is not None else 0), K2
    a.img, a.img_sn = _img_arg(img, N, a.KX, precision, what)
    if msg is not None:
        if head is None or x2 is not None or zadd1 is not None or zadd2 is not None:
            raise _lib.NmarlError('%s: the in-kernel message term needs a head and excludes x2 / addends' % what)
        m = _lib.Msg()
        nbr_idx = msg['nbr_idx']
        m.kind, m.m_max, m.K = msg['kind'], nbr_idx.shape[1], msg['w_msg'].shape[1]
        m.nbr_idx = ptr(nbr_idx, torch.int32)
        m.img, m.img_sn = ptr(msg['img'], F32), msg['img'].stride(0)
        m.b, m.b_sn = _bias(msg['b_msg'])
        if msg.get('enc') is not None:
            m.enc, m.enc_sn, m.enc_row = _rows_view(msg['enc'], H, what + ' enc')
        if msg.get('out') is not None:
            m.out, m.out_sn, m.out_row = _rows_view(msg['out'], H, what + ' msg out')
        if msg.get('mean_out') is not None:
            m.mean_out, m.mean_out_sn, m.mean_out_row = _rows_view(msg['mean_out'], H, what + ' msg mean_out')
        for key in ('carry_in', 'carry_out'):
            cb = msg.get(key)
            if cb is not None:
                if cb.shape != (N, E, H) or cb.stride(2) != 1 or cb.stride(1) != H:
                    raise _lib.NmarlError('%s: msg["%s"] must be [N,E,64] with contiguous panels' % (what, key))
                setattr(m, key, ptr(cb, F32, strided=True))
                setattr(m, key + '_sn', cb.stride(0))
        if msg.get('mean_next') is not None:
            m.mean_next, m.mean_next_sn, m.mean_next_row = _rows_view(msg['mean_next'], H, what + ' msg mean_next')
        if msg['kind'] == MSG_DIAL:
            src = msg['src']
            if src.shape != (N, E, H) or src.stride(2) != 1 or src.stride(1) != H:
                raise _lib.NmarlError('%s: msg["src"] must be [N,E,64] with contiguous panels' % what)
            m.src, m.src_sn = ptr(src, F32, strided=True), src.stride(0)
            if msg.get('out2') is not None:
                m.out2, m.out2_sn, m.out2_row = _rows_view(msg['out2'], H, what + ' msg out2')
            nxt = msg.get('next')
            if nxt is not None:
                m.next_img, m.next_img_sn = ptr(nxt['img'], F32), nxt['img'].stride(0)
                m.next_b, m.next_b_sn = _bias(nxt['b'])
                m.next_out, m.next_out_sn = _pn(nxt['out'])
        ob = msg.get('ob')
        if ob is not None:
            x_ob = ob['x']
            if head.kind != 3 or msg['kind'] != MSG_MEAN_ADD or x_ob.dim() != 3 or x_ob.shape[:2] != (E, N) or not x_ob.is_contiguous():
                raise _lib.NmarlError('%s: the in-kernel observation encoder needs the one-launch lstm_ic3 step and a compact [E,N,F] slab' % what)
            m.ob, m.ob_row, m.ob_F, m.ob_segs = ptr(x_ob, F32), N * x_ob.shape[2], x_ob.shape[2], ob['nbr'].shape[1]
            m.ob_nbr = ptr(ob['nbr'], torch.int32)
            m.ob_img, m.ob_img_sn = ptr(ob['img'], F32), ob['img'].stride(0)
            m.ob_b, m.ob_b_sn = _bias(ob['b'])
        if head.kind == 3:
            sync = msg.get('sync')
            if sync is None or sync.dtype != torch.int32 or sync.numel() < lib.nmarl_lstm_step_sync_words(E, N):
                raise _lib.NmarlError('%s: head kind 3 with a message term needs msg["sync"] (step_sync_words)' % what)
            m.sync = ptr(sync, torch.int32)
            m.status = ptr(handoff_status(h.device), torch.int32)
        spec = msg.get('enc_spec')
        if spec is not None:
            if head.kind != 3 or msg['kind'] != MSG_GATHER_RELU or x is None:
                raise _lib.NmarlError('%s: the in-kernel encoders of a coupled net need lstm_comm\'s policy + value step and its x slot' % what)
            a.enc = C.pointer(_step_enc(dict(spec, out=None), N, E))
        genv = msg.get('genv')
        if genv is not None:
            if head.kind != 3 or msg['kind'] != MSG_MEAN_ADD or ob is None:
                raise _lib.NmarlError('%s: the in-launch grid env step needs lstm_ic3\'s one-launch step with its observation encoder inside' % what)
            g = _lib.GridEnv()
            g.params = C.pointer(genv['params'])
            for k in ('q', 'transit', 'xi', 'obs_out', 'reward', 'global_reward'):
                setattr(g, k, ptr(genv[k], F32))
            g.prev_action, g.done = ptr(genv['prev_action'], torch.uint8), ptr(genv['done'], torch.uint8)
            g.t, g.episode = ptr(genv['t'], torch.int32), ptr(genv['episode'], torch.int32)
            g.auto_reset, g.seed, g.env_id_base = (1 if genv['auto_reset'] else 0), int(genv['seed']), int(genv['env_id_base'])
            if genv['words'].dtype != torch.int64 or genv['words'].numel() < lib.nmarl_lstm_step_grid_words(E):
                raise _lib.NmarlError('%s: genv["words"] must hold nmarl_lstm_step_grid_words(E) 64-bit words' % what)
            g.words = ptr(genv['words'], torch.int64)
            a.genv = C.pointer(g)
        a.msg = C.pointer(m)
    check(lib.nmarl_lstm_step_x(C.byref(a), stream()), what)


STEP_ENC_MAX_OB, STEP_ENC_MAX_FP, STEP_ENC_MAX_M, STEP_ENC_MAX_N = 64, 32, 4, 32


def step_enc_cacc_layout(n_feat):
    return n_feat == 5


def _step_enc_ob_fits(n_feat, m_max):
# ... 98 lines not shown
        e.cnt = ptr(step_env_scratch(N, E, ob.device), torch.int32)
        e._keep = ev['params']
    return e


def ob_encoder_supported(n_feat, n_obs, n_h):
    return n_h == FUSED_H and n_feat % 4 == 0 and n_obs <= FC_J


def lstm_ob_wimage(w_ob, pad, out=None):
    with torch.no_grad():
        pad[:, :w_ob.shape[1]].copy_(w_ob)
    return lstm_msg_wimage(pad, out=out)


def step_grid_env_blocks(N, E):
    return int(lib.nmarl_lstm_step_grid_env_blocks(E, N)) if handoff_enabled() else 0


def step_sync_words(N, E, device):
    return torch.zeros(lib.nmarl_lstm_step_sync_words(E, N), dtype=torch.int32, device=device)


def step_handoff_supported(N, E, device, K=128):
    if not handoff_enabled() or torch.device(device).type != 'cuda':
        return False
    cap = lib.nmarl_handoff_capacity(1, int(K))
    if cap < 0:
        raise _lib.NmarlError('nmarl_handoff_capacity failed')
    return N * ((E + 127) // 128) <= cap


def _xs_or_image(xs, wh):
    return xs if xs is not None else (None, None, lstm_wimage(None, wh))


def lstm_step_fused(h, wh, bias, zadd1, zadd2, c_prev, done, gates, c_out, h_out, xs=None, precision='fp32'):
    _step_x(h, bias, zadd1, zadd2, c_prev, done, gates, c_out, h_out, _xs_or_image(xs, wh), None, 'nmarl_lstm_step_x', precision)
    return h_out, c_out


HEAD_MAX_A = 8


def _head_param(w, what):
    if w.stride(2) != 1 or (w.shape[1] > 1 and w.stride(1) != w.shape[2]):
        raise _lib.NmarlError('%s: head weights need contiguous per-agent panels' % what)
    return ptr(w, F32, strided=True), w.stride(0)


def lstm_step_policy(h, wh, bias, zadd1, zadd2, c_prev, done, c_out, h_out, pi_w, pi_b, pi_out, act_out, mode,
                     u=None, seed=0, env_id_base=0, step=0, step_dev=None, xs=None, gates=None, precision='fp32'):
    A = pi_w.shape[2]
    hd = _lib.Head()
    hd.kind, hd.A, hd.mode = 1, A, mode
    hd.w, hd.w_sn = _head_param(pi_w, 'lstm_step_policy')
    hd.b, hd.b_sn = _bias(pi_b)
    hd.pi_out, hd.pi_sn = _pn(pi_out)
    hd.act_out, hd.u = ptr(act_out, torch.uint8), ptr(u, F32)
    hd.seed, hd.env_id_base, hd.step, hd.step_dev = seed, env_id_base, int(step), ptr(step_dev, torch.int64)
    _step_x(h, bias, zadd1, zadd2, c_prev, done, gates, c_out, h_out, _xs_or_image(xs, wh), hd, 'nmarl_lstm_step_x[p]', precision)
    return pi_out, act_out


def lstm_step_value(h, wh, bias, zadd1, zadd2, c_prev, done, c_out, h_out, v_w, v_b, action, nbr_idx, n_a, v_out, xs=None,
                    precision='fp32'):
    N, E, H = h.shape
    hd = _lib.Head()
    hd.kind, hd.A, hd.m_max = 2, n_a, nbr_idx.shape[1]
    if v_w.shape[1] != H + nbr_idx.shape[1] * n_a or v_w.shape[2] != 1:
        raise _lib.NmarlError('lstm_step_value: v_w must be [N,H+m_max*A,1]')
    hd.w, hd.w_sn = _head_param(v_w, 'lstm_step_value')
    hd.b, hd.b_sn = _bias(v_b)
    hd.act_in, hd.nbr_idx = ptr(action, torch.uint8), ptr(nbr_idx, torch.int32)
    if v_out.dim() != 2 or v_out.stride(1) != 1:
        raise _lib.NmarlError('lstm_step_value: v_out must be [N,E] with unit column stride')
    hd.v_out, hd.v_sn = ptr(v_out, F32, strided=True), v_out.stride(0)
    _step_x(h, bias, zadd1, zadd2, c_prev, done, None, c_out, h_out, _xs_or_image(xs, wh), hd, 'nmarl_lstm_step_x[v]', precision)
    return v_out


def lstm_step_policy_value(h, wh, bias, zadd1, zadd2, c, done, pi_w, pi_b, pi_out, act_out, v_w, v_b, nbr_idx, n_a,
                           v_out, mode, u=None, seed=0, env_id_base=0, step=0, step_dev=None, xs=None, h_out=None,
                           c_out=None, gates=None, defer_action_term=False, precision='fp32'):
    N, E, H = h.shape
    hd = _lib.Head()
    hd.kind, hd.A, hd.mode = 3, pi_w.shape[2], mode
    hd.w, hd.w_sn = _head_param(pi_w, 'lstm_step_policy_value')
    hd.b, hd.b_sn = _bias(pi_b)
    hd.pi_out, hd.pi_sn = _pn(pi_out)
    hd.act_out, hd.u = ptr(act_out, torch.uint8), ptr(u, F32)
    hd.seed, hd.env_id_base, hd.step, hd.step_dev = seed, env_id_base, int(step), ptr(step_dev, torch.int64)
    hd.w2, hd.w2_sn = _head_param(v_w, 'lstm_step_policy_value')
    hd.b2, hd.b2_sn = _bias(v_b)
    if v_out.shape != (N, E) or v_out.stride(1) != 1 or (N > 1 and v_out.stride(0) < E):
        raise _lib.NmarlError('lstm_step_policy_value: v_out must be [N,E] with unit column stride')
    hd.v_out, hd.v_sn = ptr(v_out, F32, strided=True), v_out.stride(0)
    h_out, c_out = (h if h_out is None else h_out), (c if c_out is None else c_out)
    _step_x(h, bias, zadd1, zadd2, c, done, gates, c_out, h_out, _xs_or_image(xs, wh), hd, 'nmarl_lstm_step_x[pv]', precision)
    if not defer_action_term:
        if not v_out.is_contiguous():
            raise _lib.NmarlError('lstm_step_policy_value: the neighbour-action add needs a contiguous v_out')
        nbr_action_value(act_out, nbr_idx, v_w[:, H:], n_a, out=v_out, accumulate=True)
    return pi_out, act_out, v_out


BIAS_NONE, BIAS_RELU, BIAS_TANH = 0, 1, 2


def bias_act_(x, bias, act, out=None):
    N, rows, W = x.shape
    xp, xs = _pn(x)
    bp, bs = _bias(bias)
    if out is None:
        yp, ys, yrow = xp, xs, W
    else:
        if out.stride(2) != 1 or out.shape != x.shape:
            raise _lib.NmarlError('bias_act_: out must be [N,rows,W] with unit column stride')
        yp, ys, yrow = ptr(out, F32, strided=True), out.stride(0), out.stride(1)
    check(lib.nmarl_bias_act(rows, N, W, xp, xs, bp, bs, act, yp, ys, yrow, stream()), 'nmarl_bias_act')
    return x if out is None else out


FC_MAX_F, FC_J = 64, 64


def _rows_view(t, W, what):
    if t.dim() != 3 or t.shape[2] != W or t.stride(2) != 1:
        raise _lib.NmarlError('%s: expected [N,rows,%d] with unit column stride, got %s / %s' % (what, W, tuple(t.shape), t.stride()))
    return ptr(t, F32, strided=True), t.stride(0), t.stride(1)


def fc_supported(x, w):
    return x.shape[2] <= FC_MAX_F and w.shape[2] == FC_J


def fc_fwd(x, w, b, act, out=None):
    N, rows, F = x.shape
    if out is None:
        out = torch.empty(N, rows, FC_J, dtype=F32, device=x.device)
    xp, xs, xr = _rows_view(x, F, 'fc_fwd x')
    yp, ys, yr = _rows_view(out, FC_J, 'fc_fwd out')
    wp, ws = _head_param(w, 'fc_fwd')
    check(lib.nmarl_fc_fwd(rows, N, F, w.shape[2], xp, xs, xr, wp, ws, *_bias(b), act, yp, ys, yr, stream()), 'nmarl_fc_fwd')
    return out


def onehot_argmax_add_(y, p, scale=None):
    N, rows, W = y.shape
    pp, p_sn = _pn(p)
    yp, ys, yr = _rows_view(y, W, 'onehot_argmax_add_ y')
    check(lib.nmarl_onehot_argmax_add(rows, N, p.shape[2], W, pp, p_sn, None if scale is None else ptr(scale, F32), yp, ys, yr, stream()),
          'nmarl_onehot_argmax_add')
    return y


def fc_fwd_multi(parts, act, out=None):
    N, rows = parts[0][0].shape[:2]
    n = len(parts)
    if out is None:
        out = torch.empty(N, rows, FC_J * n, dtype=F32, device=parts[0][0].device)
    arr = (_lib.FcPart * n)()
    for i, (x, w, b, nbr_idx) in enumerate(parts):
        pt = arr[i]
        pt.x, pt.x_sn, pt.x_row = _rows_view(x, x.shape[2], 'fc_fwd_multi x')
        if nbr_idx is None:
            pt.F = x.shape[2]
        else:
            pt.gather_A, pt.m_max, pt.F = x.shape[2], nbr_idx.shape[1], x.shape[2] * nbr_idx.shape[1]
            pt.nbr_idx = ptr(nbr_idx, torch.int32)
        if w.shape[1] != pt.F or w.shape[2] != FC_J:
            raise _lib.NmarlError('fc_fwd_multi: layer %d weight shape %s does not match input width %d' % (i, tuple(w.shape), pt.F))
        pt.w, pt.w_sn = _head_param(w, 'fc_fwd_multi')
        pt.b, pt.b_sn = _bias(b)
    yp, ys, yr = _rows_view(out, FC_J * n, 'fc_fwd_multi out')
    check(lib.nmarl_fc_fwd_multi(rows, N, n, arr, act, yp, ys, yr, stream()), 'nmarl_fc_fwd_multi')
    return out


def fc_bwd(x, y, dy, act, nbr_idx=None):
    N, rows = y.shape[:2]
    F = x.shape[2] if nbr_idx is None else x.shape[2] * nbr_idx.shape[1]
# ... 1013 lines not shown
```

deeprl_network_amd/utils.py:

```python
import glob
import logging
import os
import shutil
import time

import numpy as np
import pandas as pd
import torch

from . import ops, train_record


check_dir = os.path.exists


def copy_file(src, dst_dir):
    shutil.copy(src, dst_dir)


def find_file(cur_dir, suffix='.ini'):
    hits = sorted(glob.glob(os.path.join(cur_dir, '*' + suffix)))
    if not hits:
        logging.error('Cannot find %s file' % suffix)
        return None
# ... 272 lines not shown
        env, model = self.env, self.model
        T = self.n_step
        model.t = 0
        if self.handoff_guard:
            ops.copy_multi(zip(self._shadow, self._shadow_tensors()), skip_if=self._status[:1])
        fused = self.fused_encode
        for t in range(T):
            outs = dict(obs_out=model.buf_x[t + 1], reward_out=self.buf_rraw[t], done_out=model.buf_done_post[t], greward_out=self.buf_g[t])
            if self.env_in_kernel:
                model.act(self.done_pre if t == 0 else self.zero_done, mode=ops.SAMPLE_PHILOX, seed=env.seed,
                          env_id_base=env.env_id_base, step=t, step_dev=self.step_dev, done_is_zero=(t > 0),
                          env_step=env.inkernel_step(auto_reset=(t == T - 1), **outs))
                model.t = t + 1
                continue
            action = model.act(self.done_pre if t == 0 else self.zero_done, mode=ops.SAMPLE_PHILOX, seed=env.seed,
                               env_id_base=env.env_id_base, step=t, step_dev=self.step_dev, done_is_zero=(t > 0),
                               pre_encoded=fused and t > 0)
            enc = model.policy.fused_env_encode(model.buf_fp[t + 1], model.encode_target(t + 1)) if fused else None
            env.step(action, auto_reset=(t == T - 1), obs_out=model.buf_x[t + 1], reward_out=self.buf_rraw[t],
                     done_out=model.buf_done_post[t], greward_out=self.buf_g[t], **({'encode': enc} if fused else {}))
            model.t = t + 1
        v = model.bootstrap(self.zero_done, self.action_boot, mode=ops.SAMPLE_PHILOX, seed=env.seed,
                            env_id_base=env.env_id_base, step=T, step_dev=self.step_dev, done_is_zero=True, pre_encoded=fused)
        self.step_dev.add_(T + 1)
        torch.mul(v, (1.0 - self.last_done.to(torch.float32)).view(1, -1), out=self.R_end)

    def rollout(self):
        if not self.use_graph:
            self._rollout()
            return
        if self.graph is None:
            snap = self._snapshot()
            s = torch.cuda.Stream()
            s.wait_stream(torch.cuda.current_stream())
            with torch.cuda.stream(s):
                self._rollout()
            torch.cuda.current_stream().wait_stream(s)
            torch.cuda.synchronize()
            self._restore(snap)
            self.graph = self._new_graph()
            with torch.cuda.graph(self.graph):
                self._rollout()
            self._restore(snap)
            self._graph_flags = {k: getattr(self.model.policy, k, False) for k in ('_enc_was_saved', '_mm_was_saved', '_bits_steps')}
        self.model.t = 0
        self.graph.replay()
        self.model.t = self.n_step
        for k, v in self._graph_flags.items():
            setattr(self.model.policy, k, v)

    def _new_graph(self):
        return torch.cuda.CUDAGraph(keep_graph=True) if self.keep_graphs else torch.cuda.CUDAGraph()

    def _select_lock_step_form(self):
        env, model = self.env, self.model
        if env.device.type == 'cuda' and self.saved_acts:
            model.policy.refresh_wimage()
        self.enc_in_kernel = self.saved_acts and self.compact_obs and env.device.type == 'cuda' and \
            model.policy.enc_in_kernel(env.E, True)
        self.env_in_kernel = self.enc_in_kernel and hasattr(env, 'inkernel_step') and env.n_agent == 8 and ops.step_env_supported() and \
            model.policy.env_step_in_kernel
        if not self.env_in_kernel and self.saved_acts and self.compact_obs and env.device.type == 'cuda' and \
                getattr(env, 'inkernel_step_supported', None) is not None and model.policy.coupled and \
                getattr(model.policy, 'encodes_in_step', None) is not None and 'ENC' in model.policy._extra and \
                os.environ.get('NMARL_GRID_ENV_IN_KERNEL', '1') != '0':
            self.env_in_kernel = bool(model.policy.encodes_in_step(env.E, True) and env.inkernel_step_supported())
        self.fused_encode = self._want_fused_encode and self.saved_acts and self.compact_obs and not self.enc_in_kernel and \
            getattr(env, 'supports_fused_encode', False) and env.device.type == 'cuda' and \
            model.policy.fused_env_encode(model.buf_fp[1], model.encode_target(1)) is not None

    def _shadow_tensors(self):
        return self.env.state_tensors() + [self.step_dev, self.model.h_fw, self.model.c_fw]

    def _state_tensors(self):
        m = self.model
        return self.env.state_tensors() + [m.h_fw, m.c_fw, m.buf_x[0], m.buf_fp[0], self.step_dev, self.done_pre]

    def _snapshot(self):
        return [t.clone() for t in self._state_tensors()]

    def _restore(self, snap):
        for t, s in zip(self._state_tensors(), snap):
            t.copy_(s)

    def _epilogue(self):
        m, T = self.model, self.n_step
        m.policy.invalidate_cached_msg()
        ops.batch_epilogue(self.buf_g, self.last_done, self.ep_sum, self.ep_sq, self.ep_len, self.fin, self.env.T,
                           m.h_fw, m.c_fw, m.h_bw, m.c_bw, m.buf_fp[T], m.buf_fp[0], m.fp_uniform, m.buf_x[T], m.buf_x[0],
                           self.done_pre, skip_if=self._status[:1] if self.handoff_guard else None)

    def _record(self, lr, lr_dev=None):
        if self.recorder is not None:
            self.recorder.record(lr, lr_dev=lr_dev, skip_if=self._status[:1] if self.handoff_guard else None)

    def _capture_update(self):
        m = self.model
        split = m.dist_group is not None
        inside = True
        tun = None
        try:
            import torch.cuda.tunable as tunable
            if tunable.is_enabled() and tunable.tuning_is_enabled():
                tun = tunable
                tunable.tuning_enable(False)
        except Exception:
            tun = None
        host = (m.t, m.policy._enc_was_saved, m.policy._mm_was_saved, m.policy._bits_steps)
        ops.keepalive_begin(self._keepalive)
        try:
            torch.cuda.synchronize()
            g1, g2 = self._new_graph(), None
            with torch.cuda.graph(g1):
                m.load_rewards(self.buf_rraw)
                m.update_grads(self.R_end)
                if not split:
                    m.update_apply(0.0, rotate=False, lr_dev=self.lr_dev)
                    self._record(0.0, lr_dev=self.lr_dev)
                    if inside:
                        self._epilogue()
            if split:
                g2 = self._new_graph()
                with torch.cuda.graph(g2):
                    m.update_apply(0.0, rotate=False, lr_dev=self.lr_dev)
                    self._record(0.0, lr_dev=self.lr_dev)
                    if inside:
                        self._epilogue()
            self._upd = dict(grads=g1, apply=g2, epilogue_inside=inside)
        finally:
            ops.keepalive_end()
            m.t, m.policy._enc_was_saved, m.policy._mm_was_saved, m.policy._bits_steps = host
            if tun is not None:
                tun.tuning_enable(True)

    def _update(self):
        m = self.model
        if self.capture_update and self._upd is None and self.update_capture_error is None and self.n_batches >= 1:
            try:
                self._capture_update()
            except Exception as ex:
                self.update_capture_error = repr(ex)
                self._upd = None
                logging.warning('update capture failed, staying eager: %r' % (ex,))
                torch.cuda.synchronize()
        if self._upd is None:
            m.load_rewards(self.buf_rraw)
            m.update(self.R_end, rotate=False)
            self._record(m.cur_lr)
            return False
        lr = m.update_begin()
        if lr != self._lr_dev_host:
            self.lr_dev.fill_(lr)
            self._lr_dev_host = lr
        m.t = self.n_step
        self._upd['grads'].replay()
        if self._upd['apply'] is not None:
            m.update_reduce()
            self._upd['apply'].replay()
        m.update_end()
        return self._upd['epilogue_inside']

    def run_batch(self):
        self.rollout()
        if not self._update():
            self._epilogue()
        self.n_batches += 1
# ... 409 lines not shown
```

include/nmarl.h:

```cpp
#ifndef NMARL_H
#define NMARL_H

#include <stdint.h>

#ifdef __cplusplus
extern "C" {
#endif

#define NMARL_OK 0
#define NMARL_EINVAL (-1)
#define NMARL_EHIP (-2)

#define NMARL_CACC_N 8
#define NMARL_CACC_NF 5
#define NMARL_CACC_OBS 15

int nmarl_abi_version(void);
const char* nmarl_source_hash(void);


typedef struct nmarl_cacc_params {
    float dt;
    float h_min;
    float h_star;
// ... 161 lines not shown
                        int64_t dh2_sn, const float* dc_new, int64_t dc_sn, float* dz, int64_t dz_sn,
                        float* dc_prev, int64_t dc_prev_sn, void* stream);
typedef struct nmarl_head {
    int32_t kind, A, mode, m_max;
    const float* w; int64_t w_sn;
    const float* b; int64_t b_sn;
    float* pi_out; int64_t pi_sn;
    uint8_t* act_out;
    const float* u;
    uint64_t seed;
    int64_t env_id_base, step;
    const int64_t* step_dev;
    const uint8_t* act_in;
    const int32_t* nbr_idx;
    float* v_out; int64_t v_sn;
    const float* w2; int64_t w2_sn;
    const float* b2; int64_t b2_sn;
} nmarl_head_t;
typedef struct nmarl_msg {
    int32_t kind, m_max, K, pad_;
    const int32_t* nbr_idx;
    const float* img; int64_t img_sn;
    const float* b; int64_t b_sn;
    const float* enc; int64_t enc_sn, enc_row;
    float* out; int64_t out_sn, out_row;
    uint32_t* sync;
    const float* ob; int64_t ob_row;
    int32_t ob_F, ob_segs;
    const int32_t* ob_nbr;
    const float* ob_img; int64_t ob_img_sn;
    const float* ob_b; int64_t ob_b_sn;
    int32_t* status;
    const float* src; int64_t src_sn;
    float* out2; int64_t out2_sn, out2_row;
    const float* next_img; int64_t next_img_sn;
    const float* next_b; int64_t next_b_sn;
    float* next_out; int64_t next_out_sn;
    float* mean_out; int64_t mean_out_sn, mean_out_row;
    const float* carry_in; int64_t carry_in_sn;
    float* carry_out; int64_t carry_out_sn;
    float* mean_next; int64_t mean_next_sn, mean_next_row;
} nmarl_msg_t;
typedef struct nmarl_step_enc {
    const float* ob; int64_t ob_row;
    const float* fp; int64_t fp_sn;
    const float *w_ob, *b_ob, *w_fp, *b_fp;
    int64_t w_ob_sn, b_ob_sn, w_fp_sn, b_fp_sn;
    float* out; int64_t out_sn, out_row;
    int32_t F, A, m_max, pad_;
    int32_t nbr[128];
    const nmarl_cacc_params_t* env;
    float *h, *v, *u; int32_t* t; uint8_t* collided; float* v0_init;
    float* obs_out; float* reward; uint8_t* done; float* global_reward;
    int32_t auto_reset, pad2_; uint64_t seed; int64_t env_id_base; int32_t* episode;
    uint32_t* cnt;
    uint32_t* relu_bits; int64_t relu_bits_sn;
} nmarl_step_enc_t;
typedef struct nmarl_grid_env {
    const nmarl_grid_params_t* params;
    float *q, *transit; uint8_t* prev_action; int32_t* t; float* xi;
    float* obs_out; float* reward; uint8_t* done; float* global_reward;
    int32_t auto_reset, pad_; uint64_t seed; int64_t env_id_base; int32_t* episode;
    uint64_t* words;
} nmarl_grid_env_t;
typedef struct nmarl_step_x {
    int64_t E;
    int32_t N, H, KX, KX2, precision, pad_;
    const float* x; int64_t x_sn, x_row;
    const float* x2; int64_t x2_sn, x2_row;
    const float* h_in; int64_t h_sn;
    const float* img; int64_t img_sn;
    const float* bias; int64_t bias_sn;
    const float* zadd1; int64_t zadd1_sn;
    const float* zadd2; int64_t zadd2_sn;
    const float* c_prev; int64_t c_prev_sn;
    const float* done;
    float* gates; int64_t gates_sn;
    float* c_new; int64_t c_new_sn;
    float* h_new; int64_t h_new_sn;
    const nmarl_head_t* head;
    const nmarl_msg_t* msg;
    const nmarl_step_enc_t* enc;
    const nmarl_grid_env_t* genv;
} nmarl_step_x_t;
int nmarl_lstm_wimage_floats(int32_t KX);
int nmarl_lstm_wimage(int32_t N, int32_t KX, const float* wx, int64_t wx_sn, const float* wh, int64_t wh_sn,
                      float* img, int64_t img_sn, int32_t precision, void* stream);
int nmarl_lstm_msg_wimage(int32_t N, int32_t K, const float* w_msg, int64_t w_sn, float* img, int64_t img_sn, void* stream);
int nmarl_lstm_step_sync_words(int64_t E, int32_t N);
int nmarl_lstm_step_env_words(int64_t E);
int nmarl_lstm_step_grid_words(int64_t E);
int nmarl_lstm_step_grid_env_blocks(int64_t E, int32_t N);
int nmarl_lstm_step_x(const nmarl_step_x_t* a, void* stream);
int nmarl_lstm_bptt_wimage_floats(int32_t KM);
int nmarl_lstm_bptt_wimage(int32_t N, int32_t KM, const float* wxm, int64_t wxm_sn, const float* wh, int64_t wh_sn,
                           float* img, int64_t img_sn, void* stream);
int nmarl_lstm_bptt_step_parts(int64_t E);
int nmarl_lstm_bptt_step(int64_t E, int32_t N, int32_t H, int32_t KM, const float* gates, int64_t gates_sn,
                         const float* c_prev, int64_t c_prev_sn, const float* c_new, int64_t c_new_sn,
                         const float* done, const float* dh, int64_t dh_sn, const float* dh2, int64_t dh2_sn,
                         const float* dc_in, int64_t dc_sn, const float* img, int64_t img_sn, float* dz,
                         int64_t dz_sn, float* dc_prev, int64_t dc_prev_sn, float* dx, int64_t dx_sn,
                         const float* mask, int64_t mask_sn, int64_t mask_row, float* dhd, int64_t dhd_sn,
                         int32_t apply_keep, float* db_part, int64_t db_sn, void* stream);
int nmarl_lstm_bptt_seq_blocks(int64_t E);
int nmarl_lstm_bptt_seq(int32_t T, int64_t E, int32_t N, int32_t H, const float* gates, int64_t gates_sn,
                        int64_t gates_st, const float* c_all, int64_t c_sn, int64_t c_st, const float* done,
                        const float* dh_ext, int64_t dh_sn, int64_t dh_st, const float* dy8, int64_t dy_sn, int64_t dy_st,
                        const float* hw, int64_t hw_sn, int32_t O, const float* img, int64_t img_sn,
                        float* dz, int64_t dz_sn, int64_t dz_st, float* db_part, int64_t db_sn, float* dh0,
                        int64_t dh0_sn, float* dc0, int64_t dc0_sn, void* stream);

typedef struct nmarl_bptt_coupled {
    int32_t kind, N, T, H, m_max, r_max, r_row, symmetric, mode, ring_slots;
    int64_t E;
    const float *gates, *c_all, *done, *dh_ext, *img, *img_m, *mask;
    float *dz, *d1, *ring, *db_part, *dbm_part, *dhr_io, *dc_io;
    void* ws;
    int32_t* status;
    const int32_t *rev_agent, *rev_col;
    const float* rev_w;
    int64_t gates_sn, gates_st, c_sn, c_st, dh_sn, dh_st, img_sn, imgm_sn, mask_sn, mask_st, mask_row, dz_sn, dz_st, d1_sn, d1_st,
        ring_sn, ring_slot, db_sn, dbm_sn, io_sn;
    const float *dy8, *hw;
    int64_t dy_sn, dy_st, hw_sn;
    int32_t O, pad2_;
} nmarl_bptt_coupled_t;
int nmarl_lstm_bptt_msg_wimage(int32_t N, int32_t K, const float* w_msg, int64_t w_sn, float* img, int64_t img_sn, void* stream);
int nmarl_lstm_bptt_coupled_ws_words(int64_t E, int32_t N);
int nmarl_lstm_bptt_coupled(const nmarl_bptt_coupled_t* p, void* stream);
typedef struct nmarl_bptt_dial {
    int32_t N, T, H, m_max, r_max, r_row, symmetric, mode, ring_slots, O;
    int64_t E;
    const float *gates, *c_all, *done, *dh_ext, *dy8, *hw, *img, *img_m, *img_f, *hm, *msg;
    float *dz, *ds, *d1, *d2, *ring, *db_part, *dbm_part, *dbf_part, *dhr_io, *dc_io;
    void* ws;
    int32_t* status;
    const int32_t *rev_agent, *rev_col;
    const float* rev_w;
    int64_t gates_sn, gates_st, c_sn, c_st, dh_sn, dh_st, dy_sn, dy_st, hw_sn, img_sn, imgm_sn, imgf_sn, hm_sn, hm_st, hm_row, msg_sn,
        msg_st, dz_sn, dz_st, ds_sn, ds_st, d1_sn, d1_st, d2_sn, d2_st, ring_sn, ring_slot, db_sn, dbm_sn, dbf_sn, io_sn;
} nmarl_bptt_dial_t;
int nmarl_lstm_bptt_dial(const nmarl_bptt_dial_t* p, void* stream);
int nmarl_bias_act(int64_t rows, int32_t N, int32_t W, const float* x, int64_t x_sn, const float* bias,
                   int64_t bias_sn, int32_t act, float* y, int64_t y_sn, int64_t y_row, void* stream);
int nmarl_dial_msg_adjoint_parts(int64_t E);
int nmarl_dial_msg_adjoint(int64_t E, int32_t N, int32_t m_max, const float* ds, int64_t ds_sn, const float* hm,
                           int64_t hm_sn, const float* msg, int64_t msg_sn, const float* dhd, int64_t dhd_sn,
                           const float* img_msg_t, int64_t img_msg_sn, const float* img_mfc_t, int64_t img_mfc_sn,
                           const int32_t* rev_agent, const int32_t* rev_col, const float* rev_w, int32_t r_row,
                           float* d1, int64_t d1_sn, float* d2, int64_t d2_sn, float* dh, int64_t dh_sn,
                           float* b1_part, int64_t b1_sn, float* b2_part, int64_t b2_sn, void* stream);
int nmarl_onehot_argmax_add(int64_t rows, int32_t N, int32_t A, int32_t W, const float* p, int64_t p_sn,
                            const float* scale, float* y, int64_t y_sn, int64_t y_row, void* stream);
int nmarl_fc_fwd(int64_t rows, int32_t N, int32_t F, int32_t J, const float* x, int64_t x_sn, int64_t x_row,
                 const float* w, int64_t w_sn, const float* b, int64_t b_sn, int32_t act, float* y,
                 int64_t y_sn, int64_t y_row, void* stream);
#define NMARL_FC_MAX_PARTS 4
typedef struct nmarl_fc_part {
    const float* x; int64_t x_sn, x_row;
    int32_t F, gather_A, m_max, pad_;
    const int32_t* nbr_idx;
    const float* w; int64_t w_sn;
    const float* b; int64_t b_sn;
} nmarl_fc_part_t;
int nmarl_fc_fwd_multi(int64_t rows, int32_t N, int32_t n_parts, const nmarl_fc_part_t* parts, int32_t act,
// ... 95 lines not shown
```

Before: 244.6 million env-steps/s.

## Carry the recurrent gate pre-activation between uncoupled LSTM policy-value steps

Adds a second compiled variant of the fused LSTM step kernel. In this variant the h_new·Wh gate term, already computed in the step's tail, is written to a per-agent [N,E,4H] buffer. The next step, when no episode resets occurred, loads that term instead of recomputing the recurrent K-chunks, so it only runs the input-side chunks. Python tracks a carry epoch that is bumped on weight-image refresh, epilogue and restore, so a stale carry is never consumed. The cost is an extra global store and load of the gate panel each step, plus more kernel instantiations.

Result: faster. 250.9 million env-steps/s, median of 6 (+2.6%).

```diff
diff --git a/deeprl_network_amd/_lib.py b/deeprl_network_amd/_lib.py
--- a/deeprl_network_amd/_lib.py
+++ b/deeprl_network_amd/_lib.py
@@ -155,7 +155,8 @@
                 [f for k in ('img', 'bias', 'zadd1', 'zadd2', 'c_prev') for f in ((k, C.c_void_p), (k + '_sn', C.c_int64))] +
                 [('done', C.c_void_p)] +
                 [f for k in ('gates', 'c_new', 'h_new') for f in ((k, C.c_void_p), (k + '_sn', C.c_int64))] +
-                [('head', C.POINTER(Head)), ('msg', C.POINTER(Msg)), ('enc', C.POINTER(StepEnc)), ('genv', C.POINTER(GridEnv))])
+                [('head', C.POINTER(Head)), ('msg', C.POINTER(Msg)), ('enc', C.POINTER(StepEnc)), ('genv', C.POINTER(GridEnv))] +
+                [('rec_in', C.c_void_p), ('rec_in_sn', C.c_int64), ('rec_out', C.c_void_p), ('rec_out_sn', C.c_int64)])
 
 
 _p = C.c_void_p
diff --git a/deeprl_network_amd/agents/models.py b/deeprl_network_amd/agents/models.py
--- a/deeprl_network_amd/agents/models.py
+++ b/deeprl_network_amd/agents/models.py
@@ -250,7 +250,7 @@
                                 self.buf_vn[:, t], h_out=self.H_all[:, t + 1], c_out=self.C_all[:, t + 1],
                                 gates=self.G_buf[:, t], defer_action_term=True,
                                 **(dict(save=self._save_slots(t), ob=ob, carry=self._msg_carry(t)) if p.coupled else
-                                   (dict(ob=ob) if ob is not None else {})),
+                                   (dict(ob=ob, carry=self._rec_carry(t, done_is_zero)) if ob is not None else {})),
                                 **draw)
             return self.buf_act[t]
         if self.save_acts:
@@ -270,6 +270,22 @@
 
     _carry_buf = None
     _carry_holds = -1
+    _carry_epoch = -1
+    _rec_buf = None
+    _rec_holds = -1
+    _rec_epoch = -1
+
+    def _rec_carry(self, t, done_is_zero):
+        p = self.policy
+        if p.coupled:
+            return None
+        if self._rec_buf is None:
+            self._rec_buf = torch.zeros(self.n_agent, self.E, 4 * self.n_lstm, dtype=F32, device=self.device)
+        on = ops.rec_carry_enabled()
+        take = on and bool(done_is_zero) and t > 1 and self._rec_holds == t and self._rec_epoch == p.carry_epoch
+        hand = bool(done_is_zero) and (t < self.n_step or (not on and t > 1))
+        self._rec_holds, self._rec_epoch = (t + 1 if hand else -1), p.carry_epoch
+        return dict(rec_in=self._rec_buf if take else None, rec_out=self._rec_buf if hand else None)
 
     def _msg_carry(self, t):
         p = self.policy
@@ -278,12 +294,12 @@
             return None
         if self._carry_buf is None:
             self._carry_buf = torch.zeros(self.n_agent, self.E, self.n_lstm, dtype=F32, device=self.device)
-        d = dict(carry_in=self._carry_buf if (t > 0 and self._carry_holds == t) else None,
+        d = dict(carry_in=self._carry_buf if (t > 0 and self._carry_holds == t and self._carry_epoch == p.carry_epoch) else None,
                  carry_out=self._carry_buf if t < self.n_step else None)
         mm = getattr(p, '_extra_full', {}).get('MM')
         if mm is not None and t + 1 < self.n_step and p.msg_kind == ops.MSG_MEAN_ADD:
             d['mean_next'] = mm[:, t + 1]
-        self._carry_holds = t + 1 if t < self.n_step else -1
+        self._carry_holds, self._carry_epoch = (t + 1 if t < self.n_step else -1), p.carry_epoch
         return d
 
     S_bits = None
@@ -337,7 +353,8 @@
             p.step_policy_value(enc, self.H_all[:, T], self.C_all[:, T], done, self._pi_boot, action_scratch, self._v_boot,
                                 h_out=self.h_fw, c_out=self.c_fw, mode=mode, u=u, seed=seed, env_id_base=env_id_base,
                                 step=step, step_dev=step_dev, **(dict(ob=ob) if ob is not None else {}),
-                                **(dict(carry=self._msg_carry(T)) if p.coupled else {}))
+                                **(dict(carry=self._msg_carry(T)) if p.coupled else
+                                   (dict(carry=self._rec_carry(T, done_is_zero)) if ob is not None else {})))
             return self._v_boot
         if self.save_acts:
             T = self.n_step
diff --git a/deeprl_network_amd/agents/policies.py b/deeprl_network_amd/agents/policies.py
--- a/deeprl_network_amd/agents/policies.py
+++ b/deeprl_network_amd/agents/policies.py
@@ -351,7 +351,7 @@
     _bits_steps = 0
 
     def invalidate_cached_msg(self):
-        """(lstm_dial keeps message vectors of the last policy step: see DIALMultiAgentPolicy)"""
+        self.carry_epoch += 1
 
     def enc_in_kernel(self, E, compact):
         return False
@@ -362,6 +362,7 @@
 
     def step_policy_value(self, enc, h, c, done, pi_out, act_out, v_out, h_out=None, c_out=None, gates=None,
                           defer_action_term=False, save=None, ob=None, carry=None, **draw):
+        rec_kw = {}
         with torch.no_grad():
             if self.coupled:
                 z1, z2, xs = self._recur_addends(enc, h, save=save, fuse_msg=True)
@@ -377,12 +378,14 @@
             elif ob is not None:
                 z1, z2, xs = None, None, (self._enc_spec(ob['x'], ob['fp'], enc, ob.get('env'), ob.get('bits')), self.params[self.k_wx],
                                           self._step_img)
+                if carry and ops.rec_carry_supported(h, xs, self.precision):
+                    rec_kw = dict(rec=carry)
             else:
                 z1, z2, xs = self._recur_addends(enc, h)
             p = self.params
             ops.lstm_step_policy_value(h, p[self.k_wh], p[self.k_b], z1, z2, c, done, p['pi_w'], p['pi_b'], pi_out, act_out,
                                        p['v_w'], p['v_b'], self.nbr_idx, self.n_a, v_out, xs=xs, h_out=h_out, c_out=c_out,
-                                       gates=gates, defer_action_term=defer_action_term, **self._prec_kw, **draw)
+                                       gates=gates, defer_action_term=defer_action_term, **self._prec_kw, **rec_kw, **draw)
         return act_out
 
     @property
@@ -499,7 +502,10 @@
     def xside(self):
         return self.k_wx is not None and ops.xside_supported(self.params[self.k_wx].shape[1], self.n_h)
 
+    carry_epoch = 0
+
     def refresh_wimage(self):
+        self.carry_epoch += 1
         if self.xside:
             self._img = ops.lstm_wimage(self.params[self.k_wx], self.params[self.k_wh], out=self._img)
             if self.precision == 'bf16x3':
@@ -946,6 +952,7 @@
         self._m_next = None
 
     def invalidate_cached_msg(self):
+        super().invalidate_cached_msg()
         self._m_next = None
 
     def _cached_msg(self, h):
diff --git a/deeprl_network_amd/csrc/lstm_mfma.hip b/deeprl_network_amd/csrc/lstm_mfma.hip
--- a/deeprl_network_amd/csrc/lstm_mfma.hip
+++ b/deeprl_network_amd/csrc/lstm_mfma.hip
@@ -1,3 +1,4 @@
+#ifndef NMARL_STEP_SECOND_PASS
 #include "common.h"
 #include "cacc_tile.h"
 #include "grid_tile.h"
@@ -230,6 +231,8 @@
     float* gv_obs; float* gv_rew; uint8_t* gv_done; float* gv_grew;
     uint64_t gv_seed; int64_t gv_base; int32_t* gv_episode;
     unsigned long long* gv_words;
+    const float* rec_in; int64_t rec_in_sn;
+    float* rec_out; int64_t rec_out_sn;
 };
 
 typedef unsigned int u32x4v __attribute__((__vector_size__(16)));
@@ -323,8 +326,10 @@
 }
 
 
+#define NMARL_STEP_KERNEL lstm_step_x_kernel
+#endif
 template <int HEAD, int MSG, int ENC = 0, int CARRY = 0, int PREC = 0>
-__global__ __launch_bounds__(512, 1) void lstm_step_x_kernel(const XArgs xa) {
+__global__ __launch_bounds__(512, 1) void NMARL_STEP_KERNEL(const XArgs xa) {
     extern __shared__ __attribute__((aligned(16))) float lds[];
     const FusedArgs& a = xa.f;
     NMARL_STAMP(0)
@@ -380,6 +385,10 @@
     static_assert(HEAD != 4 || MSG != 0, "HEAD 4 is the coupled nets' policy + value step");
     static_assert(PREC == 0 || MSG == 0, "bf16x3: the uncoupled nets' step forms only");
     constexpr bool PV = HEAD == 3 || HEAD == 4;
+    constexpr int REC = HEAD == 3 ? CARRY : 0;
+    constexpr bool CANON = REC != 0;
+    constexpr bool TAKE = REC == 2;
+    static_assert(REC == 0 || (HEAD == 3 && MSG == 0 && PREC == 0 && ENC != 0), "REC: the uncoupled fp32 policy + value step with the encoders inside");
     unsigned epoch_raw = 0;
     if (HEAD == 4) epoch_raw = __hip_atomic_load((gu32*)xa.sync, __ATOMIC_RELAXED, __HIP_MEMORY_SCOPE_AGENT);
     int nbj[8];
@@ -436,7 +445,10 @@
     const float* hrow = a.h_in + (int64_t)n * a.h_sn + arow * H + 4 * grp;
     float4 a0, a1, n0, n1;
 #define NMARL_A_LOAD(ch, d0, d1)      \
-    if (ENC_LDS) {       \
+    if (TAKE) {                                  \
+        const int xc_ = (ch) < nx ? (ch) : nx - 1;                                        \
+        d0 = xslot[512 * (2 * xc_)]; d1 = xslot[512 * (2 * xc_ + 1)];                     \
+    } else if (ENC_LDS) {       \
         const int hc_ = (ch) - nx < 0 ? 0 : (ch) - nx;                                    \
         const int xc_ = (ch) < nx ? (ch) : nx - 1;                                        \
         const float4 h0_ = *reinterpret_cast<const float4*>(hrow + hc_ * CH_K);           \
@@ -634,7 +646,7 @@
     using K2 = std::integral_constant<int, 2>;
     using K4 = std::integral_constant<int, 4>;
     constexpr bool MSG_WIDE = HEAD != 4 && MSG == 1;
-    static_assert(CARRY == 0 || (HEAD == 4 && (MSG == 1 || MSG == 2)), "the message carry exists between one-launch lock-steps");
+    static_assert(CARRY == 0 || HEAD == 3 || (HEAD == 4 && (MSG == 1 || MSG == 2)), "the message carry exists between one-launch lock-steps");
     constexpr bool carried = CARRY == 2;
     if (MSG != 0) {
         if (carried) {
@@ -1028,6 +1040,53 @@
     if (DEPH && lag) __builtin_amdgcn_s_setprio(1);
     int bsel = lag ? NBUF - 1 : 0;
     int wsel = 2 % NBUF;
+    if constexpr (TAKE) {
+        const float* ri = xa.rec_in + (int64_t)n * xa.rec_in_sn + 4 * c;
+#pragma unroll
+        for (int g4 = 0; g4 < 4; ++g4)
+#pragma unroll
+            for (int r = 0; r < 4; ++r) {
+                const float4 v4 = *reinterpret_cast<const float4*>(ri + rofs[r] * G4 + g4 * H);
+                zs[4 * g4 + 0][r] = v4.x; zs[4 * g4 + 1][r] = v4.y; zs[4 * g4 + 2][r] = v4.z; zs[4 * g4 + 3][r] = v4.w;
+            }
+    }
+#define NMARL_TICK(TAU)                                                                   \
+    {                                                                                     \
+        const int ch = (TAU);                                                             \
+        const int chn = ch + 1 < nch ? ch + 1 : nch - 1;                                  \
+        NMARL_A_LOAD(chn, n0, n1)                                                         \
+        NMARL_KCHUNK(lds + bsel * CH_FLOATS, a0, a1)                                      \
+        if (ENC_LDS && ch < nx && e_out != nullptr && row0 + c < a.E) {                   \
+            float* so = e_out + (int64_t)n * e_out_sn + (row0 + c) * e_out_row + 4 * grp + ch * CH_K; \
+            *reinterpret_cast<float4*>(so) = a0;                                          \
+            *reinterpret_cast<float4*>(so + 16) = a1;                                     \
+        }                                                                                 \
+        NMARL_STAMP(2 + 2 * ch)                                                           \
+        __syncthreads();                                                                  \
+        NMARL_STAMP(3 + 2 * ch)                                                           \
+        if (ch + 2 < nch) NMARL_STAGE_STORE(wsel)                                         \
+        const int chs = ch + 3 < nch ? ch + 3 : nch - 1;                                  \
+        NMARL_STAGE_LOAD(chs)                                                             \
+        a0 = n0; a1 = n1;                                                                 \
+        NMARL_A_MASK(chn, a0, a1)                                                         \
+        bsel = bsel + 1 == NBUF ? 0 : bsel + 1;                                           \
+        wsel = wsel + 1 == NBUF ? 0 : wsel + 1;                                           \
+    }
+    if constexpr (CANON) {
+        for (int tau = 0; tau < nx; ++tau) NMARL_TICK(tau)
+        if constexpr (TAKE) {
+            __syncthreads();
+#pragma unroll
+            for (int t = 0; t < 16; ++t) { const f32x4 xs_ = acc[t]; acc[t] = xs_ + zs[t]; zs[t] = xs_; }
+        } else {
+#pragma unroll
+            for (int t = 0; t < 16; ++t) { zs[t] = acc[t]; acc[t] = f32x4{0.f, 0.f, 0.f, 0.f}; }
+            NMARL_TICK(nx)
+            NMARL_TICK(nx + 1)
+#pragma unroll
+            for (int t = 0; t < 16; ++t) acc[t] = zs[t] + acc[t];
+        }
+    } else {
     for (int tau = 0; tau < nch; ++tau) {
         const int ch = tau - lag;
         const int chn = ch + 1 < nch ? ch + 1 : nch - 1;
@@ -1062,6 +1121,8 @@
         }
         NMARL_KCHUNK(lds + bsel * CH_FLOATS, a0, a1)
     }
+    }
+#undef NMARL_TICK
     NMARL_STAMP(20)
     if (CP_PARK) {
         const float4 v = *cp_park;
@@ -1211,7 +1272,7 @@
             }
         } else {
 #pragma unroll
-            for (int t = 0; t < 16; ++t) acc[t] = zs[t];
+            for (int t = 0; t < 16; ++t) acc[t] = CANON ? f32x4{0.f, 0.f, 0.f, 0.f} : zs[t];
         }
 #pragma unroll
         for (int hc = 0; hc < 2; ++hc) {
@@ -1220,6 +1281,22 @@
             r0.x = ar[0] * keepA; r0.y = ar[1] * keepA; r0.z = ar[2] * keepA; r0.w = ar[3] * keepA;
             r1.x = ar[16] * keepA; r1.y = ar[17] * keepA; r1.z = ar[18] * keepA; r1.w = ar[19] * keepA;
             NMARL_KCHUNK(lds + ((nx + hc) % NBUF) * CH_FLOATS, r0, r1)
+        }
+        if constexpr (CANON) {
+            {
+                const bool on_ = xa.rec_out != nullptr;
+                const __amdgpu_buffer_rsrc_t rr_ = make_rsrc(on_ ? xa.rec_out + (int64_t)n * xa.rec_out_sn : a.h_new, on_ ? (uint32_t)(a.E * (G4 * 4)) : 0u);
+                const uint32_t ro_ = (uint32_t)(((row0 + 4 * grp) * G4 + 4 * c) * 4);
+#pragma unroll
+                for (int r = 0; r < 4; ++r)
+#pragma unroll
+                    for (int g4 = 0; g4 < 4; ++g4)
+                        __builtin_amdgcn_raw_buffer_store_b128(
+                            __builtin_bit_cast(u32x4v, float4{acc[4 * g4 + 0][r], acc[4 * g4 + 1][r], acc[4 * g4 + 2][r], acc[4 * g4 + 3][r]}), rr_,
+                            ro_ + (uint32_t)((r * G4 + g4 * H) * 4), 0, 0);
+            }
+#pragma unroll
+            for (int t = 0; t < 16; ++t) acc[t] = zs[t] + acc[t];
         }
         NMARL_STAMP(23)
         __builtin_amdgcn_wave_barrier();
@@ -1347,6 +1424,13 @@
 #undef NMARL_A_MASK
 #undef NMARL_KCHUNK
 }
+
+#ifndef NMARL_STEP_SECOND_PASS
+#define NMARL_STEP_SECOND_PASS
+#undef NMARL_STEP_KERNEL
+#define NMARL_STEP_KERNEL lstm_step_rec_kernel
+#include "lstm_mfma.hip"
+#undef NMARL_STEP_KERNEL
 
 __global__ void lstm_wimage_kernel(const int N, const int KX, const float* wx, const int64_t wx_sn, const float* wh,
                                    const int64_t wh_sn, float* img, const int64_t img_sn) {
@@ -1534,6 +1618,12 @@
             return NMARL_EINVAL;
     }
     if (kind < 0 || kind > 3 || (mk == 3 && kind == 3)) return NMARL_EINVAL;
+    if ((s->rec_in || s->rec_out) && (kind != 3 || mk != 0 || prec != 0 || !enc)) return NMARL_EINVAL;
+    if (s->rec_in && (!stride_ok(s->rec_in_sn, E * G4) || ((uintptr_t)s->rec_in % 16))) return NMARL_EINVAL;
+    if (s->rec_out && (!stride_ok(s->rec_out_sn, E * G4) || ((uintptr_t)s->rec_out % 16) ||
+                       (E + ROWS_B) * (int64_t)(G4 * 4) >= (int64_t)1 << 32))
+        return NMARL_EINVAL;
+    const int rec = s->rec_in ? 2 : s->rec_out ? 1 : 0;
     if (kind != 0 && E > 0) {
         if (head->A <= 0 || head->A > MAXA || !head->w || !head->b || head->b_sn < (kind == 2 ? 1 : head->A)) return NMARL_EINVAL;
         if ((kind == 1 || kind == 3) && (head->w_sn < (int64_t)H * head->A || !head->pi_out || head->pi_sn < E * head->A || !head->act_out ||
@@ -1568,6 +1658,7 @@
     xa.x2 = KX2 > 0 ? x2 : nullptr; xa.x2_sn = x2_sn; xa.x2_row = x2_row;
     xa.img = img; xa.img_sn = img_sn;
     xa.nx = KX / CH_K; xa.nx1 = (KX - KX2) / CH_K; xa.N = N;
+    xa.rec_in = s->rec_in; xa.rec_in_sn = s->rec_in_sn; xa.rec_out = s->rec_out; xa.rec_out_sn = s->rec_out_sn;
     if (mk) {
         xa.msg_kc = msg->K / CH_K; xa.m_max = msg->m_max; xa.nbr_idx = msg->nbr_idx; xa.msg_img = msg->img;
         xa.msg_img_sn = msg->img_sn; xa.msg_b = msg->b; xa.msg_b_sn = msg->b_sn; xa.enc = msg->enc; xa.enc_sn = msg->enc_sn;
@@ -1653,12 +1744,26 @@
             if (hipFuncSetAttribute(reinterpret_cast<const void*>(lstm_step_x_kernel<3, 0, 3>), hipFuncAttributeMaxDynamicSharedMemorySize,
                                     (int)lb_g) != hipSuccess ||
                 hipFuncSetAttribute(reinterpret_cast<const void*>(lstm_step_x_kernel<3, 0, 4>), hipFuncAttributeMaxDynamicSharedMemorySize,
+                                    (int)lb_g) != hipSuccess ||
+                hipFuncSetAttribute(reinterpret_cast<const void*>(lstm_step_rec_kernel<3, 0, 3, 1, 0>), hipFuncAttributeMaxDynamicSharedMemorySize,
+                                    (int)lb_g) != hipSuccess ||
+                hipFuncSetAttribute(reinterpret_cast<const void*>(lstm_step_rec_kernel<3, 0, 3, 2, 0>), hipFuncAttributeMaxDynamicSharedMemorySize,
+                                    (int)lb_g) != hipSuccess ||
+                hipFuncSetAttribute(reinterpret_cast<const void*>(lstm_step_rec_kernel<3, 0, 4, 1, 0>), hipFuncAttributeMaxDynamicSharedMemorySize,
+                                    (int)lb_g) != hipSuccess ||
+                hipFuncSetAttribute(reinterpret_cast<const void*>(lstm_step_rec_kernel<3, 0, 4, 2, 0>), hipFuncAttributeMaxDynamicSharedMemorySize,
                                     (int)lb_g) != hipSuccess)
                 return NMARL_EHIP;
             gen_once.done(bit);
         }
         hipStream_t st = static_cast<hipStream_t>(stream);
-        if (single) hipLaunchKernelGGL((lstm_step_x_kernel<3, 0, 4>), grid, dim3(512), lb_g, st, xa);
+        if (rec == 2) {
+            if (single) hipLaunchKernelGGL((lstm_step_rec_kernel<3, 0, 4, 2, 0>), grid, dim3(512), lb_g, st, xa);
+            else hipLaunchKernelGGL((lstm_step_rec_kernel<3, 0, 3, 2, 0>), grid, dim3(512), lb_g, st, xa);
+        } else if (rec == 1) {
+            if (single) hipLaunchKernelGGL((lstm_step_rec_kernel<3, 0, 4, 1, 0>), grid, dim3(512), lb_g, st, xa);
+            else hipLaunchKernelGGL((lstm_step_rec_kernel<3, 0, 3, 1, 0>), grid, dim3(512), lb_g, st, xa);
+        } else if (single) hipLaunchKernelGGL((lstm_step_x_kernel<3, 0, 4>), grid, dim3(512), lb_g, st, xa);
         else hipLaunchKernelGGL((lstm_step_x_kernel<3, 0, 3>), grid, dim3(512), lb_g, st, xa);
         return nmarl_check_launch();
     }
@@ -1713,6 +1818,14 @@
                     hipFuncSetAttribute(reinterpret_cast<const void*>(lstm_step_x_kernel<3, 0, 1, 0, 1>), hipFuncAttributeMaxDynamicSharedMemorySize,
                                         (int)lb_e) != hipSuccess ||
                     hipFuncSetAttribute(reinterpret_cast<const void*>(lstm_step_x_kernel<3, 0, 2, 0, 1>), hipFuncAttributeMaxDynamicSharedMemorySize,
+                                        (int)lb_e) != hipSuccess ||
+                    hipFuncSetAttribute(reinterpret_cast<const void*>(lstm_step_rec_kernel<3, 0, 1, 1, 0>), hipFuncAttributeMaxDynamicSharedMemorySize,
+                                    (int)lb_e) != hipSuccess ||
+                hipFuncSetAttribute(reinterpret_cast<const void*>(lstm_step_rec_kernel<3, 0, 1, 2, 0>), hipFuncAttributeMaxDynamicSharedMemorySize,
+                                        (int)lb_e) != hipSuccess ||
+                    hipFuncSetAttribute(reinterpret_cast<const void*>(lstm_step_rec_kernel<3, 0, 2, 1, 0>), hipFuncAttributeMaxDynamicSharedMemorySize,
+                                    (int)lb_e) != hipSuccess ||
+                hipFuncSetAttribute(reinterpret_cast<const void*>(lstm_step_rec_kernel<3, 0, 2, 2, 0>), hipFuncAttributeMaxDynamicSharedMemorySize,
                                         (int)lb_e) != hipSuccess)
                     return NMARL_EHIP;
                 enc_once.done(bit);
@@ -1721,6 +1834,12 @@
             if (prec) {
                 if (single) hipLaunchKernelGGL((lstm_step_x_kernel<3, 0, 2, 0, 1>), grid, dim3(512), lb_e, st, xa);
                 else hipLaunchKernelGGL((lstm_step_x_kernel<3, 0, 1, 0, 1>), grid, dim3(512), lb_e, st, xa);
+            } else if (rec == 2) {
+                if (single) hipLaunchKernelGGL((lstm_step_rec_kernel<3, 0, 2, 2, 0>), grid, dim3(512), lb_e, st, xa);
+                else hipLaunchKernelGGL((lstm_step_rec_kernel<3, 0, 1, 2, 0>), grid, dim3(512), lb_e, st, xa);
+            } else if (rec == 1) {
+                if (single) hipLaunchKernelGGL((lstm_step_rec_kernel<3, 0, 2, 1, 0>), grid, dim3(512), lb_e, st, xa);
+                else hipLaunchKernelGGL((lstm_step_rec_kernel<3, 0, 1, 1, 0>), grid, dim3(512), lb_e, st, xa);
             } else if (single) hipLaunchKernelGGL((lstm_step_x_kernel<3, 0, 2>), grid, dim3(512), lb_e, st, xa);
             else hipLaunchKernelGGL((lstm_step_x_kernel<3, 0, 1>), grid, dim3(512), lb_e, st, xa);
             return nmarl_check_launch();
@@ -1784,7 +1903,8 @@
     else if (carry == 1) hipLaunchKernelGGL((lstm_step_x_kernel<4, MS, EN, 1>), grid, dim3(512), lb + lb_extra, st, xa);         \
     else hipLaunchKernelGGL((lstm_step_x_kernel<4, MS, EN, 0>), grid, dim3(512), lb + lb_extra, st, xa);
     if (mk == 0) {
-        if (kind == 0) NMARL_LX(0, 0); else if (kind == 1) NMARL_LX(1, 0); else if (kind == 2) NMARL_LX(2, 0); else NMARL_LX(3, 0);
+        if (kind == 0) NMARL_LX(0, 0); else if (kind == 1) NMARL_LX(1, 0); else if (kind == 2) NMARL_LX(2, 0);
+        else NMARL_LX(3, 0);
     } else if (mk == 1) {
         if (kind == 1) NMARL_LX(1, 1); else if (kind == 2) NMARL_LX(2, 1);
         else if (enc) { NMARL_LC(1, 1) }
@@ -1818,3 +1938,4 @@
     return nmarl_check_launch();
 }
 #endif
+#endif
diff --git a/deeprl_network_amd/ops.py b/deeprl_network_amd/ops.py
--- a/deeprl_network_amd/ops.py
+++ b/deeprl_network_amd/ops.py
@@ -242,7 +242,16 @@
     return out
 
 
-def _step_x(h, bias, zadd1, zadd2, c_prev, done, gates, c_out, h_out, xs, head, what, precision='fp32'):
+def rec_carry_enabled():
+    return os.environ.get('NMARL_REC_CARRY', '1') != '0'
+
+
+def rec_carry_supported(h, xs, precision='fp32'):
+    return bool(h.is_cuda and h.shape[2] == FUSED_H and precision == 'fp32' and xs is not None and
+                isinstance(xs[0], dict) and len(xs) <= 3)
+
+
+def _step_x(h, bias, zadd1, zadd2, c_prev, done, gates, c_out, h_out, xs, head, what, precision='fp32', rec=None):
     N, E, H = h.shape
     x, _, img = xs[:3]
     x2 = xs[3] if len(xs) > 3 else None
@@ -275,6 +284,13 @@
             a.x2, a.x2_sn, a.x2_row = _rows_view(x2, K2, what + ' x2')
         a.KX, a.KX2 = K1 + K2 + (H if msg is not None else 0), K2
     a.img, a.img_sn = _img_arg(img, N, a.KX, precision, what)
+    for key in ('rec_in', 'rec_out'):
+        rb = rec.get(key) if rec else None
+        if rb is not None:
+            if rb.shape != (N, E, 4 * H) or rb.stride(2) != 1 or rb.stride(1) != 4 * H:
+                raise _lib.NmarlError('%s: rec["%s"] must be [N,E,256] with contiguous panels' % (what, key))
+            setattr(a, key, ptr(rb, F32, strided=True))
+            setattr(a, key + '_sn', rb.stride(0))
     if msg is not None:
         if head is None or x2 is not None or zadd1 is not None or zadd2 is not None:
             raise _lib.NmarlError('%s: the in-kernel message term needs a head and excludes x2 / addends' % what)
@@ -539,7 +555,7 @@
 
 def lstm_step_policy_value(h, wh, bias, zadd1, zadd2, c, done, pi_w, pi_b, pi_out, act_out, v_w, v_b, nbr_idx, n_a,
                            v_out, mode, u=None, seed=0, env_id_base=0, step=0, step_dev=None, xs=None, h_out=None,
-                           c_out=None, gates=None, defer_action_term=False, precision='fp32'):
+                           c_out=None, gates=None, defer_action_term=False, precision='fp32', rec=None):
     N, E, H = h.shape
     hd = _lib.Head()
     hd.kind, hd.A, hd.mode = 3, pi_w.shape[2], mode
@@ -554,7 +570,7 @@
         raise _lib.NmarlError('lstm_step_policy_value: v_out must be [N,E] with unit column stride')
     hd.v_out, hd.v_sn = ptr(v_out, F32, strided=True), v_out.stride(0)
     h_out, c_out = (h if h_out is None else h_out), (c if c_out is None else c_out)
-    _step_x(h, bias, zadd1, zadd2, c, done, gates, c_out, h_out, _xs_or_image(xs, wh), hd, 'nmarl_lstm_step_x[pv]', precision)
+    _step_x(h, bias, zadd1, zadd2, c, done, gates, c_out, h_out, _xs_or_image(xs, wh), hd, 'nmarl_lstm_step_x[pv]', precision, rec=rec)
     if not defer_action_term:
         if not v_out.is_contiguous():
             raise _lib.NmarlError('lstm_step_policy_value: the neighbour-action add needs a contiguous v_out')
diff --git a/deeprl_network_amd/utils.py b/deeprl_network_amd/utils.py
--- a/deeprl_network_amd/utils.py
+++ b/deeprl_network_amd/utils.py
@@ -378,6 +378,7 @@
     def _restore(self, snap):
         for t, s in zip(self._state_tensors(), snap):
             t.copy_(s)
+        self.model.policy.invalidate_cached_msg()
 
     def _epilogue(self):
         m, T = self.model, self.n_step
diff --git a/include/nmarl.h b/include/nmarl.h
--- a/include/nmarl.h
+++ b/include/nmarl.h
@@ -267,6 +267,8 @@
     const nmarl_msg_t* msg;
     const nmarl_step_enc_t* enc;
     const nmarl_grid_env_t* genv;
+    const float* rec_in; int64_t rec_in_sn;
+    float* rec_out; int64_t rec_out_sn;
 } nmarl_step_x_t;
 int nmarl_lstm_wimage_floats(int32_t KX);
 int nmarl_lstm_wimage(int32_t N, int32_t KX, const float* wx, int64_t wx_sn, const float* wh, int64_t wh_sn,
```
